# heheyas/V3D

Hardware: AMD Instinct MI355X
Metric: multi-view frames/sec, V3D_512 18-frame 25-step EDM (higher is better)
Workload: dtype bf16; 1 GPU; BASELINE.json configs[1]: V3D_512 random-init SVD-XT weights, 1x18x4x64x64 latent, 25 EulerEDM steps, cfg 4.5 (LinearPredictionGuider), 18-frame VideoDecoder decode to 512x512, one sample per GPU; frames=18, edm_steps=25, parallelism=replica x1, hip_graph=False

## Files before the change

include/v3d_hip.h:

```cpp
#ifndef V3D_HIP_H
#define V3D_HIP_H

#include <stdint.h>

#ifdef __cplusplus
extern "C" {
#endif

#define V3D_ABI_VERSION 9

typedef void* v3d_stream_t;

enum {
    V3D_OK = 0,
    V3D_ERR_ARG = -1,
    V3D_ERR_LAUNCH = -2,
};

int v3d_abi_version(void);
const char* v3d_last_error(void);
int v3d_device_info(int32_t* out4);

enum { V3D_GEMM_LINEAR = 0, V3D_GEMM_CONV3X3 = 1, V3D_GEMM_CONVT3 = 2 };

typedef struct v3d_gemm_args {
    const void* A;
    const void* W;
    void* out;
    const float* bias;
    const float* add;
    const void* res1;
    const void* res2;
    const float* coef;
    int64_t M, N, K;
    int64_t lda, ldw, ldo, ldr1, ldr2;
    int64_t a_rows;
    int64_t a_row0;
    int64_t add_rpg, add_ld;
    int64_t coef_rpg;
    float c_acc, c_res1, c_res2;
    int32_t mode, geglu, out_fp32;
    int32_t Hin, Win, Hout, Wout, stride, up;
    int32_t T, tmin, tmax;
    int64_t S;
    int32_t batch;
    int32_t pad_mode;
    int64_t sA, sW, sO;
    int64_t halo_rows;
    float* gn_stats;
    int64_t gn_rps;
    int32_t gn_cpg;
    int32_t gn_in_silu;
    int64_t gn_nslots;
    const float* gn_in_table;
    int64_t gn_in_rps;
    int64_t gn_in_rows;
    const void* A2;
    int64_t K1, lda2;
} v3d_gemm_args;

int v3d_gemm(const v3d_gemm_args* args, v3d_stream_t stream);
int v3d_gemm_gn_in_supported(const v3d_gemm_args* args);

int v3d_ff_fused(const void* x, int64_t ldx, const void* W1p, const float* b1, const void* W2p, const float* b2,
                 const void* res1, int64_t ldr1, const void* res2, int64_t ldr2, const float* coef, int64_t coef_rpg,
                 float c_acc, float c_res1, float c_res2, void* out, int64_t ldo, int64_t M, int32_t C, int32_t hidden,
                 v3d_stream_t stream);

int v3d_ln_ff_fused(const void* x, int64_t ldx, float ln_eps, const void* W1p, const float* b1, const void* W2p, const float* b2,
                 const void* res1, int64_t ldr1, const void* res2, int64_t ldr2, const float* coef, int64_t coef_rpg,
                 float c_acc, float c_res1, float c_res2, void* out, int64_t ldo, int64_t M, int32_t C, int32_t hidden,
                 v3d_stream_t stream);
int v3d_ln_proj(const void* x, int64_t ldx, float eps, const void* Wp, const float* bias, void* out, int64_t ldo, void* outT,
                int64_t M, int32_t C, int32_t N, int32_t n_rm, int64_t S, v3d_stream_t stream);
int v3d_sizeof_gemm_args(void);

int v3d_groupnorm_stats(const void* x1, int64_t C1, const void* x2, int64_t C2, float* stats, int64_t nslots,
                        int64_t n_img, int64_t S, int32_t groups, int64_t imgs_per_stat, v3d_stream_t stream);
int v3d_groupnorm_stats_table(const void* x1, int64_t C1, const void* x2, int64_t C2, float* stats, int64_t nslots, uint32_t* tickets,
                              int64_t n_img, int64_t S, int32_t groups, int64_t imgs_per_stat, const float* gamma, const float* beta,
                              double count, float eps, float* table, v3d_stream_t stream);
int v3d_groupnorm_finalize(const float* stats, int64_t nslots, double* sums, int64_t n_stat, int32_t groups,
                           const float* gamma, const float* beta, int64_t C, double count, float eps, float* table,
                           v3d_stream_t stream);
int v3d_groupnorm_apply(const void* x1, int64_t C1, const void* x2, int64_t C2, const float* table, void* out,
                        int64_t n_img, int64_t S, int64_t imgs_per_stat, int32_t silu, v3d_stream_t stream);

int v3d_groupnorm_small_supported(int64_t C1, int64_t C2, int64_t S, int32_t groups, int64_t imgs_per_stat);
int v3d_groupnorm_small(const void* x1, int64_t C1, const void* x2, int64_t C2, const float* gamma, const float* beta, void* out,
                        int64_t n_img, int64_t S, int32_t groups, int64_t imgs_per_stat, float eps, int32_t silu, v3d_stream_t stream);

int v3d_layernorm(const void* x, const float* add, int64_t add_rpg, int64_t add_ld, void* xsum_out,
                  const float* gamma, const float* beta, void* out, int64_t M, int64_t C, float eps,
                  v3d_stream_t stream);

int v3d_attn_spatial(const void* q, int64_t ldq, const void* k, int64_t ldk, const void* vT, void* out,
                     int64_t ldo, int64_t n_img, int64_t S, int32_t heads, float scale, v3d_stream_t stream);

int v3d_attn_spatial_ld(const void* q, int64_t ldq, const void* k, int64_t ldk, const void* vT, int64_t ldv, void* out,
                        int64_t ldo, int64_t n_img, int64_t S, int32_t heads, float scale, v3d_stream_t stream);

int v3d_quant_fp8_tiles(const void* x, int64_t ldx, void* x8, int64_t ld8, float* scales, int64_t n_img, int64_t S, int32_t ncols,
                        v3d_stream_t stream);
int v3d_quant_fp8_slab(const void* vT, void* v8, float* vscale, void* amax_scratch, int64_t n_img, int64_t S, int32_t heads, v3d_stream_t stream);
int v3d_attn_spatial_fp8(const void* qk8, int64_t ld8, const float* scales, const void* v8, const float* vscale, void* out, int64_t ldo,
                         int64_t n_img, int64_t S, int32_t heads, float scale, v3d_stream_t stream);

int v3d_attn_temporal(const void* q, int64_t q_sb, int64_t q_st, int64_t q_ss,
                      const void* k, const void* v, int64_t kv_sb, int64_t kv_st, int64_t kv_ss,
                      void* out, int64_t o_sb, int64_t o_st, int64_t o_ss,
                      int64_t B, int32_t Tq, int32_t Tk, int64_t S, int32_t heads, float scale,
                      v3d_stream_t stream);

int v3d_attn_vae_d512(const void* q, int64_t ldq, const void* k, int64_t ldk, const void* vT, const float* bias, void* out,
                      int64_t ldo, int64_t n_img, int64_t S, int32_t C, float scale, v3d_stream_t stream);

int v3d_softmax_rows(const float* in, void* out, int64_t rows, int64_t L, v3d_stream_t stream);

int v3d_timestep_embedding(const float* t, void* out_bf16, int64_t n, int32_t dim, float max_period, v3d_stream_t stream);
int v3d_silu_add(const float* in, const float* in2, void* out_bf16, int64_t n, v3d_stream_t stream);
int v3d_edm_scalings(const float* sigma, float* c_skip, float* c_out, float* c_in, float* c_noise, int64_t n, v3d_stream_t stream);
int v3d_pack_input(const float* x, const float* scale, int64_t C1, const float* cond, int64_t C2, void* out_bf16,
                   int64_t n, int64_t S, int64_t Cpad, v3d_stream_t stream);
int v3d_pack_input_im2col3x3(const float* x, const float* scale, int64_t C1, const float* cond, int64_t C2, void* out_bf16,
                             int64_t n, int32_t H, int32_t W, int64_t Kpad, v3d_stream_t stream);
int v3d_tapsum3x3(const float* y, int64_t ldy, const float* bias, float* out, int64_t n, int32_t H, int32_t W, int32_t C,
                  v3d_stream_t stream);
int v3d_denoise_combine(const float* net, int64_t ldn, const float* x, const float* c_out, const float* c_skip,
                        float* out, int64_t n, int64_t C, int64_t S, v3d_stream_t stream);
int v3d_cfg_combine(const float* x, const float* scale, float* out, int64_t n, int64_t T, int64_t chw, v3d_stream_t stream);
int v3d_euler_step(const float* x, const float* den, const float* sigma, const float* next_sigma, float* out,
                   int64_t n, int64_t chw, v3d_stream_t stream);
int v3d_heun_step(const float* x, const float* den, const float* euler, const float* den2, const float* sigma,
                  const float* next_sigma, float* out, int64_t n, int64_t chw, v3d_stream_t stream);
int v3d_clip_preprocess(const float* img, int64_t B, int32_t H, int32_t W, int32_t S, int32_t P, int32_t antialias,
                        const float* mean3, const float* std3, void* patches_bf16, int32_t Kpad, v3d_stream_t stream);
int v3d_gelu_bf16(const void* in, void* out, int64_t n, v3d_stream_t stream);
int v3d_frames_to_uint8(const float* x, void* out_u8, int64_t n, int32_t C, int64_t S, v3d_stream_t stream);
int v3d_axpb_f32(const float* x, float a, float b, float* out, int64_t n, v3d_stream_t stream);
int v3d_blend_coefs(const float* alpha, const int32_t* kind, const float* ioi, float* out, int64_t n_mixers, int64_t n_img, v3d_stream_t stream);
int v3d_nchw_to_nhwc_bf16(const float* x, float scale, void* out_bf16, int64_t n, int64_t C, int64_t S, int64_t Cpad, v3d_stream_t stream);
int v3d_tmix_small(const float* x, int64_t ld, const float* w, const float* b, float* out, int64_t B, int32_t T,
                   int64_t S, int32_t Cc, int32_t tmin, int32_t tmax, int64_t row0, v3d_stream_t stream);
int v3d_randn_add(const float* x, float scale, uint64_t seed, uint32_t call, float* out, int64_t B, int64_t T_local, int64_t T_global,
                  int64_t t0, int64_t row_elems, v3d_stream_t stream);
int v3d_lincomb_f32(const float* const* src, const float* coef, int32_t nterms, float* out, int64_t n, v3d_stream_t stream);
int v3d_copy2d_bf16(const void* src, int64_t lds, void* dst, int64_t ldd, int64_t rows, int64_t C, v3d_stream_t stream);

typedef struct v3d_gs_camera {
    float view[16];
    float proj[16];
    float tanfovx, tanfovy;
    float bg[3];
    int32_t width, height;
} v3d_gs_camera;

int v3d_gs_knn3(const float* xyz, int64_t n, float* out, v3d_stream_t stream);
int v3d_gs_preprocess_fwd(const float* xyz, const float* scale_raw, const float* rot_raw, const float* opacity_raw, const float* f_dc, int64_t P,
                          const v3d_gs_camera* cam, float* means2d, float* conic_opacity, float* rgb, float* depth, int32_t* radii,
                          int32_t* tiles_touched, int32_t* clamped, v3d_stream_t stream);
int64_t v3d_gs_scan_work_bytes(int64_t n);
int v3d_gs_scan(const int32_t* in, int64_t n, int32_t* out, void* work, int64_t work_bytes, v3d_stream_t stream);
int v3d_gs_duplicate_keys(const float* means2d, const int32_t* radii, const float* depth, const int32_t* offsets, int64_t P, int32_t width,
                          int32_t height, uint64_t* keys, uint32_t* vals, v3d_stream_t stream);
int64_t v3d_gs_sort_work_bytes(int64_t n);
int v3d_gs_radix_sort_pairs(const uint64_t* keys_in, const uint32_t* vals_in, uint64_t* keys_out, uint32_t* vals_out, int64_t n, int32_t nbits,
                            void* work, int64_t work_bytes, v3d_stream_t stream);
int v3d_gs_tile_ranges(const uint64_t* keys_sorted, const uint32_t* vals_sorted, int64_t n_inst, const float* means2d, const int32_t* radii,
                       const int32_t* offsets, int32_t width, int32_t height, int32_t* ranges, int32_t* inst_pos, v3d_stream_t stream);
int v3d_gs_render_fwd(const int32_t* ranges, const uint32_t* vals_sorted, const float* means2d, const float* conic_opacity, const float* rgb,
                      const v3d_gs_camera* cam, float* out_img, float* final_T, int32_t* n_contrib, v3d_stream_t stream);
int v3d_gs_render_bwd(const int32_t* ranges, const uint32_t* vals_sorted, const float* means2d, const float* conic_opacity, const float* rgb,
                      const v3d_gs_camera* cam, const float* final_T, const int32_t* n_contrib, const float* dL_dimg, float* inst_grads,
                      v3d_stream_t stream);
int v3d_gs_reduce_instance_grads(const float* inst_grads, const int32_t* offsets, const int32_t* inst_pos, int64_t P, float* grads9,
                                 v3d_stream_t stream);
int v3d_gs_preprocess_bwd(const float* xyz, const float* scale_raw, const float* rot_raw, const float* opacity_raw, int64_t P,
                          const v3d_gs_camera* cam, const int32_t* radii, const int32_t* clamped, const float* grads9, float* d_xyz,
                          float* d_scale_raw, float* d_rot_raw, float* d_opacity_raw, float* d_f_dc, float* d_means2d, v3d_stream_t stream);
int64_t v3d_gs_ssim_work_floats(int32_t C, int32_t H, int32_t W);
int v3d_gs_ssim_l1_fwd(const float* img, const float* gt, int32_t C, int32_t H, int32_t W, float lambda_dssim, float* work, int64_t work_floats,
                       float* out3, v3d_stream_t stream);
int v3d_gs_ssim_l1_bwd(const float* img, const float* gt, int32_t C, int32_t H, int32_t W, float lambda_dssim, float* work, int64_t work_floats,
                       const float* dloss, float* grad, v3d_stream_t stream);

#ifdef __cplusplus
}
#endif
#endif
```

v3d_amd/csrc/gemm.hip:

```cpp
#include <stdlib.h>

#include <map>
#include <mutex>
#include <vector>
#include <type_traits>

#include "gemm_common.h"


namespace {

__device__ __attribute__((aligned(256))) unsigned int g_zero_page[16384] = {0};

template <int KS>
__device__ __forceinline__ int swz_row(int row) {
    if (KS == 1) return (0x78 >> (((row >> 2) & 3) * 2)) & 3;
    return (row >> 1) & 7;
}

template <int BM, int BN, int WGM, int WGN, int NS, int KS, int MODE, bool GEGLU>
__global__ __launch_bounds__(64 * WGM * WGN, (64 * WGM * WGN) == 256 ? 2 : 1) void gemm_kernel_v2(GP p) {
    constexpr int BK2 = 32 * KS;
    constexpr int ROWB = BK2 * 2;
    constexpr int RPP = 1024 / ROWB;
// ... 114 lines not shown
    asm volatile("" ::: "memory");
    constexpr int NFO_ = GEGLU ? NF / 2 : NF;
    constexpr int STAGE_REGION = MF * 16 * (NFO_ * 32 + 16);
    constexpr bool CAN_STAGE = NW * STAGE_REGION <= NS * STAGE_BYTES;
    epilogue<MF, NF, GEGLU, CAN_STAGE>(p, acc, m0 + wm * WM, n0 + wn * WN, z, lane, lds + (CAN_STAGE ? wave * STAGE_REGION : 0));
}

constexpr int BK = 64;
constexpr int LROW = BK + 8;

template <int BM, int BN, int MODE, bool GEGLU>
__global__ __launch_bounds__(256, 2) void gemm_kernel_v1(GP p) {
    constexpr int AI = BM / 32;
    constexpr int BI = BN / 32;
    constexpr int WM = BM / 2, WN = BN / 2;
    constexpr int MF = WM / 16, NF = WN / 16;
    __shared__ __attribute__((aligned(16))) bf16_t sA[2][BM * LROW];
    __shared__ __attribute__((aligned(16))) bf16_t sB[2][BN * LROW];

    const int tid = threadIdx.x;
    const int lane = tid & 63;
    const int wave = tid >> 6;
    const int wm = wave >> 1, wn = wave & 1;
    const int bid = xcd_remap(blockIdx.x, p.mt * p.nt);
    int tile_m, tile_n;
    tile_coords(p, bid, tile_m, tile_n);
    const long long m0 = (long long)tile_m * BM;
    const long long n0 = (long long)tile_n * BN;
    const long long z = blockIdx.y;
    const bufrsrc_t rsA = make_rsrc(p.A + z * p.sA, p.a_bytes);
    const bufrsrc_t rsW = make_rsrc(p.W + z * p.sW, p.w_bytes);
    const int kc = tid & 7;
    const int r0 = tid >> 3;
    RowInfo<MODE> ri[AI];
#pragma unroll
    for (int i = 0; i < AI; ++i) ri[i].init(p, m0 + r0 + 32 * i);
    u32x4 ra[AI], rb[BI];
    unsigned aoff[AI], boff[BI];
    const int ksteps = (int)((p.K + BK - 1) / BK);
    const int nsteps = ksteps * ntaps<MODE>();
    int ld_tap = 0, ld_k0 = 0;
    auto set_tap = [&](int tap) {
#pragma unroll
        for (int i = 0; i < AI; ++i) {
            long long srow;
            const bool ok = ri[i].tap(p, tap, srow);
            aoff[i] = ok ? (unsigned)(((srow + p.a_row0) * p.lda + kc * 8) * 2) : kInvalid;
        }
#pragma unroll
        for (int i = 0; i < BI; ++i) {
            const long long n = n0 + r0 + 32 * i;
            boff[i] = (n < p.N) ? (unsigned)((((long long)tap * p.N + n) * p.ldw + kc * 8) * 2) : kInvalid;
        }
    };
    set_tap(0);
    auto gload = [&]() {
        const bool kok = (ld_k0 + kc * 8) < p.K;
        const unsigned kb = (unsigned)ld_k0 * 2u;
#pragma unroll
        for (int i = 0; i < AI; ++i) ra[i] = buf_load16(rsA, (kok && aoff[i] != kInvalid) ? aoff[i] + kb : kInvalid);
#pragma unroll
        for (int i = 0; i < BI; ++i) rb[i] = buf_load16(rsW, (kok && boff[i] != kInvalid) ? boff[i] + kb : kInvalid);
        ld_k0 += BK;
        if (ld_k0 >= p.K) {
            ld_k0 = 0;
            ++ld_tap;
            if (ntaps<MODE>() > 1 && ld_tap < ntaps<MODE>()) set_tap(ld_tap);
        }
    };
    auto lstore = [&](int buf) {
#pragma unroll
        for (int i = 0; i < AI; ++i) *reinterpret_cast<u32x4*>(&sA[buf][(r0 + 32 * i) * LROW + kc * 8]) = ra[i];
#pragma unroll
        for (int i = 0; i < BI; ++i) *reinterpret_cast<u32x4*>(&sB[buf][(r0 + 32 * i) * LROW + kc * 8]) = rb[i];
    };
    f32x4 acc[MF][NF];
#pragma unroll
    for (int i = 0; i < MF; ++i)
#pragma unroll
        for (int j = 0; j < NF; ++j) acc[i][j] = f32x4{0.f, 0.f, 0.f, 0.f};
    gload();
    lstore(0);
    __syncthreads();
    const int frow = lane & 15;
    const int fk = (lane >> 4) * 8;
    for (int step = 0; step < nsteps; ++step) {
        const int buf = step & 1;
        if (step + 1 < nsteps) gload();
#pragma unroll
        for (int kk = 0; kk < BK / 32; ++kk) {
            bf16x8 xf[MF], wf[NF];
#pragma unroll
            for (int i = 0; i < MF; ++i)
                xf[i] = *reinterpret_cast<const bf16x8*>(&sA[buf][(wm * WM + i * 16 + frow) * LROW + kk * 32 + fk]);
#pragma unroll
            for (int j = 0; j < NF; ++j)
                wf[j] = *reinterpret_cast<const bf16x8*>(&sB[buf][(wn * WN + j * 16 + frow) * LROW + kk * 32 + fk]);
#pragma unroll
            for (int i = 0; i < MF; ++i)
#pragma unroll
                for (int j = 0; j < NF; ++j)
                    acc[i][j] = __builtin_amdgcn_mfma_f32_16x16x32_bf16(wf[j], xf[i], acc[i][j], 0, 0, 0);
        }
        if (step + 1 < nsteps) lstore(buf ^ 1);
        __syncthreads();
    }
    epilogue<MF, NF, GEGLU, false>(p, acc, m0 + wm * WM, n0 + wn * WN, z, lane, nullptr);
}


template <int BM, int BN, int WGM, int WGN, int MODE, bool GEGLU, int EMF, int NS = 4, int SPAD = 16, bool GN = false>
__global__ __launch_bounds__(512, NS == 3 ? 4 : 2) void gemm_kernel_v3(GP p, int ntiles) {
    constexpr int ROWB = 64, NW = 8;
    static_assert(WGM * WGN == NW, "8 waves");
    constexpr int WM = BM / WGM, WN = BN / WGN;
    constexpr int MF = WM / 16, NF = WN / 16;
    static_assert(MF % EMF == 0, "epilogue chunking");
    constexpr int NPIECE = (BM + BN) / 16;
    constexpr int PPW = NPIECE / NW;
    static_assert(PPW * NW == NPIECE && PPW * 2 < 64, "tile / wave-count mismatch");
    constexpr int APIECES = BM / 16;
    constexpr int STAGE_BYTES = (BM + BN) * ROWB;
    constexpr int NFO = GEGLU ? NF / 2 : NF;
    constexpr int EPI_REGION = EMF * 16 * (NFO * 32 + SPAD);
    __shared__ __attribute__((aligned(1024))) unsigned char lds[NS * STAGE_BYTES + NW * EPI_REGION];

    const int tid = threadIdx.x;
    const int lane = tid & 63;
    const int wave = __builtin_amdgcn_readfirstlane(tid >> 6);
    const int grp = wave >> 2;
    const int wm = wave / WGN, wn = wave % WGN;
    const bf16_t* __restrict__ A = p.A;
    const bf16_t* __restrict__ W = p.W;
    unsigned char* estage = lds + NS * STAGE_BYTES + wave * EPI_REGION;

    const int G = gridDim.x;
    const int my_tiles = (ntiles - (int)blockIdx.x + G - 1) / G;
    auto tile_origin = [&](int it, long long& m0, long long& n0) __attribute__((always_inline)) {
        const int id = xcd_remap((int)blockIdx.x + it * G, ntiles);
        int tm, tn;
        tile_coords(p, id, tm, tn);
        n0 = (long long)tn * BN;
        m0 = (long long)tm * BM;
    };

    const bufrsrc_t rsA = make_rsrc(A, p.a_bytes);
    const bufrsrc_t rsW = make_rsrc(W, p.w_bytes);
    const int prow = lane >> 2;
    const unsigned kchunk_b = (unsigned)(((lane & 3) ^ swz_row<1>(prow)) * 16);
    RowInfo<MODE> ri[PPW];
    unsigned voff[PPW];
    long long ld_n0 = 0;
    int ld_it = 0, ld_tap = 0, ld_k0 = 0;
    auto set_tap = [&](int tap) __attribute__((always_inline)) {
#pragma unroll
        for (int i = 0; i < PPW; ++i) {
            const int q = wave + NW * i;
            if (q < APIECES) {
                long long s_;
                const bool ok = ri[i].tap(p, tap, s_);
                voff[i] = ok ? (unsigned)((s_ + p.a_row0) * p.lda * 2) + kchunk_b : kInvalid;
            } else {
                const long long n = ld_n0 + (q - APIECES) * 16 + prow;
                voff[i] = (n < p.N) ? (unsigned)(((long long)tap * p.N + n) * p.ldw * 2) + kchunk_b : kInvalid;
            }
        }
    };
    auto set_tile = [&](int it) __attribute__((always_inline)) {
        long long m0;
        tile_origin(it, m0, ld_n0);
#pragma unroll
        for (int i = 0; i < PPW; ++i) {
            const int q = wave + NW * i;
            if (q < APIECES) ri[i].init(p, m0 + q * 16 + prow);
        }
        set_tap(0);
    };
    set_tile(0);
    auto issue_piece = [&](int stage, int i, int so) __attribute__((always_inline)) {
        const int q = wave + NW * i;
        __builtin_amdgcn_raw_ptr_buffer_load_lds(q < APIECES ? rsA : rsW, (__attribute__((address_space(3))) void*)(lds + stage * STAGE_BYTES + q * 1024), 16, (int)voff[i], so, 0, 0);
    };
    auto issue_advance = [&]() __attribute__((always_inline)) {
        ld_k0 += 32;
        if (ld_k0 >= (int)p.K) {
            ld_k0 = 0;
            if (++ld_tap < ntaps<MODE>()) {
                set_tap(ld_tap);
            } else {
                ld_tap = 0;
                if (++ld_it < my_tiles) set_tile(ld_it);
                else if (ntaps<MODE>() > 1) set_tap(0);
            }
        }
    };
    auto issue = [&](int stage) __attribute__((always_inline)) {
        const int so = __builtin_amdgcn_readfirstlane(ld_k0 * 2);
#pragma unroll
        for (int i = 0; i < PPW; ++i) issue_piece(stage, i, so);
        issue_advance();
    };

    f32x4 acc[MF][NF];
#pragma unroll
    for (int i = 0; i < MF; ++i)
#pragma unroll
        for (int j = 0; j < NF; ++j) acc[i][j] = f32x4{0.f, 0.f, 0.f, 0.f};
    const int frag_off = (lane & 15) * ROWB + (((lane >> 4) ^ swz_row<1>(lane & 15)) * 16);
    const int a_base = wm * WM * ROWB;
    const int b_base = BM * ROWB + wn * WN * ROWB;
    bf16x8 xf[MF], wf[NF];

    const int nsteps = (int)(p.K / 32) * ntaps<MODE>();

#pragma unroll
    for (int st = 0; st < NS - 1; ++st) issue(st);
    asm volatile("s_waitcnt vmcnt(%0)" ::"n"(PPW * (NS - 2)) : "memory");
    __builtin_amdgcn_s_barrier();
    __builtin_amdgcn_sched_barrier(0);
    int s = 0;
    int rd = 0;
    for (int it = 0; it < my_tiles; ++it) {
        for (int kt = 0; kt < nsteps; ++kt, ++s) {
            {
                const unsigned char* sb = lds + rd * STAGE_BYTES;
#pragma unroll
                for (int i = 0; i < MF; ++i) xf[i] = *reinterpret_cast<const bf16x8*>(sb + a_base + frag_off + i * 16 * ROWB);
#pragma unroll
                for (int j = 0; j < NF; ++j) wf[j] = *reinterpret_cast<const bf16x8*>(sb + b_base + frag_off + j * 16 * ROWB);
            }
            issue(rd == 0 ? NS - 1 : rd - 1);
            rd = (rd + 1 == NS) ? 0 : rd + 1;
            if (grp == 1) {
                asm volatile("s_waitcnt lgkmcnt(0)" ::: "memory");
                __builtin_amdgcn_sched_barrier(0);
            }
            if (grp == 1) {
                asm volatile("s_waitcnt vmcnt(%0)" ::"n"(PPW * (NS - 2)) : "memory");
                __builtin_amdgcn_s_barrier();
                __builtin_amdgcn_sched_barrier(0);
            }
            __builtin_amdgcn_s_setprio(1);
#pragma unroll
            for (int i = 0; i < MF; ++i)
#pragma unroll
                for (int j = 0; j < NF; ++j)
                    acc[i][j] = __builtin_amdgcn_mfma_f32_16x16x32_bf16(wf[j], xf[i], acc[i][j], 0, 0, 0);
            __builtin_amdgcn_s_setprio(0);
            __builtin_amdgcn_sched_barrier(0);
            if (grp == 0) {
                asm volatile("s_waitcnt vmcnt(%0)" ::"n"(PPW * (NS - 2)) : "memory");
                __builtin_amdgcn_s_barrier();
            }
            __builtin_amdgcn_sched_barrier(0);
        }
        long long e_m0, e_n0;
        tile_origin(it, e_m0, e_n0);
        if constexpr (!GEGLU && EMF == 1 && SPAD == 16) {
            const long long mw0 = e_m0 + wm * WM, nw0 = e_n0 + wn * WN;
            if (mw0 < p.M && nw0 < p.N) {
                int lane_e = lane;
                asm volatile("" : "+v"(lane_e));
                auto rowfn = [&](int f) __attribute__((always_inline)) -> long long { return mw0 + f * 16; };
                E4GnRun<WM, MF> run;
                if constexpr (GN) run.init(mw0, p.gn_rps);
                auto flushfn = [&](int f, long long, unsigned& slot, unsigned& sid) __attribute__((always_inline)) -> bool { return run.step(f, slot, sid); };
                e4_retire_tile<MF, NF, GN>(p, acc, nw0, lane_e, estage, rowfn, flushfn);
            }
        } else
        {
            const long long mw0 = e_m0 + wm * WM, nw0 = e_n0 + wn * WN;
            const bool inside = mw0 < p.M && nw0 < p.N;
            const bool res_pre = p.res1 && !p.out_fp32 && (p.ldr1 % 8 == 0) && (reinterpret_cast<uintptr_t>(p.res1) % 16 == 0) && inside;
            u32x4 r0 = {0u, 0u, 0u, 0u}, r1 = r0, r2 = r0;
            if (res_pre) {
                r0 = load_res_piece<0, EMF, NF, GEGLU>(p, mw0, nw0, lane);
                r1 = load_res_piece<1, EMF, NF, GEGLU>(p, mw0, nw0, lane);
                r2 = load_res_piece<2, EMF, NF, GEGLU>(p, mw0, nw0, lane);
            }
            float4 bv[NF];
#pragma unroll
            for (int j = 0; j < NF; ++j)
                bv[j] = (p.bias && inside) ? *reinterpret_cast<const float4*>(p.bias + (int)nw0 + (lane >> 4) * 4 + j * 16) : make_float4(0.f, 0.f, 0.f, 0.f);
            GnAcc<GN ? NF : 1> gn;
            long long sid0 = 0;
            unsigned rem0 = 0;
            if constexpr (GN) {
                gn_zero(gn);
                sid0 = mw0 / p.gn_rps;
                rem0 = (unsigned)(mw0 - sid0 * p.gn_rps);
            }
            if (!GN || inside) v3_retire_chunks<0, MF / EMF, EMF, NF, GEGLU, SPAD, GN>(p, acc, mw0, nw0, lane, estage, r0, r1, r2, res_pre, bv, gn, sid0, rem0);
        }
#pragma unroll
        for (int i = 0; i < MF; ++i)
#pragma unroll
            for (int j = 0; j < NF; ++j) acc[i][j] = f32x4{0.f, 0.f, 0.f, 0.f};
    }
    asm volatile("s_waitcnt vmcnt(0)" ::: "memory");
}

template <int BM, int BN, int NS, int MODE>
__global__ __launch_bounds__(256, 2) void gemm_kernel_v6(GP p, int ntiles) {
    constexpr int ROWB = 64, NW = 4, WGN = 2;
    constexpr int WM = BM / 2, WN = BN / WGN, MF = WM / 16, NF = WN / 16;
    static_assert(NF == 5 || NF == 4, "the hand-managed epilogue retires 80- or 64-channel wave tiles");
    constexpr int NPIECE = (BM + BN) / 16, PPW = (NPIECE + NW - 1) / NW, APIECES = BM / 16, ARI = (APIECES + NW - 1) / NW;
    static_assert(PPW * (NS - 2) < 64, "vmcnt range");
    constexpr int STAGE_BYTES = NPIECE * 1024;
    constexpr int DUMMY_OFF = NS * STAGE_BYTES, NDUMMY = PPW * NW - NPIECE;
    constexpr int EPI_OFF = DUMMY_OFF + NDUMMY * 1024, EPI_REGION = 16 * (NF * 32 + 16);
    __shared__ __attribute__((aligned(1024))) unsigned char lds[EPI_OFF + NW * EPI_REGION];
    static_assert(sizeof(lds) <= 80 * 1024, "two blocks per CU");

    const int tid = threadIdx.x;
    const int lane = tid & 63;
    const int wave = __builtin_amdgcn_readfirstlane(tid >> 6);
    const int wm = wave / WGN, wn = wave % WGN;
    unsigned char* estage = lds + EPI_OFF + wave * EPI_REGION;
    const int G = gridDim.x;
    const int my_tiles = (ntiles - (int)blockIdx.x + G - 1) / G;
    auto tile_origin = [&](int it, long long& m0, long long& n0) __attribute__((always_inline)) {
        const int id = xcd_remap((int)blockIdx.x + it * G, ntiles);
        int tm, tn;
        tile_coords(p, id, tm, tn);
        n0 = (long long)tn * BN;
        m0 = (long long)tm * BM;
    };
    const bufrsrc_t rsA = make_rsrc(p.A, p.a_bytes);
    const bufrsrc_t rsW = make_rsrc(p.W, p.w_bytes);
    const int prow = lane >> 2;
    const unsigned kchunk_b = (unsigned)(((lane & 3) ^ swz_row<1>(prow)) * 16);
    RowInfo<MODE> ri[ARI];
    unsigned voff[PPW];
    long long ld_n0 = 0;
    int ld_it = 0, ld_tap = 0, ld_k0 = 0;
    auto set_tap = [&](int tap) __attribute__((always_inline)) {
#pragma unroll
        for (int i = 0; i < PPW; ++i) {
            const int q = wave + NW * i;
            if (i < ARI && q < APIECES) {
                long long s_;
                const bool ok = ri[i < ARI ? i : 0].tap(p, tap, s_);
                voff[i] = ok ? (unsigned)((s_ + p.a_row0) * p.lda * 2) + kchunk_b : kInvalid;
            } else {
                const long long n = ld_n0 + (q - APIECES) * 16 + prow;
                voff[i] = (q < NPIECE && n < p.N) ? (unsigned)(((long long)tap * p.N + n) * p.ldw * 2) + kchunk_b : kInvalid;
            }
        }
    };
    auto set_tile = [&](int it) __attribute__((always_inline)) {
        long long m0;
        tile_origin(it, m0, ld_n0);
#pragma unroll
        for (int i = 0; i < ARI; ++i) {
            const int q = wave + NW * i;
            if (q < APIECES) ri[i].init(p, m0 + q * 16 + prow);
        }
        set_tap(0);
    };
    set_tile(0);
    auto issue = [&](int stage) __attribute__((always_inline)) {
        const int so = __builtin_amdgcn_readfirstlane(ld_k0 * 2);
#pragma unroll
        for (int i = 0; i < PPW; ++i) {
            const int q = wave + NW * i;
            const int dst = q < NPIECE ? stage * STAGE_BYTES + q * 1024 : DUMMY_OFF + (q - NPIECE) * 1024;
            __builtin_amdgcn_raw_ptr_buffer_load_lds(q < APIECES ? rsA : rsW, (__attribute__((address_space(3))) void*)(lds + dst), 16, (int)voff[i], so, 0, 0);
        }
        ld_k0 += 32;
        if (ld_k0 >= (int)p.K) {
            ld_k0 = 0;
            if (++ld_tap < ntaps<MODE>()) {
                set_tap(ld_tap);
            } else {
                ld_tap = 0;
                if (++ld_it < my_tiles) set_tile(ld_it);
                else if (ntaps<MODE>() > 1) set_tap(0);
            }
        }
    };
    f32x4 acc[MF][NF];
#pragma unroll
    for (int i = 0; i < MF; ++i)
#pragma unroll
        for (int j = 0; j < NF; ++j) acc[i][j] = f32x4{0.f, 0.f, 0.f, 0.f};
    const int frag_off = (lane & 15) * ROWB + (((lane >> 4) ^ swz_row<1>(lane & 15)) * 16);
    const int a_base = wm * WM * ROWB;
    const int b_base = BM * ROWB + wn * WN * ROWB;
    bf16x8 xf[MF], wf[NF];
    const int nsteps = (int)(p.K / 32) * ntaps<MODE>();
#pragma unroll
    for (int st = 0; st < NS - 1; ++st) issue(st);
    asm volatile("s_waitcnt vmcnt(%0)" ::"n"(PPW * (NS - 2)) : "memory");
    __builtin_amdgcn_s_barrier();
    __builtin_amdgcn_sched_barrier(0);
    int rd = 0;
    for (int it = 0; it < my_tiles; ++it) {
        for (int kt = 0; kt < nsteps; ++kt) {
            {
                const unsigned char* sb = lds + rd * STAGE_BYTES;
#pragma unroll
                for (int i = 0; i < MF; ++i) xf[i] = *reinterpret_cast<const bf16x8*>(sb + a_base + frag_off + i * 16 * ROWB);
#pragma unroll
                for (int j = 0; j < NF; ++j) wf[j] = *reinterpret_cast<const bf16x8*>(sb + b_base + frag_off + j * 16 * ROWB);
            }
            issue(rd == 0 ? NS - 1 : rd - 1);
            rd = (rd + 1 == NS) ? 0 : rd + 1;
            __builtin_amdgcn_s_setprio(1);
#pragma unroll
            for (int i = 0; i < MF; ++i)
#pragma unroll
                for (int j = 0; j < NF; ++j)
                    acc[i][j] = __builtin_amdgcn_mfma_f32_16x16x32_bf16(wf[j], xf[i], acc[i][j], 0, 0, 0);
            __builtin_amdgcn_s_setprio(0);
            __builtin_amdgcn_sched_barrier(0);
            asm volatile("s_waitcnt vmcnt(%0)" ::"n"(PPW * (NS - 2)) : "memory");
            __builtin_amdgcn_s_barrier();
            __builtin_amdgcn_sched_barrier(0);
        }
        long long e_m0, e_n0;
        tile_origin(it, e_m0, e_n0);
        const long long mw0 = e_m0 + wm * WM, nw0 = e_n0 + wn * WN;
        if (mw0 < p.M && nw0 < p.N) {
            int lane_e = lane;
            asm volatile("" : "+v"(lane_e));
            auto rowfn = [&](int f) __attribute__((always_inline)) -> long long { return mw0 + f * 16; };
            auto flushfn = [&](int, long long, unsigned&, unsigned&) __attribute__((always_inline)) -> bool { return false; };
            e4_retire_tile<MF, NF, false>(p, acc, nw0, lane_e, estage, rowfn, flushfn);
        }
#pragma unroll
        for (int i = 0; i < MF; ++i)
#pragma unroll
            for (int j = 0; j < NF; ++j) acc[i][j] = f32x4{0.f, 0.f, 0.f, 0.f};
    }
    asm volatile("s_waitcnt vmcnt(0)" ::: "memory");
}

__global__ __launch_bounds__(256) void splitk_finalize_kernel(GP p) {
    const long long n4 = p.N / 4;
    const long long idx = (long long)blockIdx.x * 256 + threadIdx.x;
    if (idx >= p.M * n4) return;
    const long long m = idx / n4;
    const int n = (int)(idx - m * n4) * 4;
    float4 a = make_float4(0.f, 0.f, 0.f, 0.f);
    for (int sp = 0; sp < p.split_n; ++sp) {
        const float4 w = *reinterpret_cast<const float4*>(p.ws + ((long long)sp * p.M + m) * p.N + n);
        a.x += w.x; a.y += w.y; a.z += w.z; a.w += w.w;
    }
    if (p.bias) {
        const float4 b = *reinterpret_cast<const float4*>(p.bias + n);
        a.x += b.x; a.y += b.y; a.z += b.z; a.w += b.w;
    }
    if (p.add) {
        const float4 b = *reinterpret_cast<const float4*>(p.add + (m / p.add_rpg) * p.add_ld + n);
        a.x += b.x; a.y += b.y; a.z += b.z; a.w += b.w;
    }
    float ca = p.c_acc, c1 = p.c_res1, c2 = p.c_res2;
    if (p.coef) {
        const float* cf = p.coef + (m / p.coef_rpg) * 3;
        ca = cf[0]; c1 = cf[1]; c2 = cf[2];
    }
    float o[4] = {ca * a.x, ca * a.y, ca * a.z, ca * a.w};
    if (p.res1) {
        const uint2 rr = *reinterpret_cast<const uint2*>(p.res1 + m * p.ldr1 + n);
        o[0] += c1 * bflo(rr.x); o[1] += c1 * bfhi(rr.x); o[2] += c1 * bflo(rr.y); o[3] += c1 * bfhi(rr.y);
    }
    if (p.res2) {
        const uint2 rr = *reinterpret_cast<const uint2*>(p.res2 + m * p.ldr2 + n);
        o[0] += c2 * bflo(rr.x); o[1] += c2 * bfhi(rr.x); o[2] += c2 * bflo(rr.y); o[3] += c2 * bfhi(rr.y);
    }
    if (p.out_fp32)
        *reinterpret_cast<float4*>(reinterpret_cast<float*>(p.out) + m * p.ldo + n) = make_float4(o[0], o[1], o[2], o[3]);
    else
        *reinterpret_cast<uint2*>(reinterpret_cast<bf16_t*>(p.out) + m * p.ldo + n) = make_uint2(pack2bf(o[0], o[1]), pack2bf(o[2], o[3]));
}

float* splitk_workspace(size_t floats, hipStream_t st) {
    struct Slab { float* ptr; size_t cap; };
    static std::mutex mu;
    static std::map<hipStream_t, Slab> slabs;
    std::lock_guard<std::mutex> lock(mu);
    Slab& s = slabs[st];
    if (floats > s.cap) {
        hipStreamCaptureStatus cs = hipStreamCaptureStatusNone;
        if (hipStreamIsCapturing(st, &cs) != hipSuccess || cs != hipStreamCaptureStatusNone) return nullptr;
        const size_t want = floats + floats / 2;
        float* fresh = nullptr;
        if (hipMalloc(reinterpret_cast<void**>(&fresh), want * sizeof(float)) != hipSuccess) return nullptr;
        s.ptr = fresh;
        s.cap = want;
    }
    return s.ptr;
}

thread_local V3dLaunchInfo g_last_launch = {0, 0, 0, 0, 0, 0, 0};
long long g_gn_epilogue_launches = 0;
template <typename K>
int v3d_occupancy(K kernel, int threads) {
    int n = 0;
    if (hipOccupancyMaxActiveBlocksPerMultiprocessor(&n, kernel, threads, 0) != hipSuccess || n < 1) {
        (void)hipGetLastError();
        n = 1;
    }
    return n;
}
#define V3D_LAUNCH(KERNEL, ...)                                                                                          \
    do {                                                                                                                 \
        static const int occ_ = v3d_occupancy(KERNEL, pl.threads);                                                       \
        occ = occ_;                                                                                                      \
        hipLaunchKernelGGL(KERNEL, dim3(pl.grid_x, pl.grid_y, 1), dim3(pl.threads), 0, st, __VA_ARGS__);                 \
    } while (0)

struct GemmPolicy {
    int impl;
    int splitk;
    int v3s;
    int v6;
    int streamk;
};
const GemmPolicy& env_policy() {
    static const GemmPolicy pol = [] {
        auto rd = [](const char* name, int dflt) { const char* e = getenv(name); return e ? atoi(e) : dflt; };
        return GemmPolicy{rd("V3D_GEMM_IMPL", 0), rd("V3D_GEMM_SPLITK", -1), rd("V3D_GEMM_V3S", 2), rd("V3D_GEMM_V6", 1), rd("V3D_STREAMK", 1)};
    }();
    return pol;
}

enum GemmKernel {
    K_V1, K_V2_128_2x64, K_V2_128_3x32, K_V2_128_4x32, K_V2_256x64_2x64, K_V2_256x64_3x32, K_V2_256x128, K_SPLITK,
    K_V3_256, K_V3_256_GEGLU42, K_V3_256_GN, K_V3_192x320, K_V3_192x320_GN, K_V3_256x128_GEGLU, K_V6, K_HALO1, K_HALO2, K_HALO3, K_HALO4,
    K_COUNT, K_NONE = -1
};
struct GemmPlan {
    int kernel, family, bm, bn, mt, nt;
    long long tiles;
    unsigned grid_x, grid_y;
    int threads, group_m, splitk;
    int sk_tail, sk_full, sk_units;
    size_t sk_slot_bytes;
    bool gn_in_epilogue;
    int mode;
    bool geglu;
};

bool vec4_operands(const GP& p) {
    auto al = [](const void* q, uintptr_t a) { return (reinterpret_cast<uintptr_t>(q) % a) == 0; };
    return al(p.out, 16) && (!p.add || (al(p.add, 16) && p.add_ld % 4 == 0)) && (!p.res1 || (al(p.res1, 8) && p.ldr1 % 4 == 0)) &&
           (!p.res2 || (al(p.res2, 8) && p.ldr2 % 4 == 0));
}
bool v3_ok(const GP& p, int wm, int wn) { return p.M % wm == 0 && p.N % wn == 0 && p.ldo % (p.out_fp32 ? 4 : 8) == 0 && vec4_operands(p); }

GemmPlan plan_gemm(const GP& p, int mode, bool geglu, int batch, int cus, const GemmPolicy& pol) {
    GemmPlan pl = {};
    pl.kernel = K_NONE;
    pl.group_m = -1;
    pl.mode = mode;
    pl.geglu = geglu;
    auto cdiv = [](long long a, long long b) { return (a + b - 1) / b; };
    auto tile = [&](int kernel, int family, int bm, int bn, int threads) {
        pl.kernel = kernel; pl.family = family; pl.bm = bm; pl.bn = bn; pl.threads = threads;
        pl.mt = (int)cdiv(p.M, bm); pl.nt = (int)cdiv(p.N, bn);
        pl.tiles = (long long)pl.mt * pl.nt;
    };
    auto persistent = [&](long long slots) { pl.grid_x = (unsigned)(pl.tiles < slots ? pl.tiles : slots); pl.grid_y = 1; return pl; };
    auto fill = [&](long long bm, long long bn, long long slots) {
        const long long t = cdiv(p.M, bm) * cdiv(p.N, bn);
        return (double)t / (double)(cdiv(t, slots) * slots) * ((double)p.N / (double)(cdiv(p.N, bn) * bn));
    };
    const int taps = mode == V3D_GEMM_LINEAR ? 1 : (mode == V3D_GEMM_CONV3X3 ? 9 : 3);
    const bool dma_ok = v3d_k_steps_ok(p);

    if (p.gn_in) {
        const int halo = v3d_conv_halo_variant(p, mode);
        if (!halo) return pl;
        tile(K_HALO1 + halo - 1, 5, 192, 320, 512);
        pl.gn_in_epilogue = p.gn_stats != nullptr;
        const int G = cus, R = (int)(pl.tiles % G), units = (int)(p.K / 32);
        if (pol.streamk && R != 0 && (G - R) * 8 >= G && (long long)R * units / G >= 4 && (long long)(G - R) * units / G >= 2) {
            pl.sk_tail = R; pl.sk_full = (int)(pl.tiles / G); pl.sk_slot_bytes = (size_t)192 * 320 * 4;
            pl.grid_x = (unsigned)G; pl.grid_y = 1;
        } else {
            persistent(G);
        }
        pl.sk_units = units;
        return pl;
    }

    const bool n320 = !geglu && p.N % 320 == 0;
    const int bm3 = n320 ? 192 : 256, bn3 = n320 ? 320 : 256;
    const double fill3 = fill(bm3, bn3, cus);
    if (pol.v6 && pol.impl == 0 && mode != V3D_GEMM_CONV3X3 && !geglu && batch == 1 && dma_ok && p.M % 192 == 0 && p.N % 160 == 0 && !p.gn_stats && e4_ok(p, 96, 80)) {
        const long long t6 = (p.M / 192) * (p.N / 160), slots = 2ll * cus;
        if (t6 >= slots && (pol.v6 >= 2 || (p.K <= 1280 && fill3 < 0.9 && fill(192, 160, slots) >= fill3))) {
            tile(K_V6, 6, 192, 160, 256);
            pl.group_m = 0;
            return persistent(slots);
        }
    }
    const int bn2 = cdiv(p.N, 64) * 64 < cdiv(p.N, 128) * 128 ? 64 : 128;
    if (pol.impl != 1 && pol.impl != 2 && batch == 1 && dma_ok && p.N >= 256) {
        if (geglu && (p.K < 640 || pol.v3s >= 2) && pol.v3s && v3_ok(p, 64, 64) && cdiv(p.M, 256) * cdiv(p.N, 128) >= 2ll * cus) {
            tile(K_V3_256x128_GEGLU, 3, 256, 128, 512);
            return persistent(2ll * cus);
        }
        const bool want = pol.impl == 3 || fill3 >= 0.9 * fill(128, bn2, 2ll * cus);
        const bool eok = geglu || (n320 ? e4_ok(p, 96, 80) : e4_ok(p, 128, 64));
        if (want && eok && (n320 ? v3_ok(p, 96, 80) : v3_ok(p, 128, 128))) {
            const bool gn = !geglu && p.gn_stats && (n320 ? 80 : 64) % p.gn_cpg == 0 && p.gn_nslots >= p.gn_rps / (n320 ? 96 : 128) + 2;
            tile(n320 ? (gn ? K_V3_192x320_GN : K_V3_192x320) : gn ? K_V3_256_GN : (geglu && p.K < 640) ? K_V3_256_GEGLU42 : K_V3_256, 3, bm3, bn3, 512);
            pl.gn_in_epilogue = gn;
            return persistent(cus);
        }
    }
    tile(K_V1, 1, 128, bn2, 256);
    pl.grid_x = (unsigned)pl.tiles; pl.grid_y = (unsigned)batch;
    if (!geglu) {
        const long long steps = (long long)taps * (p.K / 32);
        int ways = pol.splitk;
        if (ways < 0) ways = (pl.tiles * 4 <= (long long)cus * 3 && steps >= 96) ? (int)((3ll * cus + pl.tiles - 1) / pl.tiles) : 1;
        if (ways > 4) ways = 4;
        if (ways > steps / 32) ways = (int)(steps / 32);
        if (ways > 1 && batch == 1 && pol.impl != 1 && p.K % 64 == 0 && p.K * 2 <= 65536 && p.N % 4 == 0 && p.ldo % 4 == 0 && vec4_operands(p)) {
            pl.kernel = K_SPLITK; pl.family = 2; pl.splitk = ways;
            pl.grid_y = (unsigned)ways;
            pl.tiles *= ways;
            return pl;
        }
    }
    const long long stages = (long long)taps * cdiv(p.K, 32);
    if (pol.impl == 1 || !dma_ok) {
    } else if (bn2 == 64) {
        tile(p.K % 64 == 0 ? K_V2_256x64_2x64 : K_V2_256x64_3x32, 2, 256, 64, 256);
    } else if (((geglu && p.K >= 640) || (mode == V3D_GEMM_CONV3X3 && p.K <= 128)) && p.M >= 4096) {
        tile(K_V2_256x128, 2, 256, 128, 256);
    } else if (stages <= 40) {
        pl.kernel = K_V2_128_3x32; pl.family = 2;
    } else {
        pl.kernel = p.K % 64 == 0 ? K_V2_128_2x64 : K_V2_128_4x32;
        pl.family = 2;
    }
    pl.grid_x = (unsigned)pl.tiles;
    pl.tiles *= batch;
    return pl;
}

struct SkWorkspace {
    hipStream_t st;
    float* ws;
    unsigned* flags;
    size_t slot_bytes;
    int G;
};
std::vector<SkWorkspace> g_sk;
std::mutex g_sk_mu;
long long g_sk_launches = 0;

bool sk_workspace(GP& p, size_t slot_bytes, int G, hipStream_t st) {
    std::lock_guard<std::mutex> lock(g_sk_mu);
    const SkWorkspace* w = nullptr;
    for (const SkWorkspace& c : g_sk)
        if (c.st == st && c.slot_bytes >= slot_bytes && c.G == G) w = &c;
    if (!w) {
        hipStreamCaptureStatus cs = hipStreamCaptureStatusNone;
        if (hipStreamIsCapturing(st, &cs) != hipSuccess || cs != hipStreamCaptureStatusNone) { (void)hipGetLastError(); return false; }
        SkWorkspace n = {st, nullptr, nullptr, slot_bytes, G};
        if (hipMalloc(reinterpret_cast<void**>(&n.ws), (size_t)G * slot_bytes) != hipSuccess ||
            hipMalloc(reinterpret_cast<void**>(&n.flags), ((size_t)G * 8 + 16) * 4) != hipSuccess ||
            hipMemset(n.flags, 0, ((size_t)G * 8 + 16) * 4) != hipSuccess) {
            (void)hipGetLastError();
            return false;
        }
        g_sk.push_back(n);
        w = &g_sk.back();
    }
    p.sk_ws = w->ws;
    p.sk_flags = w->flags;
    ++g_sk_launches;
    return true;
}

constexpr int kNoWorkspace = 1;

template <int MODE, bool GEGLU>
int launch_kernel(const GemmPlan& pl, GP& p, hipStream_t st, int& occ) {
    const int ntiles = (int)pl.tiles;
    switch (pl.kernel) {
        case K_V1:
            if (pl.bn == 64) V3D_LAUNCH((gemm_kernel_v1<128, 64, MODE, GEGLU>), p);
            else V3D_LAUNCH((gemm_kernel_v1<128, 128, MODE, GEGLU>), p);
            break;
        case K_V2_128_2x64: V3D_LAUNCH((gemm_kernel_v2<128, 128, 2, 2, 2, 2, MODE, GEGLU>), p); break;
        case K_V2_128_3x32: V3D_LAUNCH((gemm_kernel_v2<128, 128, 2, 2, 3, 1, MODE, GEGLU>), p); break;
        case K_V2_128_4x32: V3D_LAUNCH((gemm_kernel_v2<128, 128, 2, 2, 4, 1, MODE, GEGLU>), p); break;
        case K_V2_256x64_2x64: V3D_LAUNCH((gemm_kernel_v2<256, 64, 4, 1, 2, 2, MODE, GEGLU>), p); break;
        case K_V2_256x64_3x32: V3D_LAUNCH((gemm_kernel_v2<256, 64, 4, 1, 3, 1, MODE, GEGLU>), p); break;
        case K_V2_256x128: V3D_LAUNCH((gemm_kernel_v2<256, 128, 2, 2, 3, 1, MODE, GEGLU>), p); break;
        case K_SPLITK:
            if constexpr (!GEGLU) {
                float* ws = splitk_workspace((size_t)pl.splitk * (size_t)p.M * (size_t)p.N, st);
                if (!ws) return kNoWorkspace;
                GP q = p;
                q.split_n = pl.splitk;
                q.out = ws; q.out_fp32 = 1; q.ldo = p.N; q.sO = p.M * p.N; q.sA = 0; q.sW = 0;
                q.bias = nullptr; q.add = nullptr; q.res1 = nullptr; q.res2 = nullptr; q.coef = nullptr;
                q.c_acc = 1.f; q.c_res1 = 0.f; q.c_res2 = 0.f;
                if (pl.bn == 64) V3D_LAUNCH((gemm_kernel_v2<128, 64, 2, 2, 2, 2, MODE, GEGLU>), q);
                else V3D_LAUNCH((gemm_kernel_v2<128, 128, 2, 2, 2, 2, MODE, GEGLU>), q);
                p.split_n = pl.splitk;
                p.ws = ws;
                hipLaunchKernelGGL(splitk_finalize_kernel, dim3((unsigned)((p.M * (p.N / 4) + 255) / 256)), dim3(256), 0, st, p);
                return v3d_check_launch("v3d_gemm(split-K)");
            }
            break;
        case K_V3_256: V3D_LAUNCH((gemm_kernel_v3<256, 256, 2, 4, MODE, GEGLU, GEGLU ? 2 : 1>), p, ntiles); break;
        case K_V3_256_GEGLU42:
            if constexpr (GEGLU) V3D_LAUNCH((gemm_kernel_v3<256, 256, 4, 2, MODE, GEGLU, 1>), p, ntiles);
            break;
        case K_V3_256x128_GEGLU:
            if constexpr (GEGLU && MODE == V3D_GEMM_LINEAR) V3D_LAUNCH((gemm_kernel_v3<256, 128, 4, 2, MODE, GEGLU, 1, 3, 0>), p, ntiles);
            break;
        case K_V3_256_GN:
            if constexpr (!GEGLU) V3D_LAUNCH((gemm_kernel_v3<256, 256, 2, 4, MODE, GEGLU, 1, 4, 16, true>), p, ntiles);
            break;
        case K_V3_192x320:
            if constexpr (!GEGLU) V3D_LAUNCH((gemm_kernel_v3<192, 320, 2, 4, MODE, GEGLU, 1>), p, ntiles);
            break;
        case K_V3_192x320_GN:
            if constexpr (!GEGLU) V3D_LAUNCH((gemm_kernel_v3<192, 320, 2, 4, MODE, GEGLU, 1, 4, 16, true>), p, ntiles);
            break;
        case K_V6:
            if constexpr ((MODE == V3D_GEMM_LINEAR || MODE == V3D_GEMM_CONVT3) && !GEGLU) {
                V3D_LAUNCH((gemm_kernel_v6<192, 160, 3, MODE>), p, ntiles);
                return v3d_check_launch("v3d_gemm(v6)");
            }
            break;
    }
    return v3d_check_launch("v3d_gemm");
}

int launch_plan(const GemmPlan& pl, GP& p0, hipStream_t st) {
    GP p = p0;
    p.mt = pl.mt; p.nt = pl.nt; p.group_m = pl.group_m;
    int occ = 1, rc;
    if (pl.family == 5) {
        p.sk_units = pl.sk_units;
        if (pl.sk_tail) {
            if (!sk_workspace(p, pl.sk_slot_bytes, (int)pl.grid_x, st)) return kNoWorkspace;
            p.sk_tail = pl.sk_tail; p.sk_full = pl.sk_full;
        }
        rc = v3d_conv_halo_launch(p, pl.kernel - K_HALO1 + 1, (int)pl.grid_x, (int)pl.tiles, (void*)st);
    } else if (pl.mode == V3D_GEMM_LINEAR) {
        rc = pl.geglu ? launch_kernel<V3D_GEMM_LINEAR, true>(pl, p, st, occ) : launch_kernel<V3D_GEMM_LINEAR, false>(pl, p, st, occ);
    } else if (pl.mode == V3D_GEMM_CONV3X3) {
        rc = launch_kernel<V3D_GEMM_CONV3X3, false>(pl, p, st, occ);
    } else {
        rc = launch_kernel<V3D_GEMM_CONVT3, false>(pl, p, st, occ);
    }
    if (rc == kNoWorkspace) return rc;
    if (pl.family == 3 && pl.gn_in_epilogue) ++g_gn_epilogue_launches;
    g_last_launch = V3dLaunchInfo{pl.family, pl.bm, pl.bn, pl.tiles, occ, pl.splitk, pl.sk_tail};
    return rc;
}

int fill_params(const v3d_gemm_args* a, GP& p) {
    V3D_REQUIRE(a != nullptr, "v3d_gemm: null args");
    V3D_REQUIRE(a->A && a->W && a->out, "v3d_gemm: null A/W/out");
    V3D_REQUIRE(a->M > 0 && a->N > 0 && a->K > 0, "v3d_gemm: bad M/N/K (%lld,%lld,%lld)", (long long)a->M, (long long)a->N, (long long)a->K);
    V3D_REQUIRE(a->K % 8 == 0 && a->lda % 8 == 0, "v3d_gemm: K and lda must be multiples of 8 (K=%lld lda=%lld)", (long long)a->K, (long long)a->lda);
    V3D_REQUIRE(((uintptr_t)a->A & 15) == 0 && ((uintptr_t)a->W & 15) == 0, "v3d_gemm: A/W must be 16-byte aligned");
    V3D_REQUIRE(a->batch >= 1 && a->batch <= 65535, "v3d_gemm: bad batch %d", a->batch);
    V3D_REQUIRE(!a->geglu || (a->N % 32 == 0 && a->mode == V3D_GEMM_LINEAR), "v3d_gemm: geglu needs LINEAR mode and N %% 32 == 0");
    V3D_REQUIRE(!a->add || a->add_rpg > 0, "v3d_gemm: add_rpg must be > 0");
    V3D_REQUIRE(!a->coef || a->coef_rpg > 0, "v3d_gemm: coef_rpg must be > 0");
    V3D_REQUIRE(a->sA % 8 == 0 && a->sW % 8 == 0, "v3d_gemm: batch strides must keep 16-byte alignment");
    V3D_REQUIRE(a->a_rows > 0 && a->a_row0 >= 0, "v3d_gemm: a_rows (rows addressable behind A) must be given");
    V3D_REQUIRE(!a->bias || ((uintptr_t)a->bias & 15) == 0, "v3d_gemm: bias must be 16-byte aligned");
    const long long mtiles = (a->M + 127) / 128, ntiles = (a->N + 63) / 64;
    V3D_REQUIRE(mtiles * ntiles < (1ll << 31), "v3d_gemm: grid too large");
    const int taps = a->mode == V3D_GEMM_LINEAR ? 1 : (a->mode == V3D_GEMM_CONV3X3 ? 9 : 3);
    const long long ldw = a->ldw ? a->ldw : a->K;
    V3D_REQUIRE(ldw >= a->K && ldw % 8 == 0, "v3d_gemm: ldw must be >= K and a multiple of 8");
    const unsigned long long a_bytes = (unsigned long long)a->a_rows * a->lda * 2ull;
    const unsigned long long w_bytes = ((unsigned long long)(taps * a->N - 1) * ldw + a->K) * 2ull;
    V3D_REQUIRE(a_bytes <= kMaxBufBytes && w_bytes <= kMaxBufBytes, "v3d_gemm: operand larger than 4 GiB - 256 B (A %llu B, W %llu B)", a_bytes, w_bytes);
    p.A = (const bf16_t*)a->A; p.W = (const bf16_t*)a->W; p.out = a->out;
    p.bias = a->bias; p.add = a->add; p.res1 = (const bf16_t*)a->res1; p.res2 = (const bf16_t*)a->res2; p.coef = a->coef;
    p.M = a->M; p.N = a->N; p.K = a->K;
    p.lda = a->lda; p.ldw = ldw; p.ldo = a->ldo; p.ldr1 = a->ldr1; p.ldr2 = a->ldr2;
    p.add_rpg = a->add_rpg; p.add_ld = a->add_ld; p.coef_rpg = a->coef_rpg;
    p.c_acc = a->c_acc; p.c_res1 = a->c_res1; p.c_res2 = a->c_res2;
    p.out_fp32 = a->out_fp32;
    p.a_row0 = a->a_row0; p.a_bytes = (unsigned)a_bytes; p.w_bytes = (unsigned)w_bytes;
    p.Hin = a->Hin; p.Win = a->Win; p.Hout = a->Hout; p.Wout = a->Wout; p.stride = a->stride;
    p.upshift = 0;
    p.pad_lo = 1;
    p.T = a->T; p.tmin = a->tmin; p.tmax = a->tmax; p.S = a->S;
    p.halo_rows = a->mode == V3D_GEMM_CONVT3 ? a->halo_rows : 0;
    p.sA = a->sA; p.sW = a->sW; p.sO = a->sO;
    p.mt = p.nt = 0;
    p.group_m = -1;
    p.split_n = 1;
    p.ws = nullptr;
    p.sk_tail = p.sk_full = p.sk_units = 0; p.sk_ws = nullptr; p.sk_flags = nullptr;
    p.gn_stats = nullptr; p.gn_rps = 0; p.gn_cpg = 0; p.gn_nslots = 0;
    if (a->gn_stats) {
        V3D_REQUIRE(!a->geglu && !a->out_fp32 && a->batch == 1, "v3d_gemm: gn_stats needs a bf16, non-GEGLU, unbatched output");
        V3D_REQUIRE(a->gn_cpg > 0 && a->gn_cpg % 2 == 0 && a->N == 32ll * a->gn_cpg, "v3d_gemm: gn_stats needs N = 32 * gn_cpg (got N=%lld cpg=%d)", (long long)a->N, a->gn_cpg);
        V3D_REQUIRE(a->gn_rps >= 16 && a->gn_rps % 16 == 0 && a->gn_rps < (1ll << 30) && a->M % a->gn_rps == 0, "v3d_gemm: gn_rps must be a multiple of 16 that divides M");
        V3D_REQUIRE(a->ldo == a->N && ((uintptr_t)a->gn_stats & 7) == 0, "v3d_gemm: gn_stats needs a dense output (ldo == N) and an 8-byte aligned buffer");
        V3D_REQUIRE(a->gn_nslots >= 1, "v3d_gemm: gn_nslots must be >= 1");
        p.gn_stats = a->gn_stats; p.gn_rps = a->gn_rps; p.gn_cpg = a->gn_cpg; p.gn_nslots = a->gn_nslots;
    }
    p.A2 = (const bf16_t*)a->A2; p.K1 = a->A2 ? a->K1 : a->K; p.lda2 = a->lda2; p.a2_bytes = 0;
    p.gn_in = a->gn_in_table; p.gn_in_rps = a->gn_in_rps; p.gn_in_silu = a->gn_in_silu; p.gn_in_bytes = 0;
    if (a->A2) {
        V3D_REQUIRE(a->gn_in_table != nullptr, "v3d_gemm: a two-source input (A2) is only defined together with gn_in_table");
        const unsigned long long a2b = (unsigned long long)a->a_rows * a->lda2 * 2ull;
        V3D_REQUIRE(a->lda2 >= a->K - a->K1 && a2b <= kMaxBufBytes, "v3d_gemm: bad lda2 / A2 larger than 4 GiB - 256 B");
        p.a2_bytes = (unsigned)a2b;
    }
    if (a->gn_in_table) {
        V3D_REQUIRE(a->gn_in_rps > 0 && a->gn_in_rows > 0, "v3d_gemm: gn_in_table needs gn_in_rps and gn_in_rows");
        const unsigned long long tb = (unsigned long long)a->gn_in_rows * a->K * 8ull;
        V3D_REQUIRE(tb <= kMaxBufBytes && a->batch == 1 && !a->geglu, "v3d_gemm: gn_in_table too large / batched / GEGLU");
        p.gn_in_bytes = (unsigned)tb;
    }
    switch (a->mode) {
        case V3D_GEMM_LINEAR: break;
        case V3D_GEMM_CONV3X3:
            V3D_REQUIRE(a->up == 1 || a->up == 2, "v3d_gemm: up must be 1 or 2");
            V3D_REQUIRE(a->stride == 1 || a->stride == 2, "v3d_gemm: stride must be 1 or 2");
            V3D_REQUIRE(a->Hin > 0 && a->Win > 0 && a->Hout > 0 && a->Wout > 0, "v3d_gemm: bad conv geometry");
            V3D_REQUIRE(a->M % ((long long)a->Hout * a->Wout) == 0, "v3d_gemm: M must be n_img*Hout*Wout");
            V3D_REQUIRE(a->pad_mode == 0 || a->pad_mode == 1, "v3d_gemm: pad_mode must be 0 or 1");
            p.upshift = a->up - 1;
            p.pad_lo = a->pad_mode ? 0 : 1;
            break;
        case V3D_GEMM_CONVT3:
            V3D_REQUIRE(a->T > 0 && a->S > 0, "v3d_gemm: convt3 needs T,S");
            V3D_REQUIRE(a->halo_rows >= 0, "v3d_gemm: halo_rows must be >= 0");
            if (a->halo_rows > 0) {
                V3D_REQUIRE(a->M % ((long long)a->T * a->S) == 0 && a->halo_rows == a->M / a->T, "v3d_gemm: split-halo layout needs M = B*T*S and halo_rows = B*S");
                V3D_REQUIRE(a->a_row0 >= a->halo_rows && a->a_rows >= a->a_row0 + a->M + a->halo_rows, "v3d_gemm: split-halo layout: A must hold halo_rows rows on either side of the M local rows");
                V3D_REQUIRE(a->tmin >= -1 && a->tmax <= a->T, "v3d_gemm: split-halo layout carries one halo frame per side");
            }
            break;
        default:
            v3d_set_error("v3d_gemm: unknown mode %d", a->mode);
            return V3D_ERR_ARG;
    }
    return V3D_OK;
}

}

extern "C" int v3d_debug_last_gemm_launch(long long* out) {
    out[0] = g_last_launch.family; out[1] = g_last_launch.bm; out[2] = g_last_launch.bn; out[3] = g_last_launch.tiles;
    out[4] = g_last_launch.blocks_per_cu; out[5] = g_last_launch.splitk; out[6] = g_last_launch.streamk; out[7] = v3d_num_cus();
    return 0;
}

extern "C" int v3d_debug_gemm_plan(const v3d_gemm_args* a, int cus, const int* policy5, long long* out) {
    GP p;
    const int frc = fill_params(a, p);
    if (frc != V3D_OK) return frc;
    const GemmPolicy pol = policy5 ? GemmPolicy{policy5[0], policy5[1], policy5[2], policy5[3], policy5[4]} : env_policy();
    const GemmPlan pl = plan_gemm(p, a->mode, a->geglu != 0, a->batch, cus, pol);
    out[0] = pl.kernel; out[1] = pl.family; out[2] = pl.bm; out[3] = pl.bn; out[4] = pl.tiles; out[5] = (long long)pl.grid_x * pl.grid_y;
    out[6] = pl.splitk; out[7] = pl.sk_tail; out[8] = pl.gn_in_epilogue; out[9] = K_COUNT;
    return V3D_OK;
}

extern "C" long long v3d_debug_gn_epilogue_launches(void) { return g_gn_epilogue_launches; }

extern "C" int v3d_debug_sk_table(int ntiles, int units, int G, int b, int min_units, int min_saved, int* out) {
    const int R = ntiles % G;
    if (R == 0 || (G - R) * 8 < G || (long long)R * units / G < min_units || (long long)(G - R) * units / G < min_saved) return 0;
    V3dGemmParams p = {};
    p.sk_tail = R;
    p.sk_full = ntiles / G;
    p.sk_units = units;
    int tab[SK_TAB_BYTES / 4] = {0};
    sk_build_table(p, b, G, ntiles, units, tab);
    out[0] = tab[0];
    out[1] = tab[1];
    for (int k = 0; k < 2; ++k)
        for (int j = 0; j < 6; ++j) out[2 + 6 * k + j] = tab[4 + 8 * k + j];
    return 1;
}

extern "C" long long v3d_debug_sk_launches(void) { return g_sk_launches; }
extern "C" long long v3d_debug_sk_timeouts(void) {
    long long t = 0;
    std::lock_guard<std::mutex> lock(g_sk_mu);
    for (const SkWorkspace& c : g_sk) {
        unsigned v = 0;
        if (hipMemcpy(&v, c.flags + (size_t)c.G * 8, 4, hipMemcpyDeviceToHost) == hipSuccess) t += v;
    }
    return t;
}

extern "C" int v3d_gemm_gn_in_supported(const v3d_gemm_args* a) {
    GP p;
    if (!a || !a->gn_in_table || fill_params(a, p) != V3D_OK) return 0;
    return plan_gemm(p, a->mode, false, 1, v3d_num_cus(), env_policy()).kernel != K_NONE;
}

extern "C" int v3d_gemm(const v3d_gemm_args* a, v3d_stream_t stream) {
    GP p;
    const int frc = fill_params(a, p);
    if (frc != V3D_OK) return frc;
    hipStream_t st = (hipStream_t)stream;
    GemmPolicy pol = env_policy();
    GemmPlan pl = plan_gemm(p, a->mode, a->geglu != 0, a->batch, v3d_num_cus(), pol);
    V3D_REQUIRE(pl.kernel != K_NONE, "v3d_gemm: gn_in_table is set but this shape is not one of the LDS-haloed kernels' (v3d_gemm_gn_in_supported): "
                                     "normalise the input with v3d_groupnorm_apply first");
    int rc = launch_plan(pl, p, st);
    if (rc == kNoWorkspace) {
        pol.splitk = 0;
        pol.streamk = 0;
        pl = plan_gemm(p, a->mode, a->geglu != 0, a->batch, v3d_num_cus(), pol);
        rc = launch_plan(pl, p, st);
    }
    if (rc != V3D_OK || !p.gn_stats || pl.gn_in_epilogue) return rc;
    return v3d_groupnorm_stats(a->out, a->N, nullptr, 0, a->gn_stats, a->gn_nslots, a->M / a->gn_rps, a->gn_rps, 32, 1, stream);
}
```

v3d_amd/csrc/gemm_common.h:

```cpp
#pragma once
#include <type_traits>

#include "common.h"

#ifndef E4_ASM_READS
#define E4_ASM_READS 1
#endif

struct V3dGemmParams {
    const bf16_t* A;
    const bf16_t* W;
    void* out;
    const float* bias;
    const float* add;
    const bf16_t* res1;
    const bf16_t* res2;
    const float* coef;
    long long M, N, K;
    long long lda, ldw, ldo, ldr1, ldr2;
    long long add_rpg, add_ld, coef_rpg;
    float c_acc, c_res1, c_res2;
    int out_fp32;
    long long a_row0;
    unsigned a_bytes, w_bytes;
    int Hin, Win, Hout, Wout, stride, upshift;
    int pad_lo;
    int T, tmin, tmax;
    long long S;
    long long halo_rows;
    long long sA, sW, sO;
    int mt, nt;
    int group_m;
    int split_n;
    const float* ws;
    float* gn_stats;
    long long gn_rps;
    long long gn_nslots;
    int gn_cpg;
    const bf16_t* A2;
    long long K1, lda2;
    unsigned a2_bytes;
    const float* gn_in;
    long long gn_in_rps;
    int gn_in_silu;
    unsigned gn_in_bytes;
    int sk_tail;
    int sk_full;
    int sk_units;
    float* sk_ws;
    unsigned* sk_flags;
};

struct V3dLaunchInfo {
    int family, bm, bn;
    long long tiles;
    int blocks_per_cu, splitk, streamk;
};
int v3d_conv_halo_variant(const V3dGemmParams& p, int mode);
int v3d_conv_halo_launch(const V3dGemmParams& p, int variant, int grid, int ntiles, void* stream);
inline bool v3d_k_steps_ok(const V3dGemmParams& p) { return p.K % 32 == 0 && p.K * 2 <= 65536; }

namespace {

using GP = V3dGemmParams;

template <int I, int N, typename F>
__device__ __forceinline__ void static_for(F&& f) {
    if constexpr (I < N) {
        f(std::integral_constant<int, I>{});
        static_for<I + 1, N>(f);
    }
}

template <int MODE>
struct RowInfo {};

template <>
struct RowInfo<V3D_GEMM_LINEAR> {
    long long src;
    bool ok;
    __device__ void init(const GP& p, long long m) {
        ok = m < p.M;
        src = m;
    }
    __device__ bool tap(const GP&, int, long long& s) const {
        s = src;
        return ok;
    }
};

template <>
struct RowInfo<V3D_GEMM_CONV3X3> {
    long long base;
    int iy0, ix0;
    bool ok;
    __device__ void init(const GP& p, long long m) {
        ok = m < p.M;
        long long hw = (long long)p.Hout * p.Wout;
        long long img = m / hw;
        int rem = (int)(m - img * hw);
        int oy = rem / p.Wout;
        int ox = rem - oy * p.Wout;
        base = img * (long long)p.Hin * p.Win;
        iy0 = oy * p.stride - p.pad_lo;
        ix0 = ox * p.stride - p.pad_lo;
    }
    __device__ bool tap(const GP& p, int t, long long& s) const {
        int ky = t / 3, kx = t - ky * 3;
        int iy = iy0 + ky, ix = ix0 + kx;
        bool v = ok && iy >= 0 && ix >= 0 && iy < (p.Hin << p.upshift) && ix < (p.Win << p.upshift);
        s = base + (long long)(iy >> p.upshift) * p.Win + (ix >> p.upshift);
        return v;
    }
};

template <>
struct RowInfo<V3D_GEMM_CONVT3> {
    long long m_;
    long long hoff_;
    int t_;
    bool ok;
    __device__ void init(const GP& p, long long m) {
        ok = m < p.M;
        m_ = m;
        long long frame = m / p.S;
        t_ = (int)(frame % p.T);
        hoff_ = (frame / p.T) * p.S + (m - frame * p.S);
    }
    __device__ bool tap(const GP& p, int t, long long& s) const {
        int tt = t_ + t - 1;
        s = m_ + (long long)(t - 1) * p.S;
        if (p.halo_rows > 0) {
            if (tt < 0) s = hoff_ - p.halo_rows;
            else if (tt >= p.T) s = p.M + hoff_;
        }
        return ok && tt >= p.tmin && tt <= p.tmax;
    }
};

template <int MODE>
constexpr int ntaps() {
    return MODE == V3D_GEMM_LINEAR ? 1 : (MODE == V3D_GEMM_CONV3X3 ? 9 : 3);
}

__device__ __forceinline__ int xcd_remap(int bid, int nblk) {
    const int xcd = bid & 7, slot = bid >> 3;
    const int q = nblk >> 3, r = nblk & 7;
    return (xcd < r ? xcd * (q + 1) : r * (q + 1) + (xcd - r) * q) + slot;
}

__device__ __forceinline__ void tile_coords(const GP& p, int id, int& tm, int& tn) {
    const int gm = p.group_m >= 0 ? p.group_m : (p.mt >= 96 ? 8 : 4);
    if (gm <= 1 || p.nt == 1) {
        tn = id % p.nt;
        tm = id / p.nt;
        return;
    }
    const int width = gm * p.nt;
    const int gid = id / width;
    const int first = gid * gm;
    const int gsz = (p.mt - first) < gm ? (p.mt - first) : gm;
    const int r = id - gid * width;
    tn = r / gsz;
    tm = first + (r - tn * gsz);
}

template <int MF, int NF, bool GEGLU>
struct ResGeom {
    static constexpr int NFO = GEGLU ? NF / 2 : NF;
    static constexpr int CPRO = NFO * 2, ROWS = MF * 16, NV = (ROWS * CPRO + 63) / 64;
};
template <int K, int MF, int NF, bool GEGLU>
__device__ __forceinline__ u32x4 load_res_piece(const GP& p, long long mw0, long long nw0, int lane) {
    using G = ResGeom<MF, NF, GEGLU>;
    u32x4 r = {0u, 0u, 0u, 0u};
    if constexpr (K < G::NV) {
        const long long ncol0 = GEGLU ? ((nw0 >> 5) * 16) : nw0;
        const int c = K * 64 + lane;
        if ((G::ROWS * G::CPRO) % 64 == 0 || c < G::ROWS * G::CPRO)
            r = *reinterpret_cast<const u32x4*>(p.res1 + (mw0 + c / G::CPRO) * p.ldr1 + ncol0 + (c % G::CPRO) * 8);
    }
    return r;
}
template <int K, int MF, int NF, bool GEGLU>
__device__ __forceinline__ void res_piece_to_stage(u32x4 r, unsigned char* stage, int srow, int lane) {
    using G = ResGeom<MF, NF, GEGLU>;
    if constexpr (K < G::NV) {
        const int c = K * 64 + lane;
        if ((G::ROWS * G::CPRO) % 64 == 0 || c < G::ROWS * G::CPRO) *reinterpret_cast<u32x4*>(stage + (c / G::CPRO) * srow + (c % G::CPRO) * 16) = r;
    }
}

template <int NF>
struct GnAcc {
    float s[NF][2], q[NF][2];
};
template <int NF>
__device__ __forceinline__ void gn_zero(GnAcc<NF>& a) {
#pragma unroll
    for (int j = 0; j < NF; ++j) a.s[j][0] = a.s[j][1] = a.q[j][0] = a.q[j][1] = 0.f;
}
typedef __bf16 gn_bf16x2 __attribute__((ext_vector_type(2)));
__device__ __forceinline__ void gn_add_pair(float& s, float& q, uint32_t w) {
    const gn_bf16x2 v = __builtin_bit_cast(gn_bf16x2, w), ones = __builtin_bit_cast(gn_bf16x2, 0x3f803f80u);
    s = __builtin_amdgcn_fdot2_f32_bf16(v, ones, s, false);
    q = __builtin_amdgcn_fdot2_f32_bf16(v, v, q, false);
}
template <int CTRL>
__device__ __forceinline__ float dpp_row_shr(float v) {
    return __int_as_float(__builtin_amdgcn_update_dpp(0, __float_as_int(v), 0x110 | CTRL, 0xf, 0xf, true));
}
template <int NF>
__device__ __forceinline__ void gn_flush(const GP& p, GnAcc<NF>& a, long long sid, long long nw0, int lane, unsigned char* stage, unsigned slot) {
    float* sf = reinterpret_cast<float*>(stage);
#pragma unroll
    for (int j = 0; j < NF; ++j) {
        f32x4 t = {a.s[j][0], a.s[j][1], a.q[j][0], a.q[j][1]};
#pragma unroll
        for (int e = 0; e < 4; ++e) {
            float v = t[e];
            v += dpp_row_shr<1>(v);
            v += dpp_row_shr<2>(v);
            v += dpp_row_shr<4>(v);
            v += dpp_row_shr<8>(v);
            t[e] = v;
        }
        if ((lane & 15) == 15) lds_store16_nowait(sf + (j * 4 + (lane >> 4)) * 4, t);
    }
    const int cpg = p.gn_cpg;
    const int g_lo = (int)(nw0 / cpg), g_hi = (int)((nw0 + NF * 16 - 1) / cpg);
    const int g = g_lo + lane;
    if (g <= g_hi) {
        const int c0 = g * cpg > (int)nw0 ? g * cpg - (int)nw0 : 0;
        const int c1 = (g + 1) * cpg - (int)nw0 < NF * 16 ? (g + 1) * cpg - (int)nw0 : NF * 16;
        float sa = 0.f, sb = 0.f;
        for (int cp = c0 >> 1; cp < (c1 >> 1); ++cp) {
#if E4_ASM_READS
            const unsigned ea = lds_addr(sf + (cp >> 1) * 4 + (cp & 1));
            float e0, e2;
            asm volatile("ds_read_b32 %0, %2\n\tds_read_b32 %1, %2 offset:8\n\ts_waitcnt lgkmcnt(0)" : "=&v"(e0), "=&v"(e2) : "v"(ea) : "memory");
#else
            const float* e = sf + (cp >> 1) * 4 + (cp & 1);
            const float e0 = e[0], e2 = e[2];
#endif
            sa += e0;
            sb += e2;
        }
        float* dst = p.gn_stats + ((sid * p.gn_nslots + slot) * 32 + g) * 2;
        *reinterpret_cast<float2*>(dst) = make_float2(sa, sb);
    }
    gn_zero(a);
}

template <int MF, int NF, bool GEGLU, bool CAN_STAGE, bool FAST_ONLY = false, int SPAD = 16, bool GN = false>
__device__ __forceinline__ void epilogue(const GP& p, f32x4 (&acc)[MF][NF], long long mw0, long long nw0, long long z, int lane,
                                         unsigned char* stage, u32x4 pre0, u32x4 pre1, u32x4 pre2, bool res_pre,
                                         const float4 (&bias_pre)[NF], bool has_bias_pre, GnAcc<GN ? NF : 1>* gn = nullptr) {
    const long long Nout = GEGLU ? p.N / 2 : p.N;
    constexpr int NFO = GEGLU ? NF / 2 : NF;
    constexpr int SROW = NFO * 32 + SPAD;
    const long long ncol0 = GEGLU ? ((nw0 >> 5) * 16) : nw0;
    const bool staged = CAN_STAGE && !p.out_fp32 && (p.ldo % 8 == 0) && (ncol0 % 8 == 0) &&
                        ((reinterpret_cast<uintptr_t>(p.out) + (size_t)z * p.sO * 2) % 16 == 0);
    const bool vec_ok = (p.ldo % 4 == 0) && (!p.res1 || p.ldr1 % 4 == 0) && (!p.res2 || p.ldr2 % 4 == 0);
    const bool fast = (mw0 + MF * 16 <= p.M) && (nw0 + NF * 16 <= p.N) && vec_ok && (staged || p.out_fp32) &&
                      (!p.add || ((reinterpret_cast<uintptr_t>(p.add) % 16 == 0) && (p.add_ld % 4 == 0))) &&
                      (!p.res1 || reinterpret_cast<uintptr_t>(p.res1) % 8 == 0) && (!p.res2 || reinterpret_cast<uintptr_t>(p.res2) % 8 == 0);
    const int fr = lane & 15, fq = (lane >> 4) * 4;
    if (FAST_ONLY && (mw0 >= p.M || nw0 >= p.N)) return;
    if (FAST_ONLY || fast) {
        const int nb = (int)nw0 + fq;
        constexpr int CPRO = NFO * 2;
        constexpr int ROWS = MF * 16;
        constexpr bool WHOLE = (ROWS * CPRO) % 64 == 0;
        const bool res1_lds = CAN_STAGE && p.res1 && !p.out_fp32 && (p.ldr1 % 8 == 0) && (reinterpret_cast<uintptr_t>(p.res1) % 16 == 0);
        if (CAN_STAGE && res1_lds) {
            if (res_pre) {
                res_piece_to_stage<0, MF, NF, GEGLU>(pre0, stage, SROW, lane);
                res_piece_to_stage<1, MF, NF, GEGLU>(pre1, stage, SROW, lane);
                res_piece_to_stage<2, MF, NF, GEGLU>(pre2, stage, SROW, lane);
            } else {
                const bf16_t* rz = p.res1 + mw0 * p.ldr1 + ncol0;
                uint4 rv[(ROWS * CPRO + 63) / 64];
#pragma unroll
                for (int c0 = 0; c0 < ROWS * CPRO; c0 += 64) {
                    const int c = c0 + lane;
                    if (WHOLE || c < ROWS * CPRO) rv[c0 / 64] = *reinterpret_cast<const uint4*>(rz + (long long)(c / CPRO) * p.ldr1 + (c % CPRO) * 8);
                }
#pragma unroll
                for (int c0 = 0; c0 < ROWS * CPRO; c0 += 64) {
                    const int c = c0 + lane;
                    if (WHOLE || c < ROWS * CPRO) *reinterpret_cast<uint4*>(stage + (c / CPRO) * SROW + (c % CPRO) * 16) = rv[c0 / 64];
                }
            }
            asm volatile("s_waitcnt lgkmcnt(0)" ::: "memory");
// ... 116 lines not shown
#pragma unroll
                for (int r = 0; r < 4; ++r) {
                    float g = acc[i][jg][r];
                    if (ng + r < p.N) {
                        if (p.bias) g += p.bias[ng + r];
                        if (addv) g += addv[ng + r];
                    }
                    v[r] = v[r] * gelu_erf_f(g);
                }
                col = (np >> 5) * 16 + (np & 15);
            }
            if (col >= Nout) continue;
#pragma unroll
            for (int r = 0; r < 4; ++r) {
                if (col + r < Nout) {
                    float o = ca * v[r];
                    if (p.res1) o += c1 * bf2f(p.res1[m * p.ldr1 + col + r]);
                    if (p.res2) o += c2 * bf2f(p.res2[m * p.ldr2 + col + r]);
                    if (p.out_fp32)
                        (reinterpret_cast<float*>(p.out) + z * p.sO + m * p.ldo + col)[r] = o;
                    else
                        (reinterpret_cast<bf16_t*>(p.out) + z * p.sO + m * p.ldo + col)[r] = f2bf(o);
                }
            }
        }
    }
}

template <int MF, int NF, bool GEGLU, bool CAN_STAGE, bool FAST_ONLY = false>
__device__ __forceinline__ void epilogue(const GP& p, f32x4 (&acc)[MF][NF], long long mw0, long long nw0, long long z, int lane,
                                         unsigned char* stage) {
    const u32x4 none = {0u, 0u, 0u, 0u};
    float4 nob[NF];
    epilogue<MF, NF, GEGLU, CAN_STAGE, FAST_ONLY>(p, acc, mw0, nw0, z, lane, stage, none, none, none, false, nob, false);
}


template <int C, int NCH, int EMF, int NF, bool GEGLU, int SPAD, bool GN>
__device__ __forceinline__ void v3_retire_chunks(const GP& p, f32x4 (&acc)[NCH * EMF][NF], long long mw0, long long nw0, int lane, unsigned char* estage,
                                                 u32x4 c0, u32x4 c1, u32x4 c2, bool res_pre, const float4 (&bv)[NF], GnAcc<GN ? NF : 1>& gn,
                                                 long long sid0, unsigned rem0) {
    static_assert(ResGeom<EMF, NF, GEGLU>::NV <= 3, "v3 epilogue chunk: at most 3 residual pieces per lane");
    if constexpr (C < NCH) {
        u32x4 n0 = c0, n1 = c1, n2 = c2;
        if constexpr (C + 1 < NCH) {
            if (res_pre) {
                n0 = load_res_piece<0, EMF, NF, GEGLU>(p, mw0 + (C + 1) * EMF * 16, nw0, lane);
                n1 = load_res_piece<1, EMF, NF, GEGLU>(p, mw0 + (C + 1) * EMF * 16, nw0, lane);
                n2 = load_res_piece<2, EMF, NF, GEGLU>(p, mw0 + (C + 1) * EMF * 16, nw0, lane);
            }
        }
        epilogue<EMF, NF, GEGLU, true, true, SPAD, GN>(p, *reinterpret_cast<f32x4(*)[EMF][NF]>(&acc[C * EMF]), mw0 + C * EMF * 16, nw0, 0, lane, estage, c0, c1, c2, res_pre, bv, true, &gn);
        if constexpr (GN) {
            static_assert(EMF == 1, "GN epilogue: one row fragment per chunk");
            const unsigned rps = (unsigned)p.gn_rps;
            const unsigned here = (rem0 + C * 16) / rps, next = (rem0 + (C + 1) * 16) / rps;
            const unsigned off = here == rem0 / rps ? rem0 - here * rps : 0u;
            if (C + 1 == NCH || next != here) gn_flush<NF>(p, gn, sid0 + here, nw0, lane, estage, (off + NCH * 16 - 1) / (NCH * 16));
        }
        v3_retire_chunks<C + 1, NCH, EMF, NF, GEGLU, SPAD, GN>(p, acc, mw0, nw0, lane, estage, n0, n1, n2, res_pre, bv, gn, sid0, rem0);
    }
}


struct E4Res {
    u32x4 a0, a1, a2;
};
template <int NF>
struct E4Tile {
    f32x4 ba[NF];
    float ca, c1, c2;
    unsigned add_grp, coef_grp, add_rem, coef_rem;
};
__device__ __forceinline__ unsigned e4_udiv(unsigned a, unsigned b) {
    return (unsigned)__builtin_amdgcn_readfirstlane((int)(a / b));
}
__device__ __forceinline__ u32x4 e4_load16(const void* ptr) {
    u32x4 r;
    asm volatile("global_load_dwordx4 %0, %1, off" : "=v"(r) : "v"(ptr) : "memory");
    return r;
}
__device__ __forceinline__ float e4_load4(const float* ptr) {
    float r;
    asm volatile("global_load_dword %0, %1, off" : "=v"(r) : "v"(ptr) : "memory");
    return r;
}
template <int NF>
__device__ __forceinline__ void e4_load_res(const GP& p, long long m0f, long long nw0, int lane, E4Res& r) {
    constexpr int CPRO = NF * 2, NP = 16 * CPRO;
    auto piece = [&](const bf16_t* base, long long ld, int k) __attribute__((always_inline)) -> u32x4 {
        int c = k * 64 + lane;
        if (NP % 64 != 0 && c >= NP) c = lane;
        return e4_load16(base + (m0f + c / CPRO) * ld + nw0 + (c % CPRO) * 8);
    };
    r.a0 = piece(p.res1, p.ldr1, 0);
    r.a1 = piece(p.res1, p.ldr1, 1);
    if constexpr (NP > 128) r.a2 = piece(p.res1, p.ldr1, 2);
}
__device__ __forceinline__ void e4_wait_res(E4Res& r) {
    asm volatile("s_waitcnt vmcnt(0)" : "+v"(r.a0), "+v"(r.a1), "+v"(r.a2)::"memory");
}
template <int N>
__device__ __forceinline__ void e4_wait_cnt(E4Res& r) {
    static_assert(N >= 0 && N < 64, "vmcnt range");
    asm volatile("s_waitcnt vmcnt(%3)" : "+v"(r.a0), "+v"(r.a1), "+v"(r.a2) : "n"(N) : "memory");
}
template <int NF>
__device__ __forceinline__ void e4_tile_consts(const GP& p, long long m0f, long long nw0, int lane, E4Tile<NF>& t) {
    const int nb = (int)nw0 + (lane >> 4) * 4;
    f32x4 bv[NF], av[NF];
    float cf0 = p.c_acc, cf1 = p.c_res1, cf2 = p.c_res2;
#pragma unroll
    for (int j = 0; j < NF; ++j) bv[j] = av[j] = f32x4{0.f, 0.f, 0.f, 0.f};
    if (p.bias) {
#pragma unroll
        for (int j = 0; j < NF; ++j) bv[j] = __builtin_bit_cast(f32x4, e4_load16(p.bias + nb + j * 16));
    }
    t.add_grp = p.add ? e4_udiv((unsigned)m0f, (unsigned)p.add_rpg) : 0u;
    t.add_rem = p.add ? (unsigned)m0f - t.add_grp * (unsigned)p.add_rpg : 0u;
    if (p.add) {
        const float* av0 = p.add + (long long)t.add_grp * p.add_ld + nb;
#pragma unroll
        for (int j = 0; j < NF; ++j) av[j] = __builtin_bit_cast(f32x4, e4_load16(av0 + j * 16));
    }
    t.coef_grp = p.coef ? e4_udiv((unsigned)m0f, (unsigned)p.coef_rpg) : 0u;
    t.coef_rem = p.coef ? (unsigned)m0f - t.coef_grp * (unsigned)p.coef_rpg : 0u;
    if (p.coef) {
        const float* cf = p.coef + (long long)t.coef_grp * 3;
        cf0 = e4_load4(cf);
        cf1 = e4_load4(cf + 1);
        cf2 = e4_load4(cf + 2);
    }
    static_assert(NF == 4 || NF == 5, "e4: 64- or 80-channel wave tiles");
    if constexpr (NF == 5)
        asm volatile("s_waitcnt vmcnt(0)" : "+v"(bv[0]), "+v"(bv[1]), "+v"(bv[2]), "+v"(bv[3]), "+v"(bv[4]), "+v"(av[0]), "+v"(av[1]), "+v"(av[2]), "+v"(av[3]),
                     "+v"(av[4]), "+v"(cf0), "+v"(cf1), "+v"(cf2)::"memory");
    else
        asm volatile("s_waitcnt vmcnt(0)" : "+v"(bv[0]), "+v"(bv[1]), "+v"(bv[2]), "+v"(bv[3]), "+v"(av[0]), "+v"(av[1]), "+v"(av[2]), "+v"(av[3]), "+v"(cf0),
                     "+v"(cf1), "+v"(cf2)::"memory");
#pragma unroll
    for (int j = 0; j < NF; ++j) t.ba[j] = bv[j] + av[j];
    t.ca = cf0;
    t.c1 = cf1;
    t.c2 = cf2;
}
__device__ __forceinline__ void e4_lds_read8(u32x2& dst, unsigned addr) { asm volatile("ds_read_b64 %0, %1" : "=v"(dst) : "v"(addr) : "memory"); }
__device__ __forceinline__ void e4_lds_read16(u32x4& dst, unsigned addr) { asm volatile("ds_read_b128 %0, %1" : "=v"(dst) : "v"(addr) : "memory"); }
__device__ __forceinline__ void e4_lds_write16(unsigned addr, u32x4 v) { asm volatile("ds_write_b128 %0, %1" ::"v"(addr), "v"(v) : "memory"); }
__device__ __forceinline__ void e4_lds_write8(unsigned addr, uint32_t w0, uint32_t w1) {
    const u32x2 v = {w0, w1};
    asm volatile("ds_write_b64 %0, %1" ::"v"(addr), "v"(v) : "memory");
}

template <int NF, bool GN, int RD = E4_ASM_READS>
__device__ __forceinline__ void e4_fragment(const GP& p, f32x4 (&acc)[NF], long long m0f, long long nw0, int lane, unsigned char* stage, const E4Res& cur,
                                            const E4Tile<NF>& t, GnAcc<GN ? NF : 1>& gn) {
    constexpr int CPRO = NF * 2, NP = 16 * CPRO, SROW = NF * 32 + 16;
    const int fr = lane & 15, fq = (lane >> 4) * 4;
    const unsigned sbase = lds_addr(stage);
    auto piece_addr = [&](int k) __attribute__((always_inline)) -> unsigned {
        const int c = k * 64 + lane;
        return sbase + (unsigned)((c / CPRO) * SROW + (c % CPRO) * 16);
    };
    const int mine_off = fr * SROW + fq * 2;
    const unsigned mine = sbase + (unsigned)mine_off;
    const bool has1 = p.res1 != nullptr, has2 = p.res2 != nullptr;
    if (has1) {
        e4_lds_write16(piece_addr(0), cur.a0);
        e4_lds_write16(piece_addr(1), cur.a1);
        if constexpr (NP > 128) {
            if (NP % 64 == 0 || lane < NP - 128) e4_lds_write16(piece_addr(2), cur.a2);
        }
    }
    u32x2 q2[NF];
#pragma unroll
    for (int j = 0; j < NF; ++j) q2[j] = u32x2{0u, 0u};
    if (has2) {
        const bf16_t* r2 = p.res2 + (m0f + fr) * p.ldr2 + nw0 + fq;
#pragma unroll
        for (int j = 0; j < NF; ++j) asm volatile("global_load_dwordx2 %0, %1, off" : "=v"(q2[j]) : "v"(r2 + j * 16) : "memory");
        static_assert(NF == 4 || NF == 5, "e4: 64- or 80-channel wave tiles");
        if constexpr (NF == 5)
            asm volatile("s_waitcnt vmcnt(0)" : "+v"(q2[0]), "+v"(q2[1]), "+v"(q2[2]), "+v"(q2[3]), "+v"(q2[4])::"memory");
        else
            asm volatile("s_waitcnt vmcnt(0)" : "+v"(q2[0]), "+v"(q2[1]), "+v"(q2[2]), "+v"(q2[3])::"memory");
    }
    if constexpr (RD != 0) {
    u32x2 rr[RD == 1 ? NF : 1];
#pragma unroll
    for (int j = 0; j < (RD == 1 ? NF : 1); ++j) rr[j] = u32x2{0u, 0u};
    if (has1) {
        asm volatile("s_waitcnt lgkmcnt(0)" ::: "memory");
        if constexpr (RD == 1) {
#pragma unroll
            for (int j = 0; j < NF; ++j) e4_lds_read8(rr[j], mine + j * 32);
            static_assert(NF == 4 || NF == 5, "e4: 64- or 80-channel wave tiles");
            if constexpr (NF == 5) asm volatile("s_waitcnt lgkmcnt(0)" : "+v"(rr[0]), "+v"(rr[1]), "+v"(rr[2]), "+v"(rr[3]), "+v"(rr[RD == 1 ? 4 : 0])::"memory");
            else asm volatile("s_waitcnt lgkmcnt(0)" : "+v"(rr[0]), "+v"(rr[1]), "+v"(rr[2]), "+v"(rr[3])::"memory");
        }
    }
#pragma unroll
    for (int j = 0; j < NF; ++j) {
        float o[4];
#pragma unroll
        for (int r = 0; r < 4; ++r) o[r] = (acc[j][r] + t.ba[j][r]) * t.ca;
        if (has1) {
            const int jr = RD == 1 ? j : 0;
            if constexpr (RD != 1) {
                e4_lds_read8(rr[0], mine + j * 32);
                asm volatile("s_waitcnt lgkmcnt(0)" : "+v"(rr[0])::"memory");
            }
            o[0] += t.c1 * bflo(rr[jr][0]); o[1] += t.c1 * bfhi(rr[jr][0]); o[2] += t.c1 * bflo(rr[jr][1]); o[3] += t.c1 * bfhi(rr[jr][1]);
        }
        if (has2) {
            o[0] += t.c2 * bflo(q2[j][0]); o[1] += t.c2 * bfhi(q2[j][0]); o[2] += t.c2 * bflo(q2[j][1]); o[3] += t.c2 * bfhi(q2[j][1]);
        }
        const uint32_t w0 = pack2bf(o[0], o[1]), w1 = pack2bf(o[2], o[3]);
        e4_lds_write8(mine + j * 32, w0, w1);
        if constexpr (GN) {
            gn_add_pair(gn.s[j][0], gn.q[j][0], w0);
            gn_add_pair(gn.s[j][1], gn.q[j][1], w1);
        }
    }
    asm volatile("s_waitcnt lgkmcnt(0)" ::: "memory");
    bf16_t* outz = reinterpret_cast<bf16_t*>(p.out) + m0f * p.ldo + nw0;
    constexpr int NK = (NP + 63) / 64;
    static_assert(NK == 2 || NK == 3, "row pieces per lane");
#pragma unroll
    for (int k = 0; k < NK; ++k) {
        const int c = k * 64 + lane;
        int cr = c;
        if (NP % 64 != 0 && cr >= NP) cr = lane;
        u32x4 sr;
        e4_lds_read16(sr, sbase + (unsigned)((cr / CPRO) * SROW + (cr % CPRO) * 16));
        asm volatile("s_waitcnt lgkmcnt(0)" : "+v"(sr)::"memory");
        const int row = c / CPRO, ch = c % CPRO;
        if (NP % 64 == 0 || c < NP) *reinterpret_cast<u32x4*>(outz + (long long)row * p.ldo + ch * 8) = sr;
    }
    } else {
    if (has1) asm volatile("s_waitcnt lgkmcnt(0)" ::: "memory");
#pragma unroll
    for (int j = 0; j < NF; ++j) {
        float o[4];
#pragma unroll
        for (int r = 0; r < 4; ++r) o[r] = (acc[j][r] + t.ba[j][r]) * t.ca;
        if (has1) {
            const uint2 rr = *reinterpret_cast<const uint2*>(stage + mine_off + j * 32);
            o[0] += t.c1 * bflo(rr.x); o[1] += t.c1 * bfhi(rr.x); o[2] += t.c1 * bflo(rr.y); o[3] += t.c1 * bfhi(rr.y);
        }
        if (has2) {
            o[0] += t.c2 * bflo(q2[j][0]); o[1] += t.c2 * bfhi(q2[j][0]); o[2] += t.c2 * bflo(q2[j][1]); o[3] += t.c2 * bfhi(q2[j][1]);
        }
        const uint32_t w0 = pack2bf(o[0], o[1]), w1 = pack2bf(o[2], o[3]);
        e4_lds_write8(mine + j * 32, w0, w1);
        if constexpr (GN) {
            gn_add_pair(gn.s[j][0], gn.q[j][0], w0);
            gn_add_pair(gn.s[j][1], gn.q[j][1], w1);
        }
    }
    asm volatile("s_waitcnt lgkmcnt(0)" ::: "memory");
    bf16_t* outz = reinterpret_cast<bf16_t*>(p.out) + m0f * p.ldo + nw0;
#pragma unroll
    for (int k = 0; k < (NP + 63) / 64; ++k) {
        const int c = k * 64 + lane;
        const int row = c / CPRO, ch = c % CPRO;
        if (NP % 64 == 0 || c < NP) *reinterpret_cast<uint4*>(outz + (long long)row * p.ldo + ch * 8) = *reinterpret_cast<const uint4*>(stage + row * SROW + ch * 16);
    }
    }
}

template <int NF>
struct E4Cnt {
    static constexpr int NP = 16 * NF * 2;
    static constexpr int LOADS = NP > 128 ? 3 : 2;
    static constexpr int STORES = (NP + 63) / 64;
};
template <int WMR, int MF>
struct E4GnRun {
    unsigned sid, rem, sid0, rem0, rps;
    __device__ __forceinline__ void init(long long mw0, long long gn_rps) {
        rps = (unsigned)gn_rps;
        sid0 = sid = rps ? e4_udiv((unsigned)mw0, rps) : 0u;
        rem0 = rem = (unsigned)mw0 - sid * rps;
    }
    __device__ __forceinline__ bool step(int f, unsigned& slot, unsigned& sid_out) {
        const unsigned first = sid == sid0 ? rem0 : 0u;
        slot = (first + WMR - 1) / WMR;
        sid_out = sid;
        rem += 16;
        const bool ends = rem >= rps;
        if (ends) {
            rem -= rps;
            ++sid;
        }
        return f + 1 == MF || ends;
    }
};
template <int F, int MF, int NF, bool GN, int RD, typename RowFn, typename FlushFn>
__device__ __forceinline__ void e4_retire(const GP& p, f32x4 (&acc)[MF][NF], long long nw0, int lane, unsigned char* stage, E4Res cur, E4Res n1, E4Res n2,
                                          E4Tile<NF> t, GnAcc<GN ? NF : 1>& gn, RowFn rowfn, FlushFn flushfn) {
    if constexpr (F < MF) {
        const long long m0f = rowfn(F);
        const bool has1 = p.res1 != nullptr;
        E4Res n3 = n2;
        if constexpr (F + 1 < MF) {
            if (has1) e4_load_res<NF>(p, rowfn(F + 1), nw0, lane, n1);
        }
        if constexpr (F >= 1) {
            if (has1) e4_wait_cnt<E4Cnt<NF>::STORES + (F + 1 < MF ? E4Cnt<NF>::LOADS : 0)>(cur);
        }
        bool regroup = false;
        if constexpr (F > 0) {
            const unsigned d = (unsigned)(m0f - rowfn(F - 1));
            t.add_rem += d;
            t.coef_rem += d;
            regroup = (p.add && t.add_rem >= (unsigned)p.add_rpg) || (p.coef && t.coef_rem >= (unsigned)p.coef_rpg);
        }
        if (regroup) {
            e4_tile_consts<NF>(p, m0f, nw0, lane, t);
            asm volatile("" : "+v"(n1.a0), "+v"(n1.a1), "+v"(n1.a2), "+v"(n2.a0), "+v"(n2.a1), "+v"(n2.a2), "+v"(n3.a0), "+v"(n3.a1), "+v"(n3.a2));
        }
        {
            f32x4 accf[NF];
#pragma unroll
            for (int j = 0; j < NF; ++j) accf[j] = acc[F][j];
            e4_fragment<NF, GN, RD>(p, accf, m0f, nw0, lane, stage, cur, t, gn);
        }
        if constexpr (GN) {
            unsigned slot = 0, sid = 0;
            if (flushfn(F, m0f, slot, sid)) gn_flush<NF>(p, gn, (long long)sid, nw0, lane, stage, slot);
        }
        e4_retire<F + 1, MF, NF, GN, RD>(p, acc, nw0, lane, stage, n1, n2, n3, t, gn, rowfn, flushfn);
    }
}
template <int MF, int NF, bool GN, int RD = E4_ASM_READS, typename RowFn, typename FlushFn>
__device__ __forceinline__ void e4_retire_tile(const GP& p, f32x4 (&acc)[MF][NF], long long nw0, int lane, unsigned char* stage, RowFn rowfn, FlushFn flushfn) {
    E4Res r0, r1, r2;
    r0.a0 = r0.a1 = r0.a2 = u32x4{0u, 0u, 0u, 0u};
    r1 = r0;
    r2 = r0;
    if (p.res1) e4_load_res<NF>(p, rowfn(0), nw0, lane, r0);
    E4Tile<NF> t;
    e4_tile_consts<NF>(p, rowfn(0), nw0, lane, t);
    asm volatile("" : "+v"(r0.a0), "+v"(r0.a1), "+v"(r0.a2), "+v"(r1.a0), "+v"(r1.a1), "+v"(r1.a2), "+v"(r2.a0), "+v"(r2.a1), "+v"(r2.a2));
    GnAcc<GN ? NF : 1> gn;
    if constexpr (GN) gn_zero(gn);
    e4_retire<0, MF, NF, GN, RD>(p, acc, nw0, lane, stage, r0, r1, r2, t, gn, rowfn, flushfn);
}

struct SkItem {
    int tile;
    int u0, u1;
    int role;
    int d0, d1;
};
constexpr int SK_TAB_BYTES = 96;
__host__ __device__ __forceinline__ void sk_build_table(const GP& p, int b, int G, int ntiles, int U, int* tab) {
    tab[1] = 0;
    if (p.sk_tail == 0) {
        tab[0] = (ntiles - b + G - 1) / G;
        return;
    }
    const long long RU = (long long)p.sk_tail * U;
    const long long lo = b * RU / G, hi = (b + 1) * RU / G;
    int n = 0;
    for (long long a = lo; a < hi; ++n) {
        const long long jt = a / U, t0 = jt * U, t1 = t0 + U;
        const long long e = hi < t1 ? hi : t1;
        int* q = tab + 4 + 8 * n;
        q[0] = p.sk_full * G + (int)jt;
        q[1] = (int)(a - t0);
        q[2] = (int)(e - t0);
        q[3] = a > t0 ? 1 : (e < t1 ? 2 : 0);
        q[4] = b + 1;
        q[5] = (int)((t1 * G + RU - 1) / RU) - 1;
        if (n == 0 && q[3] == 1) tab[1] = 1;
        a = e;
    }
    tab[0] = p.sk_full + n;
}
__device__ __forceinline__ SkItem sk_item(const GP& p, int b, int G, int i, int nitems, int ndonor, int U, const int* tab) {
    SkItem it;
    it.u0 = 0; it.u1 = U; it.role = 0; it.d0 = it.d1 = 0;
    it.tile = i < nitems ? b + (i - ndonor) * G : -1;
    if (p.sk_tail != 0 && i < nitems && (i < ndonor || i >= ndonor + p.sk_full)) {
        const int* q = tab + 4 + 8 * (i < ndonor ? 0 : ndonor);
        it.tile = __builtin_amdgcn_readfirstlane(q[0]);
        it.u0 = __builtin_amdgcn_readfirstlane(q[1]);
        it.u1 = __builtin_amdgcn_readfirstlane(q[2]);
        it.role = __builtin_amdgcn_readfirstlane(q[3]);
        it.d0 = __builtin_amdgcn_readfirstlane(q[4]);
        it.d1 = __builtin_amdgcn_readfirstlane(q[5]);
    }
    return it;
}
template <int MF, int NF>
__device__ __forceinline__ void sk_publish(const GP& p, const f32x4 (&acc)[MF][NF], int blk, int wave, int lane) {
    asm volatile("" : "+v"(lane));
    const float* base = p.sk_ws + ((size_t)blk * 8 + wave) * (MF * NF) * 256;
    unsigned voff = (unsigned)lane * 16u;
#pragma unroll
    for (int i = 0; i < MF; ++i)
#pragma unroll
        for (int j = 0; j < NF; ++j) {
            constexpr int dummy = 0;
            (void)dummy;
            const int k = i * NF + j;
            if (k % 4 == 0 && k > 0) voff += 4096u;
            switch (k % 4) {
                case 0: asm volatile("global_store_dwordx4 %0, %1, %2 sc0 sc1\n\ts_nop 1" ::"v"(voff), "v"(acc[i][j]), "s"(base) : "memory"); break;
                case 1: asm volatile("global_store_dwordx4 %0, %1, %2 offset:1024 sc0 sc1\n\ts_nop 1" ::"v"(voff), "v"(acc[i][j]), "s"(base) : "memory"); break;
                case 2: asm volatile("global_store_dwordx4 %0, %1, %2 offset:2048 sc0 sc1\n\ts_nop 1" ::"v"(voff), "v"(acc[i][j]), "s"(base) : "memory"); break;
                default: asm volatile("global_store_dwordx4 %0, %1, %2 offset:3072 sc0 sc1\n\ts_nop 1" ::"v"(voff), "v"(acc[i][j]), "s"(base) : "memory"); break;
            }
        }
    asm volatile("s_waitcnt vmcnt(0)" ::: "memory");
    if (lane == 0) __hip_atomic_store(p.sk_flags + blk * 8 + wave, 1u, __ATOMIC_RELAXED, __HIP_MEMORY_SCOPE_AGENT);
}
template <int MF, int NF>
__device__ __forceinline__ void sk_gather(const GP& p, f32x4 (&acc)[MF][NF], int d0, int d1, int wave, int lane, int G) {
    asm volatile("" : "+v"(lane));
    for (int d = d0; d <= d1; ++d) {
        unsigned* flag = p.sk_flags + d * 8 + wave;
        bool ok = false;
        for (int spin = 0; spin < (1 << 21); ++spin) {
            if (__builtin_amdgcn_readfirstlane((int)__hip_atomic_load(flag, __ATOMIC_RELAXED, __HIP_MEMORY_SCOPE_AGENT)) != 0) { ok = true; break; }
            __builtin_amdgcn_s_sleep(4);
        }
        if (!ok) {
            if (lane == 0) atomicAdd(p.sk_flags + G * 8, 1u);
            continue;
        }
        __builtin_amdgcn_fence(__ATOMIC_ACQUIRE, "agent");
        const float* base = p.sk_ws + ((size_t)d * 8 + wave) * (MF * NF) * 256;
        static_assert(MF % 2 == 0, "rows are gathered in pairs");
        auto load = [&](f32x4& dst, int k) __attribute__((always_inline)) {
            const unsigned voff = (unsigned)lane * 16u + (unsigned)(k / 4) * 4096u;
            switch (k % 4) {
                case 0: asm volatile("global_load_dwordx4 %0, %1, %2 sc0 sc1" : "=v"(dst) : "v"(voff), "s"(base) : "memory"); break;
                case 1: asm volatile("global_load_dwordx4 %0, %1, %2 offset:1024 sc0 sc1" : "=v"(dst) : "v"(voff), "s"(base) : "memory"); break;
                case 2: asm volatile("global_load_dwordx4 %0, %1, %2 offset:2048 sc0 sc1" : "=v"(dst) : "v"(voff), "s"(base) : "memory"); break;
                default: asm volatile("global_load_dwordx4 %0, %1, %2 offset:3072 sc0 sc1" : "=v"(dst) : "v"(voff), "s"(base) : "memory"); break;
            }
        };
#pragma unroll
        for (int i = 0; i < MF; i += 2) {
            f32x4 r[2 * NF];
#pragma unroll
            for (int j = 0; j < 2 * NF; ++j) load(r[j], i * NF + j);
            if constexpr (NF == 5)
                asm volatile("s_waitcnt vmcnt(0)" : "+v"(r[0]), "+v"(r[1]), "+v"(r[2]), "+v"(r[3]), "+v"(r[4]), "+v"(r[5]), "+v"(r[6]), "+v"(r[7]), "+v"(r[8]), "+v"(r[9])::"memory");
            else if constexpr (NF == 4)
                asm volatile("s_waitcnt vmcnt(0)" : "+v"(r[0]), "+v"(r[1]), "+v"(r[2]), "+v"(r[3]), "+v"(r[4]), "+v"(r[5]), "+v"(r[6]), "+v"(r[7])::"memory");
            else
                static_assert(NF == 4 || NF == 5, "wait statement for this fragment count");
#pragma unroll
            for (int j = 0; j < 2 * NF; ++j) acc[i + j / NF][j % NF] += r[j];
        }
        if (lane == 0) __hip_atomic_store(flag, 0u, __ATOMIC_RELAXED, __HIP_MEMORY_SCOPE_AGENT);
    }
}

inline bool e4_ok(const V3dGemmParams& p, int wm, int wn) {
    auto al = [](const void* q, uintptr_t a) { return (reinterpret_cast<uintptr_t>(q) % a) == 0; };
    if (p.out_fp32 || p.M % wm || p.N % wn || p.ldo % 8 || !al(p.out, 16)) return false;
    if (p.M >= (1ll << 32) || (p.add && p.add_rpg >= (1ll << 32)) || (p.coef && p.coef_rpg >= (1ll << 32))) return false;
    if (p.bias && !al(p.bias, 16)) return false;
    if (p.add && (!al(p.add, 16) || p.add_ld % 4 || p.add_rpg % 16)) return false;
    if (p.res1 && (!al(p.res1, 16) || p.ldr1 % 8)) return false;
    if (p.res2 && (!al(p.res2, 8) || p.ldr2 % 4)) return false;
    if (p.coef && p.coef_rpg % 16) return false;
    return true;
}

}
```

v3d_amd/engine/packing.py:

```python
from __future__ import annotations

from dataclasses import dataclass, field
from typing import Dict, List, Optional

import torch
import torch.nn as nn

BF, F32 = torch.bfloat16, torch.float32


def _bf(t: torch.Tensor) -> torch.Tensor:
    from ..ops import get_ops
    return t.detach().to(get_ops().act_dtype).contiguous()


def _f(t: torch.Tensor) -> torch.Tensor:
    return t.detach().to(F32).contiguous()


def round_up(x: int, m: int) -> int:
    return (x + m - 1) // m * m


def pack_linear(lin: nn.Linear, k_pad: int = 0):
    w = lin.weight.detach()
    if k_pad and w.shape[1] < k_pad:
        w = torch.cat([w, w.new_zeros(w.shape[0], k_pad - w.shape[1])], dim=1)
    return _bf(w), (None if lin.bias is None else _f(lin.bias))


def pack_conv1x1(conv: nn.Module):
    w = conv.weight.detach()
    return _bf(w.reshape(w.shape[0], w.shape[1])), (None if conv.bias is None else _f(conv.bias))


def pack_conv3x3(conv: nn.Conv2d):
    w = conv.weight.detach()
    O, I = w.shape[0], w.shape[1]
    Ip = round_up(I, 8)
    if Ip != I:
        w = torch.cat([w, w.new_zeros(O, Ip - I, 3, 3)], dim=1)
    return _bf(w.permute(2, 3, 0, 1).reshape(9, O, Ip)), (None if conv.bias is None else _f(conv.bias))


def pack_conv3x3_im2col(conv: nn.Conv2d, Kpad=96):
    w = conv.weight.detach()
    O, I = w.shape[0], w.shape[1]
    assert I <= 8 and Kpad >= 72
    wp = w.new_zeros(O, Kpad)
    wp.view(O, Kpad)[:, :72].view(O, 9, 8)[:, :, :I] = w.permute(0, 2, 3, 1).reshape(O, 9, I)
    return _bf(wp), (None if conv.bias is None else _f(conv.bias))


def pack_conv3x3_taps(conv: nn.Conv2d, Npad=64):
    w = conv.weight.detach()
    O, I = w.shape[0], w.shape[1]
    assert 9 * O <= Npad
    wp = w.new_zeros(Npad, I)
    wp[:9 * O] = w.permute(2, 3, 0, 1).reshape(9 * O, I)
    return _bf(wp), (None if conv.bias is None else _f(conv.bias))


def pack_convt3(conv: nn.Conv3d):
    w = conv.weight.detach()
    O, I = w.shape[0], w.shape[1]
    return _bf(w.reshape(O, I, 3).permute(2, 0, 1)), (None if conv.bias is None else _f(conv.bias))


def pack_geglu(lin: nn.Linear):
    w, b = lin.weight.detach(), lin.bias.detach()
    inner = w.shape[0] // 2
    assert inner % 16 == 0
    wv, wg = w[:inner].reshape(inner // 16, 16, -1), w[inner:].reshape(inner // 16, 16, -1)
    wp = torch.stack([wv, wg], dim=1).reshape(2 * inner, -1)
    bp = torch.stack([b[:inner].reshape(-1, 16), b[inner:].reshape(-1, 16)], dim=1).reshape(2 * inner)
    return _bf(wp), _f(bp)


def pack_norm(n: nn.Module):
    return _f(n.weight), _f(n.bias), float(n.eps)


@dataclass
class ResPack:
    cin: int
    cout: int
    split: Optional[tuple]
    gn1: tuple = None
    w1: torch.Tensor = None
    b1: torch.Tensor = None
    gn2: tuple = None
    w2: torch.Tensor = None
    b2: torch.Tensor = None
    skip_w: Optional[torch.Tensor] = None
    skip_b: Optional[torch.Tensor] = None
    emb_off: int = -1
    t_gn1: tuple = None
    t_w1: torch.Tensor = None
    t_b1: torch.Tensor = None
    t_gn2: tuple = None
    t_w2: torch.Tensor = None
    t_b2: torch.Tensor = None
    t_emb_off: int = -1
    mixer: int = -1
    alpha: float = 0.0


@dataclass
class FFPack:
    w1: torch.Tensor
    b1: torch.Tensor
    w2: torch.Tensor
    b2: torch.Tensor
    w1_fused: Optional[torch.Tensor] = None
    b1_fused: Optional[torch.Tensor] = None
    w2_fused: Optional[torch.Tensor] = None
    w1_ln_fused: Optional[torch.Tensor] = None
    b1_ln_fused: Optional[torch.Tensor] = None
    ln_eps: float = 0.0


def ff_fused_row_order(hidden: int) -> torch.Tensor:
    s_, a, g, h, c = torch.meshgrid(torch.arange(hidden // 32), torch.arange(2), torch.arange(4), torch.arange(2), torch.arange(4),
                                    indexing="ij")
    return ((g & 1) * hidden + 32 * s_ + 16 * a + 8 * (g >> 1) + 4 * h + c).reshape(-1)


def ff_fused_k_perm(hidden: int) -> torch.Tensor:
    s_, a, h, t, c = torch.meshgrid(torch.arange(hidden // 32), torch.arange(2), torch.arange(2), torch.arange(2), torch.arange(4),
                                    indexing="ij")
    return (32 * s_ + 16 * a + 8 * t + 4 * h + c).reshape(-1)


def ff_dma_tile_index(rows: int, cols: int, slab_rows: int, slab_cols: int) -> torch.Tensor:
    assert rows % slab_rows == 0 and cols % slab_cols == 0 and slab_rows % 16 == 0 and slab_cols % 32 == 0
    idx = []
    swz = torch.tensor([0, 2, 3, 1])
    r16, pp, e = torch.meshgrid(torch.arange(16), torch.arange(4), torch.arange(8), indexing="ij")
    chunk = pp ^ swz[(r16 >> 2) & 3]
    piece = r16 * cols + chunk * 8 + e
    for sr in range(rows // slab_rows):
        for sc in range(cols // slab_cols):
            for cb in range(slab_cols // 32):
                for rb in range(slab_rows // 16):
                    idx.append(((sr * slab_rows + rb * 16) * cols + sc * slab_cols + cb * 32) + piece.reshape(-1))
    return torch.cat(idx)


def ff_fused_pack(w1: torch.Tensor, b1: torch.Tensor, w2: torch.Tensor, ln=None):
    hidden = w2.shape[-1]
    C = w1.shape[1]
    if ln is not None:
        w1f = w1.detach().float()
        b1 = b1.detach().float() + w1f @ ln[1].detach().float()
        w1 = w1f * ln[0].detach().float()[None, :]
    ro = ff_fused_row_order(hidden).to(w1.device)
    w1p = w1[ro]
    w2p = w2.reshape(-1, hidden)[:, ff_fused_k_perm(hidden).to(w2.device)]
    t1 = ff_dma_tile_index(2 * hidden, C, 64, C).to(w1.device)
    t2 = ff_dma_tile_index(C, hidden, C, 32).to(w2.device)
    return (_bf(w1p.reshape(-1)[t1].reshape(2 * hidden, C)), _f(b1[ro]), _bf(w2p.reshape(-1)[t2].reshape(C, hidden)))


def ln_proj_pack(w: torch.Tensor, gamma: torch.Tensor, beta: torch.Tensor):
    N, C = w.shape
    wf = w.detach().float()
    wg = wf * gamma.detach().float()[None, :]
    return (_bf(wg.reshape(-1)[ff_dma_tile_index(N, C, 64, C).to(w.device)].reshape(N, C)), _f(wf @ beta.detach().float()))


@dataclass
class SVTPack:
    C: int
    heads: int
    norm: tuple
    proj_in: tuple
    proj_out: tuple
    s_norm1: tuple = None
    s_wqk: torch.Tensor = None
    s_wv: torch.Tensor = None
    s_wo: tuple = None
    s_ctx_off: int = 0
    s_norm3: tuple = None
    s_ff: FFPack = None
    t_norm_in: tuple = None
    t_ff_in: FFPack = None
    t_norm1: tuple = None
    t_wqkv: torch.Tensor = None
    s_wqkv_fused: Optional[tuple] = None
    t_wqkv_fused: Optional[tuple] = None
    t_wo: tuple = None
    t_ctx_off: int = 0
    s_attn2: object = None
    s_norm2: object = None
    t_attn2: object = None
# ... 12 lines not shown
    device: torch.device
    in_channels: int
    in_pad: int
    model_channels: int
    out_channels: int
    context_dim: int
    adm_in: Optional[int]
    time_embed: tuple
    label_emb: Optional[tuple]
    conv_in: tuple
    input_stages: List[list]
    middle: list
    output_stages: List[list]
    out_norm: tuple
    out_conv: tuple
    emb_w: torch.Tensor
    emb_b: torch.Tensor
    ctx_w: torch.Tensor
    ctx_b: torch.Tensor
    mix_alpha: torch.Tensor
    mix_kind: torch.Tensor
    uses_ioi: bool
    conv_in_gemm: Optional[tuple] = None
    out_conv_taps: Optional[tuple] = None


def _pack_ff(ff, norm=None) -> FFPack:
    w1, b1 = pack_geglu(ff.net[0].proj)
    w2, b2 = pack_linear(ff.net[2])
    p = FFPack(w1, b1, w2, b2)
    C, hidden = w2.shape[-2], w2.shape[-1]
    if C == 320 and hidden % 64 == 0 and hidden >= 128:
        lin1, lin2 = ff.net[0].proj, ff.net[2]
        p.w1_fused, p.b1_fused, p.w2_fused = ff_fused_pack(lin1.weight.detach(), lin1.bias.detach(), lin2.weight.detach())
        if norm is not None:
            p.w1_ln_fused, p.b1_ln_fused, _ = ff_fused_pack(lin1.weight.detach(), lin1.bias.detach(), lin2.weight.detach(),
                                                             ln=(norm.weight, norm.bias))
            p.ln_eps = float(norm.eps)
    return p


class _Collector:

    def __init__(self):
        self.emb_w, self.emb_b, self.emb_cols = [], [], 0
        self.ctx_w, self.ctx_b, self.ctx_cols = [], [], 0
        self.alphas, self.kinds = [], []

    def add_emb(self, lin: nn.Linear) -> int:
        off = self.emb_cols
        self.emb_w.append(lin.weight.detach().float())
        self.emb_b.append(lin.bias.detach().float())
        self.emb_cols += lin.weight.shape[0]
        return off

    def add_ctx(self, attn) -> int:
        off = self.ctx_cols
        wo, wv = attn.to_out[0].weight.detach().float(), attn.to_v.weight.detach().float()
        self.ctx_w.append(wo @ wv)
        self.ctx_b.append(attn.to_out[0].bias.detach().float())
        self.ctx_cols += wo.shape[0]
        return off

    def add_mixer(self, blender, kind: int) -> int:
        self.alphas.append(blender.alpha_value())
        self.kinds.append(kind)
        return len(self.alphas) - 1


def pack_resblock(rb, col: Optional[_Collector]) -> ResPack:
    p = ResPack(cin=rb.channels, cout=rb.out_channels, split=getattr(rb, "concat_split", None))
    p.gn1 = pack_norm(rb.in_layers[0])
    p.w1, p.b1 = pack_conv3x3(rb.in_layers[2])
    p.gn2 = pack_norm(rb.out_layers[0])
    p.w2, p.b2 = pack_conv3x3(rb.out_layers[3])
    if not isinstance(rb.skip_connection, nn.Identity):
        p.skip_w, p.skip_b = pack_conv1x1(rb.skip_connection)
    if rb.emb_layers is not None:
        p.emb_off = col.add_emb(rb.emb_layers[1])
    ts = rb.time_stack
    p.t_gn1 = pack_norm(ts.in_layers[0])
    p.t_w1, p.t_b1 = pack_convt3(ts.in_layers[2])
    p.t_gn2 = pack_norm(ts.out_layers[0])
    p.t_w2, p.t_b2 = pack_convt3(ts.out_layers[3])
    if ts.emb_layers is not None:
        p.t_emb_off = col.add_emb(ts.emb_layers[1])
    p.mixer = col.add_mixer(rb.time_mixer, 0)
    return p


def pack_svt(st, col: _Collector) -> SVTPack:
    assert len(st.transformer_blocks) == 1 and len(st.time_stack) == 1, "transformer_depth > 1 is not used by V3D/SVD"
    blk, tb = st.transformer_blocks[0], st.time_stack[0]
    C = st.proj_in.weight.shape[0]
    p = SVTPack(C=C, heads=st.n_heads, norm=pack_norm(st.norm), proj_in=pack_linear(st.proj_in), proj_out=pack_linear(st.proj_out))
    assert st.d_head == 64, "attention kernels are specialised for d_head = 64"
    p.s_norm1 = pack_norm(blk.norm1)
    p.s_wqk = _bf(torch.cat([blk.attn1.to_q.weight.detach(), blk.attn1.to_k.weight.detach()], dim=0))
    p.s_wv = _bf(blk.attn1.to_v.weight)
    if C == 320:
        p.s_wqkv_fused = ln_proj_pack(torch.cat([blk.attn1.to_q.weight, blk.attn1.to_k.weight, blk.attn1.to_v.weight], dim=0), blk.norm1.weight, blk.norm1.bias)
        p.t_wqkv_fused = ln_proj_pack(torch.cat([tb.attn1.to_q.weight, tb.attn1.to_k.weight, tb.attn1.to_v.weight], dim=0), tb.norm1.weight, tb.norm1.bias)
    p.s_wo = pack_linear(blk.attn1.to_out[0])
    p.s_ctx_off = col.add_ctx(blk.attn2)
    p.s_attn2, p.s_norm2 = blk.attn2, blk.norm2
    p.s_norm3 = pack_norm(blk.norm3)
    p.s_ff = _pack_ff(blk.ff, blk.norm3)
    assert tb.ff_in is not False and tb.is_res
    p.t_norm_in = pack_norm(tb.norm_in)
    p.t_ff_in = _pack_ff(tb.ff_in)
    p.t_norm1 = pack_norm(tb.norm1)
    p.t_wqkv = _bf(torch.cat([tb.attn1.to_q.weight.detach(), tb.attn1.to_k.weight.detach(), tb.attn1.to_v.weight.detach()], dim=0))
    p.t_wo = pack_linear(tb.attn1.to_out[0])
    assert tb.attn2 is not None, "disable_temporal_crossattention is not used by V3D/SVD"
    p.t_ctx_off = col.add_ctx(tb.attn2)
    p.t_attn2, p.t_norm2 = tb.attn2, tb.norm2
    p.t_norm3 = pack_norm(tb.norm3)
    p.t_ff = _pack_ff(tb.ff, tb.norm3)
    p.tpe = pack_linear(st.time_pos_embed[0]) + pack_linear(st.time_pos_embed[2])
    p.max_period = float(st.max_time_embed_period)
    p.mixer = col.add_mixer(st.time_mixer, 1)
    return p


def cross_attn_pack(p: SVTPack, which: str):
    if which not in p.x2:
        if torch.cuda.is_available() and torch.cuda.is_current_stream_capturing():
            raise RuntimeError("cross_attn_pack: first multi-token cross-attention evaluation inside a HIP-graph capture; run one eager evaluation before capturing")
        attn, norm = (p.s_attn2, p.s_norm2) if which == "s" else (p.t_attn2, p.t_norm2)
        wq = _bf(attn.to_q.weight)
        wkv = _bf(torch.cat([attn.to_k.weight.detach(), attn.to_v.weight.detach()], dim=0))
        p.x2[which] = (pack_norm(norm), wq, wkv) + pack_linear(attn.to_out[0])
    return p.x2[which]


def pack_unet(net) -> UNetPack:
    from ..sgm.modules.diffusionmodules.openaimodel import Downsample, Upsample
    from ..sgm.modules.diffusionmodules.video_model import VideoResBlock
    from ..sgm.modules.video_attention import SpatialVideoTransformer

    col = _Collector()
    dev = net.out[2].weight.device

    def pack_stage(seq) -> list:
        items = []
        for m in seq:
            if isinstance(m, VideoResBlock):
                items.append(("res", pack_resblock(m, col)))
            elif isinstance(m, SpatialVideoTransformer):
                items.append(("svt", pack_svt(m, col)))
            elif isinstance(m, Downsample):
                items.append(("down", pack_conv3x3(m.op)))
            elif isinstance(m, Upsample):
                items.append(("up", pack_conv3x3(m.conv)))
            elif isinstance(m, nn.Conv2d):
                items.append(("conv_in", pack_conv3x3(m)))
            else:
                raise TypeError(f"unsupported U-Net stage member {type(m).__name__}")
        return items

    input_stages = [pack_stage(seq) for seq in net.input_blocks]
    middle = pack_stage(net.middle_block)
    output_stages = [pack_stage(seq) for seq in net.output_blocks]
    conv_in = input_stages[0][0][1]
    te = net.time_embed
    time_embed = pack_linear(te[0]) + pack_linear(te[2])
    label = None
    adm_in = None
    if net.num_classes == "sequential":
        le = net.label_emb[0]
        adm_in = le[0].weight.shape[1]
        label = pack_linear(le[0], k_pad=round_up(adm_in, 8)) + pack_linear(le[2])
    uses_ioi = net.merge_strategy == "learned_with_images"
    return UNetPack(
        device=dev, in_channels=net.in_channels, in_pad=round_up(net.in_channels, 8), model_channels=net.model_channels,
        out_channels=net.out_channels, context_dim=net.context_dim, adm_in=adm_in, time_embed=time_embed, label_emb=label,
        conv_in=conv_in, input_stages=input_stages, middle=middle, output_stages=output_stages,
        out_norm=pack_norm(net.out[0]), out_conv=pack_conv3x3(net.out[2]),
        conv_in_gemm=pack_conv3x3_im2col(net.input_blocks[0][0]) if net.in_channels <= 8 else None,
        out_conv_taps=pack_conv3x3_taps(net.out[2]) if 9 * net.out_channels <= 64 else None,
        emb_w=_bf(torch.cat(col.emb_w, 0)), emb_b=_f(torch.cat(col.emb_b, 0)),
        ctx_w=_bf(torch.cat(col.ctx_w, 0)), ctx_b=_f(torch.cat(col.ctx_b, 0)),
        mix_alpha=torch.tensor(col.alphas, dtype=F32, device=dev), mix_kind=torch.tensor(col.kinds, dtype=torch.int32, device=dev),
        uses_ioi=uses_ioi)


@dataclass
class AttnPack:
    C: int
    norm: tuple
    wq: tuple
    wk: tuple
    wv: torch.Tensor
    bv: torch.Tensor
    proj: tuple


@dataclass
class VAEPack:
    device: torch.device
    z_channels: int
    z_pad: int
    conv_in: tuple
    mid: list
    up: List[dict]
    norm_out: tuple
    conv_out: tuple
    tmix_w: torch.Tensor
    tmix_b: torch.Tensor
    out_ch: int


def pack_vae_resblock(rb) -> ResPack:
    p = ResPack(cin=rb.in_channels, cout=rb.out_channels, split=None)
    p.gn1 = pack_norm(rb.norm1)
    p.w1, p.b1 = pack_conv3x3(rb.conv1)
    p.gn2 = pack_norm(rb.norm2)
    p.w2, p.b2 = pack_conv3x3(rb.conv2)
    if rb.in_channels != rb.out_channels:
        p.skip_w, p.skip_b = pack_conv1x1(rb.nin_shortcut)
    ts = rb.time_stack
    p.t_gn1 = pack_norm(ts.in_layers[0])
    p.t_w1, p.t_b1 = pack_convt3(ts.in_layers[2])
    p.t_gn2 = pack_norm(ts.out_layers[0])
    p.t_w2, p.t_b2 = pack_convt3(ts.out_layers[3])
    m = float(rb.mix_factor.detach().float().cpu())
    p.alpha = m if rb.merge_strategy == "fixed" else float(torch.sigmoid(torch.tensor(m)))
    return p


def pack_vae_decoder(dec) -> VAEPack:
    dev = dec.conv_in.weight.device
    a = dec.mid.attn_1
    wv, bv = pack_conv1x1(a.v)
    attn = AttnPack(C=a.in_channels, norm=pack_norm(a.norm), wq=pack_conv1x1(a.q), wk=pack_conv1x1(a.k), wv=wv, bv=bv,
                    proj=pack_conv1x1(a.proj_out))
    mid = [("res", pack_vae_resblock(dec.mid.block_1)), ("attn", attn), ("res", pack_vae_resblock(dec.mid.block_2))]
    up = []
    for lvl in dec.up:
        d = {"blocks": [pack_vae_resblock(b) for b in lvl.block], "upsample": None}
        if hasattr(lvl, "upsample"):
            d["upsample"] = pack_conv3x3(lvl.upsample.conv)
        up.append(d)
    co = dec.conv_out
    tw = co.time_mix_conv.weight.detach()
    return VAEPack(device=dev, z_channels=dec.conv_in.weight.shape[1], z_pad=round_up(dec.conv_in.weight.shape[1], 8),
                   conv_in=pack_conv3x3(dec.conv_in), mid=mid, up=up, norm_out=pack_norm(dec.norm_out),
                   conv_out=pack_conv3x3(co), tmix_w=_f(tw.reshape(tw.shape[0], tw.shape[1], 3)), tmix_b=_f(co.time_mix_conv.bias),
                   out_ch=co.weight.shape[0])



@dataclass
class VAEEncPack:
    device: torch.device
    in_ch: int
    in_pad: int
    conv_in: tuple
    down: List[dict]
    mid: list
    norm_out: tuple
    conv_out: tuple
    out_ch: int


def pack_resnet2d(rb) -> ResPack:
    p = ResPack(cin=rb.in_channels, cout=rb.out_channels, split=None)
    p.gn1 = pack_norm(rb.norm1)
    p.w1, p.b1 = pack_conv3x3(rb.conv1)
    p.gn2 = pack_norm(rb.norm2)
    p.w2, p.b2 = pack_conv3x3(rb.conv2)
    if rb.in_channels != rb.out_channels:
        p.skip_w, p.skip_b = pack_conv1x1(rb.nin_shortcut)
    return p


def _pack_attnblock(a) -> AttnPack:
    wv, bv = pack_conv1x1(a.v)
    return AttnPack(C=a.in_channels, norm=pack_norm(a.norm), wq=pack_conv1x1(a.q), wk=pack_conv1x1(a.k), wv=wv, bv=bv,
                    proj=pack_conv1x1(a.proj_out))


def pack_vae_encoder(enc) -> VAEEncPack:
    down = []
    for lvl in enc.down:
        d = {"blocks": [pack_resnet2d(b) for b in lvl.block], "attn": [_pack_attnblock(a) for a in lvl.attn], "downsample": None}
        if hasattr(lvl, "downsample"):
            d["downsample"] = pack_conv3x3(lvl.downsample.conv)
        down.append(d)
    mid = [("res", pack_resnet2d(enc.mid.block_1)), ("attn", _pack_attnblock(enc.mid.attn_1)), ("res", pack_resnet2d(enc.mid.block_2))]
    cin = enc.conv_in.weight.shape[1]
    return VAEEncPack(device=enc.conv_in.weight.device, in_ch=cin, in_pad=round_up(cin, 8), conv_in=pack_conv3x3(enc.conv_in), down=down,
                      mid=mid, norm_out=pack_norm(enc.norm_out), conv_out=pack_conv3x3(enc.conv_out), out_ch=enc.conv_out.weight.shape[0])
```

v3d_amd/engine/unet.py:

```python
from __future__ import annotations

import os

from typing import Optional

import torch

from ..ops import GemmCall, get_ops
from .blocks import Env, Geo, unet_resblock
from .packing import SVTPack, UNetPack, cross_attn_pack, round_up

BF, F32 = torch.bfloat16, torch.float32


def _cast_rows_bf16(ops, x2d: torch.Tensor, pad_to: int = 0) -> torch.Tensor:
    n, C = x2d.shape
    return ops.nchw_to_nhwc_bf16(x2d.float().contiguous().reshape(n, C, 1), 1.0, max(pad_to, round_up(C, 8)))


def frame_pos_table(ops, p: SVTPack, B: int, frame_ids) -> torch.Tensor:
    key = (B, tuple(frame_ids))
    tab = p.tables.get(key)
    if tab is None:
        dev = p.proj_in[0].device
# ... 46 lines not shown
        ops.layernorm(x, ga, be, n1, eps)
        qk = ops.linear(n1, p.s_wqk)
        vT = ops.empty((n, C, S), ops.act_dtype, x.device) if S % 8 == 0 else ops.empty((n, C, -(-S // 8) * 8), ops.act_dtype, x.device)[..., :S]
        ops.gemm(GemmCall(A=p.s_wv, W=n1.view(n, S, C), out=vT, M=C, N=S, K=C, batch=n))
    a = ops.empty((n * S, C), ops.act_dtype, x.device)
    if os.environ.get("V3D_ATTN_FP8", "0") not in ("", "0") and hasattr(ops, "attn_spatial_fp8") and S % 16 == 0:
        qk8, qk_scales = ops.quant_fp8_tiles(qk, n, S)
        v8, v_scale = ops.quant_fp8_slab(vT, p.heads)
        ops.attn_spatial_fp8(qk8, qk_scales, v8, v_scale, a, n, S, p.heads, 0.125)
    else:
        ops.attn_spatial(qk[:, :C], qk[:, C:], vT, a, n, S, p.heads, 0.125)
    multi = env.ctx_tok is not None
    if multi:
        x = ops.linear(a, p.s_wo[0], p.s_wo[1], res1=x)
        x = cross_attention(ops, x, cross_attn_pack(p, "s"), env.ctx_tok, env.n_ctx, p.heads)
    else:
        x = ops.linear(a, p.s_wo[0], p.s_wo[1], res1=x, add=ctx[:, p.s_ctx_off:], add_rpg=S, add_ld=ctx_ld)
    x_s = feed_forward(ops, x, p.s_ff, res1=x, ln=p.s_norm3)

    frames = range(T) if sh is None else sh.local_frames
    table = frame_pos_table(ops, p, B, frames)
    ga, be, eps = p.t_norm_in
    x_mix = ops.empty((n * S, C), ops.act_dtype, x.device)
    nin = ops.empty((n * S, C), ops.act_dtype, x.device)
    ops.layernorm(x_s, ga, be, nin, eps, add=table, add_rpg=S, add_ld=C, xsum_out=x_mix)
    x_t = feed_forward(ops, nin, p.t_ff_in, res1=x_mix)
    ga, be, eps = p.t_norm1
    ta = ops.empty((B, T, S, C), ops.act_dtype, x.device)
    if sh is None and ln_proj:
        qkv = ops.ln_proj(x_t, eps, p.t_wqkv_fused[0], p.t_wqkv_fused[1], 3 * C, S)[0].view(B, T, S, 3 * C)
        ops.attn_temporal(qkv[..., :C], qkv[..., C:2 * C], qkv[..., 2 * C:], ta, p.heads, 0.125)
    elif sh is None:
        n1 = ops.empty((n * S, C), ops.act_dtype, x.device) if n1 is None else n1
        ops.layernorm(x_t, ga, be, n1, eps)
        qkv = ops.linear(n1, p.t_wqkv).view(B, T, S, 3 * C)
        ops.attn_temporal(qkv[..., :C], qkv[..., C:2 * C], qkv[..., 2 * C:], ta, p.heads, 0.125)
    else:
        n1 = ops.empty((n * S, C), ops.act_dtype, x.device) if n1 is None else n1
        ops.layernorm(x_t, ga, be, n1, eps)
        kv_loc = ops.linear(n1, p.t_wqkv[C:]).view(B, T, S, 2 * C)
        kv, pending = sh.allgather_frames(kv_loc, async_op=True)
        q = ops.linear(n1, p.t_wqkv[:C]).view(B, T, S, C)
        pending.wait()
        ops.attn_temporal(q, kv[..., :C], kv[..., C:], ta, p.heads, 0.125)
    if multi:
        x_t = ops.linear(ta.view(n * S, C), p.t_wo[0], p.t_wo[1], res1=x_t)
        x_t = cross_attention(ops, x_t, cross_attn_pack(p, "t"), env.ctx0_tok, env.n_ctx, p.heads)
    else:
        x_t = ops.linear(ta.view(n * S, C), p.t_wo[0], p.t_wo[1], res1=x_t, add=ctx[n:, p.t_ctx_off:], add_rpg=S * T,
                         add_ld=ctx_ld)
    x = feed_forward(ops, x_t, p.t_ff, res1=x_t, res2=x_s, coef=env.coefs[p.mixer], coef_rpg=S, ln=p.t_norm3)
    return ops.linear(x, p.proj_out[0], p.proj_out[1], res1=x_in)


_FF_FUSED = os.environ.get("V3D_FF_FUSED", "1") not in ("", "0")
_LN_FF = os.environ.get("V3D_LN_FF", "1") not in ("", "0")


def feed_forward(ops, xin, ff, *, res1, res2=None, coef=None, coef_rpg=0, ln=None):
    M, C = xin.shape
    kw = dict(res1=res1)
    if res2 is not None:
        kw.update(res2=res2, coef=coef, coef_rpg=coef_rpg)
    fused = _FF_FUSED and ff.w2_fused is not None and M % 128 == 0 and hasattr(ops, "ff_fused")
    if ln is not None:
        if fused and _LN_FF and ff.w1_ln_fused is not None and hasattr(ops, "ln_ff_fused"):
            out = ops.empty((M, C), ops.act_dtype, xin.device)
            return ops.ln_ff_fused(xin, ff.ln_eps, ff.w1_ln_fused, ff.b1_ln_fused, ff.w2_fused, ff.b2, out, **kw)
        ga, be, eps = ln
        normed = ops.empty((M, C), ops.act_dtype, xin.device)
        ops.layernorm(xin, ga, be, normed, eps)
        xin = normed
    if fused:
        out = ops.empty((M, C), ops.act_dtype, xin.device)
        return ops.ff_fused(xin, ff.w1_fused, ff.b1_fused, ff.w2_fused, ff.b2, out, **kw)
    f = ops.linear(xin, ff.w1, ff.b1, geglu=True)
    return ops.linear(f, ff.w2, ff.b2, **kw)


def run_unet(pk: UNetPack, x, scale, concat, timesteps, context, y, num_video_frames, image_only_indicator, shard=None,
             context_frame0=None):
    ops = get_ops()
    n, _, H, W = x.shape
    ops.begin_evaluation(x.device)
    T = int(num_video_frames) if num_video_frames is not None else 1
    if shard is None:
        from ..dist import active_shard
        shard = active_shard()
    if shard is not None:
        T = shard.T_local
        if context_frame0 is None:
            context_frame0 = shard.context_frame0
        assert context_frame0 is not None, "frame-sharded evaluation needs the context of each sample's global frame 0 (FrameShard.activate)"
    assert n % T == 0, f"batch {n} is not a multiple of num_video_frames {T}"
    B = n // T
    dev = x.device
    mc = pk.model_channels

    te = ops.timestep_embedding(timesteps.reshape(-1).float().contiguous(), mc)
    w0, b0, w2, b2 = pk.time_embed
    e = ops.linear(ops.silu_add(ops.linear(te, w0, b0, out_dtype=F32)), w2, b2, out_dtype=F32)
    lab = None
    if pk.label_emb is not None:
        w0, b0, w2, b2 = pk.label_emb
        yb = _cast_rows_bf16(ops, y.reshape(n, -1), w0.shape[1])
        lab = ops.linear(ops.silu_add(ops.linear(yb, w0, b0, out_dtype=F32)), w2, b2, out_dtype=F32)
    semb = ops.silu_add(e, lab)
    emb_all = ops.linear(semb, pk.emb_w, pk.emb_b, out_dtype=F32)
    assert context is not None and context.dim() == 3 and context.shape[0] == n and 1 <= context.shape[1] <= 32, \
        f"context must be [n={n}, N, context_dim] with 1 <= N <= 32 tokens per image (V3D / SVD condition on one), got {None if context is None else tuple(context.shape)}"
    n_ctx = context.shape[1]
    ctx_all = ctx_tok = ctx0_tok = None
    if n_ctx == 1:
        c2 = context.reshape(n, -1)
        c0 = c2[::T] if context_frame0 is None else context_frame0.reshape(B, -1)
        cb = _cast_rows_bf16(ops, torch.cat([c2, c0.to(c2.dtype)], dim=0))
        ctx_all = ops.linear(cb, pk.ctx_w, pk.ctx_b, out_dtype=F32)
    else:
        assert shard is None, "frame-sharded evaluation supports one context token per image"
        c0 = context[::T] if context_frame0 is None else context_frame0.reshape(B, n_ctx, -1)
        both = _cast_rows_bf16(ops, torch.cat([context.reshape(n * n_ctx, -1), c0.reshape(B * n_ctx, -1).to(context.dtype)], dim=0))
        ctx_tok, ctx0_tok = both[:n * n_ctx], both[n * n_ctx:]
    ioi = None
    assert not pk.uses_ioi or image_only_indicator is not None, "image_only_indicator is required by merge_strategy='learned_with_images'"
    if pk.uses_ioi and image_only_indicator is not None:
        ioi = image_only_indicator
        if shard is not None and ioi.numel() == B * shard.T_global:
            ioi = ioi.reshape(B, shard.T_global)[:, shard.t0:shard.t0 + T]
        ioi = ioi.reshape(-1).float().contiguous()
        assert ioi.numel() == n, f"image_only_indicator has {ioi.numel()} entries for {n} images"
    coefs = ops.blend_coefs(pk.mix_alpha, pk.mix_kind, ioi, n)
    env = Env(ops=ops, emb_all=emb_all, ctx_all=ctx_all, coefs=coefs, shard=shard, ctx_tok=ctx_tok, ctx0_tok=ctx0_tok, n_ctx=n_ctx)

    in_gemm = pk.conv_in_gemm is not None and x.dim() == 4 and os.environ.get("V3D_CONV_IO_GEMM", "1") != "0"
    if in_gemm:
        h = ops.pack_input_im2col3x3(x.float().contiguous(), scale, None if concat is None else concat.float().contiguous(), pk.conv_in_gemm[0].shape[-1])
    else:
        h = ops.pack_input(x.float().contiguous(), scale, None if concat is None else concat.float().contiguous(), pk.in_pad)
    g = Geo(n=n, B=B, T=T, H=H, W=W)

    def run_stage(items, h, g, skip=None):
        for kind, p in items:
            if kind == "conv_in":
                h = ops.linear(h, pk.conv_in_gemm[0], pk.conv_in_gemm[1]) if in_gemm else ops.conv3x3(h, p[0], p[1], g.n, g.H, g.W)
            elif kind == "res":
                h = unet_resblock(env, g, p, h, skip)
                skip = None
            elif kind == "svt":
                h = run_svt(env, g, p, h)
            elif kind == "down":
                h = ops.conv3x3(h, p[0], p[1], g.n, g.H, g.W, stride=2)
                g = Geo(n=g.n, B=g.B, T=g.T, H=(g.H + 1) // 2, W=(g.W + 1) // 2)
            elif kind == "up":
                h = ops.conv3x3(h, p[0], p[1], g.n, g.H, g.W, up=2)
                g = Geo(n=g.n, B=g.B, T=g.T, H=g.H * 2, W=g.W * 2)
            else:
                raise ValueError(kind)
        return h, g

    hs = []
    for items in pk.input_stages:
        h, g = run_stage(items, h, g)
        hs.append(h)
    h, g = run_stage(pk.middle, h, g)
    for items in pk.output_stages:
        h, g = run_stage(items, h, g, skip=hs.pop())
    ga, be, eps = pk.out_norm
    h = ops.groupnorm(h, None, ga, be, g.n, g.S, eps=eps, silu=True)
    if pk.out_conv_taps is not None and os.environ.get("V3D_CONV_IO_GEMM", "1") != "0":
        y = ops.linear(h, pk.out_conv_taps[0], None, out_dtype=F32)
        out = ops.tapsum3x3(y, pk.out_conv_taps[1], g.n, g.H, g.W, pk.out_channels)
    else:
        out = ops.conv3x3(h, pk.out_conv[0], pk.out_conv[1], g.n, g.H, g.W, out_dtype=F32)
    return out.view(n, g.H, g.W, pk.out_channels).permute(0, 3, 1, 2)
```

v3d_amd/engine/vae.py:

```python
from __future__ import annotations

import torch

from ..ops import GemmCall, get_ops
from .blocks import Env, Geo, res_spatial, vae_resblock
from .packing import AttnPack, VAEEncPack, VAEPack

F32 = torch.float32


def run_vae_attn(env: Env, g: Geo, p: AttnPack, x: torch.Tensor) -> torch.Tensor:
    ops = env.ops
    n, S, C = g.n, g.S, p.C
    ga, be, eps = p.norm
    hn = ops.groupnorm(x, None, ga, be, n, S, eps=eps, silu=False)
    q = ops.linear(hn, *p.wq)
    k = ops.linear(hn, *p.wk)
    vT = ops.empty((n, C, S), None, x.device)
    ops.gemm(GemmCall(A=p.wv, W=hn.view(n, S, C), out=vT, M=C, N=S, K=C, batch=n))
    if C in getattr(ops, "ATTN_VAE_WIDTHS", ()) and S % 8 == 0:
        o = ops.empty((n * S, C), None, x.device)
        ops.attn_vae(q, k, vT, p.bv, o, n, S, C, float(C) ** -0.5)
        return ops.linear(o, p.proj[0], p.proj[1], res1=x)
    scores = ops.empty((n, S, S), F32, x.device)
    ops.gemm(GemmCall(A=q.view(n, S, C), W=k.view(n, S, C), out=scores, M=S, N=S, K=C, batch=n, c_acc=float(C) ** -0.5))
    prob = ops.empty((n, S, S), None, x.device)
    ops.softmax_rows(scores, prob)
    o = ops.empty((n, S, C), None, x.device)
    ops.gemm(GemmCall(A=prob, W=vT, out=o, M=S, N=C, K=S, batch=n, bias=p.bv))
    return ops.linear(o.view(n * S, C), p.proj[0], p.proj[1], res1=x)


def run_decoder(pk: VAEPack, z: torch.Tensor, T: int, shard=None) -> torch.Tensor:
    ops = get_ops()
    n, _, H, W = z.shape
    ops.begin_evaluation(z.device)
    if shard is None:
        from ..dist import active_shard
        shard = active_shard()
    if shard is not None:
        if n % shard.T_local != 0:
            raise ValueError(f"frame-sharded decode: {n} latent frames is not a multiple of this rank's {shard.T_local} frames "
                             "(chunked decode_first_stage is not defined under a FrameShard: decode all local frames in one call)")
        T = shard.T_local
    assert n % T == 0, f"{n} latent frames is not a multiple of timesteps={T}"
    env = Env(ops=ops, shard=shard)
    g = Geo(n=n, B=n // T, T=T, H=H, W=W)
    h = ops.nchw_to_nhwc_bf16(z.float().contiguous(), 1.0, pk.z_pad)
    h = ops.conv3x3(h, pk.conv_in[0], pk.conv_in[1], n, H, W)
    for kind, p in pk.mid:
        h = vae_resblock(env, g, p, h) if kind == "res" else run_vae_attn(env, g, p, h)
    for lvl in reversed(range(len(pk.up))):
        for p in pk.up[lvl]["blocks"]:
            h = vae_resblock(env, g, p, h)
        us = pk.up[lvl]["upsample"]
        if us is not None:
            h = ops.conv3x3(h, us[0], us[1], g.n, g.H, g.W, up=2)
            g = Geo(n=g.n, B=g.B, T=g.T, H=g.H * 2, W=g.W * 2)
    ga, be, eps = pk.norm_out
    h = ops.groupnorm(h, None, ga, be, g.n, g.S, eps=eps, silu=True)
    y = ops.empty((g.n * g.S, 4), F32, z.device)
    ops.conv3x3(h, pk.conv_out[0], pk.conv_out[1], g.n, g.H, g.W, out=y[:, :pk.out_ch])
    if shard is None:
        out = ops.tmix_small(y, pk.tmix_w, pk.tmix_b, g.B, g.T, g.S, pk.out_ch, 0, g.T - 1)
    else:
        out = shard.tmix_small(ops, y, pk.tmix_w, pk.tmix_b, g, pk.out_ch)
    return out.view(g.n, pk.out_ch, g.H, g.W)


def run_encoder(pk: VAEEncPack, x: torch.Tensor) -> torch.Tensor:
    ops = get_ops()
    n, _, H, W = x.shape
    ops.begin_evaluation(x.device)
    env = Env(ops=ops, shard=None)
    g = Geo(n=n, B=n, T=1, H=H, W=W)
    h = ops.nchw_to_nhwc_bf16(x.float().contiguous(), 1.0, pk.in_pad)
    h = ops.conv3x3(h, pk.conv_in[0], pk.conv_in[1], n, H, W)
    for lvl in pk.down:
        for i, p in enumerate(lvl["blocks"]):
            h = res_spatial(env, g, p, h, None)
            if lvl["attn"]:
                h = run_vae_attn(env, g, lvl["attn"][i], h)
        ds = lvl["downsample"]
        if ds is not None:
            assert g.H % 2 == 0 and g.W % 2 == 0, "VAE Downsample expects even feature maps"
            h = ops.conv3x3(h, ds[0], ds[1], g.n, g.H, g.W, stride=2, pad_mode=1)
            g = Geo(n=g.n, B=g.B, T=1, H=g.H // 2, W=g.W // 2)
    for kind, p in pk.mid:
        h = res_spatial(env, g, p, h, None) if kind == "res" else run_vae_attn(env, g, p, h)
    ga, be, eps = pk.norm_out
    h = ops.groupnorm(h, None, ga, be, g.n, g.S, eps=eps, silu=True)
    y = ops.conv3x3(h, pk.conv_out[0], pk.conv_out[1], g.n, g.H, g.W, out_dtype=F32)
    return y.view(g.n, g.H, g.W, pk.out_ch).permute(0, 3, 1, 2).contiguous()
```

v3d_amd/hip.py:

```python
from __future__ import annotations

import ctypes as C
import os
from typing import Optional

import torch

from .ops import GemmCall, OpsBase

_HERE = os.path.dirname(os.path.abspath(__file__))
LIB_PATH = os.environ.get("V3D_HIP_LIB") or os.path.join(_HERE, "lib", "libv3d_hip.so")

ABI_VERSION = 9

c_i64, c_i32, c_f32, c_f64, c_vp = C.c_int64, C.c_int32, C.c_float, C.c_double, C.c_void_p


class _GemmArgs(C.Structure):
    _fields_ = [
        ("A", c_vp), ("W", c_vp), ("out", c_vp), ("bias", c_vp), ("add", c_vp), ("res1", c_vp), ("res2", c_vp),
        ("coef", c_vp),
        ("M", c_i64), ("N", c_i64), ("K", c_i64),
        ("lda", c_i64), ("ldw", c_i64), ("ldo", c_i64), ("ldr1", c_i64), ("ldr2", c_i64),
        ("a_rows", c_i64), ("a_row0", c_i64),
        ("add_rpg", c_i64), ("add_ld", c_i64), ("coef_rpg", c_i64),
        ("c_acc", c_f32), ("c_res1", c_f32), ("c_res2", c_f32),
        ("mode", c_i32), ("geglu", c_i32), ("out_fp32", c_i32),
        ("Hin", c_i32), ("Win", c_i32), ("Hout", c_i32), ("Wout", c_i32), ("stride", c_i32), ("up", c_i32),
        ("T", c_i32), ("tmin", c_i32), ("tmax", c_i32),
        ("S", c_i64),
        ("batch", c_i32), ("pad_mode", c_i32),
        ("sA", c_i64), ("sW", c_i64), ("sO", c_i64),
        ("halo_rows", c_i64),
        ("gn_stats", c_vp), ("gn_rps", c_i64), ("gn_cpg", c_i32), ("gn_in_silu", c_i32),
        ("gn_nslots", c_i64),
        ("gn_in_table", c_vp), ("gn_in_rps", c_i64), ("gn_in_rows", c_i64),
        ("A2", c_vp), ("K1", c_i64), ("lda2", c_i64),
    ]


class GsCamera(C.Structure):
    _fields_ = [("view", c_f32 * 16), ("proj", c_f32 * 16), ("tanfovx", c_f32), ("tanfovy", c_f32), ("bg", c_f32 * 3),
                ("width", c_i32), ("height", c_i32)]


_CAM = C.POINTER(GsCamera)

SIGNATURES = {
    "v3d_abi_version": (c_i32, []),
    "v3d_last_error": (C.c_char_p, []),
    "v3d_device_info": (c_i32, [c_vp]),
    "v3d_gemm": (c_i32, [C.POINTER(_GemmArgs), c_vp]),
    "v3d_sizeof_gemm_args": (c_i32, []),
    "v3d_ff_fused": (c_i32, [c_vp, c_i64, c_vp, c_vp, c_vp, c_vp, c_vp, c_i64, c_vp, c_i64, c_vp, c_i64, c_f32, c_f32, c_f32,
                             c_vp, c_i64, c_i64, c_i32, c_i32, c_vp]),
    "v3d_ln_ff_fused": (c_i32, [c_vp, c_i64, c_f32, c_vp, c_vp, c_vp, c_vp, c_vp, c_i64, c_vp, c_i64, c_vp, c_i64, c_f32, c_f32, c_f32,
                                c_vp, c_i64, c_i64, c_i32, c_i32, c_vp]),
    "v3d_ln_proj": (c_i32, [c_vp, c_i64, c_f32, c_vp, c_vp, c_vp, c_i64, c_vp, c_i64, c_i32, c_i32, c_i32, c_i64, c_vp]),
    "v3d_gemm_gn_in_supported": (c_i32, [C.POINTER(_GemmArgs)]),
    "v3d_groupnorm_stats": (c_i32, [c_vp, c_i64, c_vp, c_i64, c_vp, c_i64, c_i64, c_i64, c_i32, c_i64, c_vp]),
    "v3d_groupnorm_stats_table": (c_i32, [c_vp, c_i64, c_vp, c_i64, c_vp, c_i64, c_vp, c_i64, c_i64, c_i32, c_i64, c_vp, c_vp, C.c_double, C.c_float, c_vp, c_vp]),
    "v3d_groupnorm_finalize": (c_i32, [c_vp, c_i64, c_vp, c_i64, c_i32, c_vp, c_vp, c_i64, c_f64, c_f32, c_vp, c_vp]),
    "v3d_groupnorm_apply": (c_i32, [c_vp, c_i64, c_vp, c_i64, c_vp, c_vp, c_i64, c_i64, c_i64, c_i32, c_vp]),
    "v3d_groupnorm_small_supported": (c_i32, [c_i64, c_i64, c_i64, c_i32, c_i64]),
    "v3d_groupnorm_small": (c_i32, [c_vp, c_i64, c_vp, c_i64, c_vp, c_vp, c_vp, c_i64, c_i64, c_i32, c_i64, c_f32, c_i32, c_vp]),
    "v3d_layernorm": (c_i32, [c_vp, c_vp, c_i64, c_i64, c_vp, c_vp, c_vp, c_vp, c_i64, c_i64, c_f32, c_vp]),
    "v3d_attn_spatial": (c_i32, [c_vp, c_i64, c_vp, c_i64, c_vp, c_vp, c_i64, c_i64, c_i64, c_i32, c_f32, c_vp]),
    "v3d_attn_spatial_ld": (c_i32, [c_vp, c_i64, c_vp, c_i64, c_vp, c_i64, c_vp, c_i64, c_i64, c_i64, c_i32, c_f32, c_vp]),
    "v3d_attn_temporal": (c_i32, [c_vp, c_i64, c_i64, c_i64, c_vp, c_vp, c_i64, c_i64, c_i64, c_vp, c_i64, c_i64,
                                  c_i64, c_i64, c_i32, c_i32, c_i64, c_i32, c_f32, c_vp]),
    "v3d_attn_vae_d512": (c_i32, [c_vp, c_i64, c_vp, c_i64, c_vp, c_vp, c_vp, c_i64, c_i64, c_i64, c_i32, c_f32, c_vp]),
    "v3d_quant_fp8_tiles": (c_i32, [c_vp, c_i64, c_vp, c_i64, c_vp, c_i64, c_i64, c_i32, c_vp]),
    "v3d_quant_fp8_slab": (c_i32, [c_vp, c_vp, c_vp, c_vp, c_i64, c_i64, c_i32, c_vp]),
    "v3d_attn_spatial_fp8": (c_i32, [c_vp, c_i64, c_vp, c_vp, c_vp, c_vp, c_i64, c_i64, c_i64, c_i32, c_f32, c_vp]),
    "v3d_softmax_rows": (c_i32, [c_vp, c_vp, c_i64, c_i64, c_vp]),
    "v3d_timestep_embedding": (c_i32, [c_vp, c_vp, c_i64, c_i32, c_f32, c_vp]),
    "v3d_silu_add": (c_i32, [c_vp, c_vp, c_vp, c_i64, c_vp]),
    "v3d_edm_scalings": (c_i32, [c_vp, c_vp, c_vp, c_vp, c_vp, c_i64, c_vp]),
    "v3d_pack_input": (c_i32, [c_vp, c_vp, c_i64, c_vp, c_i64, c_vp, c_i64, c_i64, c_i64, c_vp]),
    "v3d_pack_input_im2col3x3": (c_i32, [c_vp, c_vp, c_i64, c_vp, c_i64, c_vp, c_i64, c_i32, c_i32, c_i64, c_vp]),
    "v3d_tapsum3x3": (c_i32, [c_vp, c_i64, c_vp, c_vp, c_i64, c_i32, c_i32, c_i32, c_vp]),
    "v3d_denoise_combine": (c_i32, [c_vp, c_i64, c_vp, c_vp, c_vp, c_vp, c_i64, c_i64, c_i64, c_vp]),
    "v3d_cfg_combine": (c_i32, [c_vp, c_vp, c_vp, c_i64, c_i64, c_i64, c_vp]),
    "v3d_euler_step": (c_i32, [c_vp, c_vp, c_vp, c_vp, c_vp, c_i64, c_i64, c_vp]),
    "v3d_heun_step": (c_i32, [c_vp, c_vp, c_vp, c_vp, c_vp, c_vp, c_vp, c_i64, c_i64, c_vp]),
    "v3d_clip_preprocess": (c_i32, [c_vp, c_i64, c_i32, c_i32, c_i32, c_i32, c_i32, c_vp, c_vp, c_vp, c_i32, c_vp]),
    "v3d_gelu_bf16": (c_i32, [c_vp, c_vp, c_i64, c_vp]),
    "v3d_frames_to_uint8": (c_i32, [c_vp, c_vp, c_i64, c_i32, c_i64, c_vp]),
    "v3d_axpb_f32": (c_i32, [c_vp, c_f32, c_f32, c_vp, c_i64, c_vp]),
    "v3d_blend_coefs": (c_i32, [c_vp, c_vp, c_vp, c_vp, c_i64, c_i64, c_vp]),
    "v3d_nchw_to_nhwc_bf16": (c_i32, [c_vp, c_f32, c_vp, c_i64, c_i64, c_i64, c_i64, c_vp]),
    "v3d_tmix_small": (c_i32, [c_vp, c_i64, c_vp, c_vp, c_vp, c_i64, c_i32, c_i64, c_i32, c_i32, c_i32, c_i64, c_vp]),
    "v3d_copy2d_bf16": (c_i32, [c_vp, c_i64, c_vp, c_i64, c_i64, c_i64, c_vp]),
    "v3d_randn_add": (c_i32, [c_vp, c_f32, C.c_uint64, C.c_uint32, c_vp, c_i64, c_i64, c_i64, c_i64, c_i64, c_vp]),
    "v3d_lincomb_f32": (c_i32, [c_vp, c_vp, c_i32, c_vp, c_i64, c_vp]),
    "v3d_gs_knn3": (c_i32, [c_vp, c_i64, c_vp, c_vp]),
    "v3d_gs_preprocess_fwd": (c_i32, [c_vp, c_vp, c_vp, c_vp, c_vp, c_i64, _CAM, c_vp, c_vp, c_vp, c_vp, c_vp, c_vp, c_vp, c_vp]),
    "v3d_gs_scan_work_bytes": (c_i64, [c_i64]),
    "v3d_gs_scan": (c_i32, [c_vp, c_i64, c_vp, c_vp, c_i64, c_vp]),
    "v3d_gs_duplicate_keys": (c_i32, [c_vp, c_vp, c_vp, c_vp, c_i64, c_i32, c_i32, c_vp, c_vp, c_vp]),
    "v3d_gs_sort_work_bytes": (c_i64, [c_i64]),
    "v3d_gs_radix_sort_pairs": (c_i32, [c_vp, c_vp, c_vp, c_vp, c_i64, c_i32, c_vp, c_i64, c_vp]),
    "v3d_gs_tile_ranges": (c_i32, [c_vp, c_vp, c_i64, c_vp, c_vp, c_vp, c_i32, c_i32, c_vp, c_vp, c_vp]),
    "v3d_gs_render_fwd": (c_i32, [c_vp, c_vp, c_vp, c_vp, c_vp, _CAM, c_vp, c_vp, c_vp, c_vp]),
    "v3d_gs_render_bwd": (c_i32, [c_vp, c_vp, c_vp, c_vp, c_vp, _CAM, c_vp, c_vp, c_vp, c_vp, c_vp]),
    "v3d_gs_reduce_instance_grads": (c_i32, [c_vp, c_vp, c_vp, c_i64, c_vp, c_vp]),
    "v3d_gs_preprocess_bwd": (c_i32, [c_vp, c_vp, c_vp, c_vp, c_i64, _CAM, c_vp, c_vp, c_vp, c_vp, c_vp, c_vp, c_vp, c_vp, c_vp, c_vp]),
    "v3d_gs_ssim_work_floats": (c_i64, [c_i32, c_i32, c_i32]),
    "v3d_gs_ssim_l1_fwd": (c_i32, [c_vp, c_vp, c_i32, c_i32, c_i32, c_f32, c_vp, c_i64, c_vp, c_vp]),
    "v3d_gs_ssim_l1_bwd": (c_i32, [c_vp, c_vp, c_i32, c_i32, c_i32, c_f32, c_vp, c_i64, c_vp, c_vp, c_vp]),
}


def load_library(path: str = LIB_PATH) -> C.CDLL:
    if not os.path.exists(path):
        raise RuntimeError(
            f"{path} not found: the HIP extension is not built. Run `python -c 'import __graft_entry__ as g; g.build()'` "
            "(or `python -m v3d_amd.build`). There is no CPU fallback for the V3D hot path.")
    lib = C.CDLL(path)
    for name, (res, args) in SIGNATURES.items():
        fn = getattr(lib, name)
        fn.restype = res
        fn.argtypes = args
    v = lib.v3d_abi_version()
    if v != ABI_VERSION:
        raise RuntimeError(f"libv3d_hip.so ABI version {v} != expected {ABI_VERSION}; rebuild the extension")
    if lib.v3d_sizeof_gemm_args() != C.sizeof(_GemmArgs):
        raise RuntimeError(f"v3d_gemm_args layout mismatch: library {lib.v3d_sizeof_gemm_args()} B vs binding {C.sizeof(_GemmArgs)} B")
    return lib


def _ptr(t: Optional[torch.Tensor]):
    return None if t is None else t.data_ptr()


class HipOps(OpsBase):
    name = "hip"

    def __init__(self, device: Optional[torch.device] = None, lib_path: Optional[str] = None):
        self.lib = load_library(lib_path or LIB_PATH)
        if not torch.cuda.is_available():
            raise RuntimeError("v3d_amd: no HIP device visible (torch.cuda.is_available() is False); the V3D hot path "
                               "has no CPU fallback")
        self.device = torch.device("cuda", torch.cuda.current_device()) if device is None else torch.device(device)
        info = (c_i32 * 4)()
        self._check(self.lib.v3d_device_info(C.cast(info, c_vp)), "v3d_device_info")
        self.cu_count, self.lds_bytes, self.wave_size, self.arch = info[0], info[1], info[2], info[3]
        if self.wave_size != 64:
            raise RuntimeError(f"v3d_amd kernels are wave64 gfx950 code; device reports wave size {self.wave_size}")

    def streamk_timeouts(self) -> int:
        fn = self.lib.v3d_debug_sk_timeouts
        fn.restype, fn.argtypes = C.c_longlong, []
        return int(fn())

    def last_gemm_launch(self) -> dict:
        fn = self.lib.v3d_debug_last_gemm_launch
        fn.restype, fn.argtypes = c_i32, [c_vp]
        o = (C.c_longlong * 8)()
        fn(C.cast(o, c_vp))
        fam, bm, bn, tiles, bpc, sk, tail, cus = (int(v) for v in o)
        slots = max(1, bpc) * max(1, cus)
        tiles_eff = tiles * max(1, sk)
        fill = 1.0 if tail else tiles_eff / (-(-tiles_eff // slots) * slots) if tiles_eff else 0.0
        return {"family": fam, "bm": bm, "bn": bn, "tiles": tiles, "blocks_per_cu": bpc, "splitk": sk, "streamk_tail": tail, "cus": cus, "fill": fill}

    def gemm_plan(self, g: GemmCall) -> dict:
        fn = self.lib.v3d_debug_gemm_plan
        fn.restype, fn.argtypes = c_i32, [C.POINTER(_GemmArgs), c_i32, c_vp, c_vp]
        o = (C.c_longlong * 10)()
        a = self._gemm_args(g)
        self._check(fn(C.byref(a), self.cu_count, None, C.cast(o, c_vp)), "v3d_debug_gemm_plan")
        kid, fam, bm, bn, tiles, grid, sk, tail, gn, _ = (int(v) for v in o)
        return {"kernel": kid, "family": fam, "bm": bm, "bn": bn, "tiles": tiles, "grid": grid, "splitk": sk, "streamk_tail": tail, "gn_in_epilogue": bool(gn)}

    def check_health(self):
        n = self.streamk_timeouts()
        if n:
            raise RuntimeError(f"v3d_amd: {n} stream-K hand-off(s) timed out in this process (a donor block was not co-resident): results of the "
                               "affected launches are wrong; rerun with V3D_STREAMK=0 and report the configuration")

    def _check(self, rc: int, what: str):
        if rc != 0:
            msg = self.lib.v3d_last_error()
            raise RuntimeError(f"{what} failed (rc={rc}): {msg.decode() if msg else ''}")

    @staticmethod
    def _stream():
        return torch.cuda.current_stream().cuda_stream

    @staticmethod
    def _req(t: torch.Tensor, dtype, what: str, inner_contig: bool = True):
        if t.device.type != "cuda":
            raise RuntimeError(f"{what}: tensor is on {t.device}, HIP ops need device memory")
        if t.dtype != dtype:
            raise RuntimeError(f"{what}: dtype {t.dtype} != {dtype}")
        if inner_contig and t.dim() > 0 and t.stride(-1) != 1 and t.shape[-1] != 1:
            raise RuntimeError(f"{what}: inner stride must be 1")
        return t

    @staticmethod
    def _req_c(t: torch.Tensor, dtype, what: str):
        HipOps._req(t, dtype, what)
        if not t.is_contiguous():
            raise RuntimeError(f"{what}: tensor must be contiguous")
        return t

    _MAX_OPERAND_BYTES = 0xFFFFFF00

    def _gemm_in_row_chunks(self, g: GemmCall) -> bool:
        import dataclasses
        import math
        if g.batch != 1 or g.mode == 2 or g.A.dim() != 2:
            return False
        lda = g.A.stride(0)
        rows_in = g.A.shape[0]
        if rows_in * lda * 2 <= self._MAX_OPERAND_BYTES:
            return False
        if g.mode == 1:
            s_out, s_in = g.Hout * g.Wout, g.Hin * g.Win
        else:
            s_out = s_in = 1
        align = 1
        for rpg in (g.add_rpg if g.add is not None else 0, g.coef_rpg if g.coef is not None else 0, g.gn_rps if g.gn_stats is not None else 0):
            if rpg:
                align = align * rpg // math.gcd(align, rpg)
        unit_out = s_out * align // math.gcd(s_out, align)
        unit_in = unit_out // s_out * s_in
        units = g.M // unit_out
        if units * unit_out != g.M:
            raise RuntimeError("gemm: operand larger than 4 GiB and M is not a whole number of images / row groups")
        per = max(1, int((self._MAX_OPERAND_BYTES // 2) // (unit_in * lda * 2)))
        for u0 in range(0, units, per):
            u1 = min(units, u0 + per)
            r0, r1 = u0 * unit_out, u1 * unit_out
            kw = dict(A=g.A[u0 * unit_in:u1 * unit_in], out=g.out[r0:r1], M=r1 - r0, a_rows=0)
            if g.res1 is not None:
                kw["res1"] = g.res1[r0:r1]
            if g.res2 is not None:
                kw["res2"] = g.res2[r0:r1]
            if g.add is not None:
                kw["add"] = g.add[r0 // g.add_rpg:]
            if g.coef is not None:
                kw["coef"] = g.coef.reshape(-1, 3)[r0 // g.coef_rpg:].contiguous()
            if g.gn_stats is not None:
                kw["gn_stats"] = g.gn_stats[r0 // g.gn_rps:]
            if g.gn_in is not None:
                raise RuntimeError("gemm: gn_in is not defined for operands beyond one buffer descriptor (normalise with groupnorm_apply first)")
            self.gemm(dataclasses.replace(g, **kw))
        return True

    def _gemm_args(self, g: GemmCall) -> _GemmArgs:
        bf, f32 = torch.bfloat16, torch.float32
        a = _GemmArgs()
        self._req(g.A, bf, "gemm.A")
        self._req(g.W, bf, "gemm.W")
        ldw = g.W.stride(-2)
        if g.W.dim() == 3 and g.mode != 0 and g.W.stride(0) != g.N * ldw:
            raise RuntimeError("gemm.W: taps must be densely stacked")
        out_fp32 = g.out.dtype == f32
        self._req(g.out, f32 if out_fp32 else bf, "gemm.out")
        a.A, a.W, a.out = g.A.data_ptr(), g.W.data_ptr(), g.out.data_ptr()
        a.bias = _ptr(None if g.bias is None else self._req_c(g.bias, f32, "gemm.bias"))
        a.add = _ptr(None if g.add is None else self._req(g.add, f32, "gemm.add"))
        a.res1 = _ptr(None if g.res1 is None else self._req(g.res1, bf, "gemm.res1"))
        a.res2 = _ptr(None if g.res2 is None else self._req(g.res2, bf, "gemm.res2"))
        a.coef = _ptr(None if g.coef is None else self._req_c(g.coef, f32, "gemm.coef"))
        a.M, a.N, a.K = g.M, g.N, g.K
        a.lda = g.A.stride(-2) if g.A.dim() >= 2 else g.K
        a.ldw = ldw
        a.ldo = g.out.stride(-2)
        a.ldr1 = 0 if g.res1 is None else g.res1.stride(-2)
        a.ldr2 = 0 if g.res2 is None else g.res2.stride(-2)
        a.a_rows = g.a_rows if g.a_rows else g.A.shape[-2]
        a.a_row0 = g.a_row0
        a.add_rpg, a.add_ld, a.coef_rpg = g.add_rpg, g.add_ld, g.coef_rpg
        a.c_acc, a.c_res1, a.c_res2 = g.c_acc, g.c_res1, g.c_res2
        a.mode, a.geglu, a.out_fp32 = g.mode, int(g.geglu), int(out_fp32)
        a.Hin, a.Win, a.Hout, a.Wout, a.stride, a.up = g.Hin, g.Win, g.Hout, g.Wout, g.stride, g.up
        a.T, a.tmin, a.tmax, a.S = g.T, g.tmin, g.tmax, g.S
        a.batch = g.batch
        a.pad_mode = g.pad_mode
        a.halo_rows = g.halo_rows
        if g.gn_stats is not None:
            self._req_c(g.gn_stats, f32, "gemm.gn_stats")
            a.gn_stats, a.gn_rps, a.gn_cpg, a.gn_nslots = g.gn_stats.data_ptr(), g.gn_rps, g.gn_cpg, g.gn_stats.shape[1]
        if g.gn_in is not None:
            self._req_c(g.gn_in, f32, "gemm.gn_in")
            a.gn_in_table, a.gn_in_rps, a.gn_in_rows, a.gn_in_silu = g.gn_in.data_ptr(), g.gn_in_rps, g.gn_in.shape[0], int(g.gn_in_silu)
        if g.A2 is not None:
            self._req(g.A2, bf, "gemm.A2")
            a.A2, a.K1, a.lda2 = g.A2.data_ptr(), g.A.shape[-1], g.A2.stride(-2)
        if g.batch > 1:
            if g.mode != 0:
                raise RuntimeError("gemm: batching is only defined for LINEAR mode")
            a.sA = g.A.stride(0) if g.A.dim() == 3 else 0
            a.sW = g.W.stride(0) if g.W.dim() == 3 else 0
            a.sO = g.out.stride(0) if g.out.dim() == 3 else 0
            if g.out.dim() != 3:
                raise RuntimeError("gemm: batched out must be 3-D")
        return a

    def gemm(self, g: GemmCall):
        if self._gemm_in_row_chunks(g):
            return
        a = self._gemm_args(g)
        self._check(self.lib.v3d_gemm(C.byref(a), self._stream()), "v3d_gemm")

    def gemm_gn_in_supported(self, g: GemmCall) -> bool:
        if g.gn_in is None or g.A.dim() != 2 or g.A.shape[0] * g.A.stride(0) * 2 > self._MAX_OPERAND_BYTES:
            return False
        a = self._gemm_args(g)
        return bool(self.lib.v3d_gemm_gn_in_supported(C.byref(a)))

    def groupnorm_stats(self, x1, x2, stats, n_img, S, groups, imgs_per_stat):
        bf = torch.bfloat16
        self._req_c(x1, bf, "gn.x1")
        if x2 is not None:
            self._req_c(x2, bf, "gn.x2")
        self._req_c(stats, torch.float32, "gn.stats")
        self._check(self.lib.v3d_groupnorm_stats(x1.data_ptr(), x1.shape[-1], _ptr(x2), 0 if x2 is None else x2.shape[-1],
                                                 stats.data_ptr(), stats.shape[1], n_img, S, groups, imgs_per_stat, self._stream()),
                    "v3d_groupnorm_stats")

    def groupnorm_stats_table(self, x1, x2, stats, tickets, n_img, S, groups, imgs_per_stat, gamma, beta, count, eps, table):
        bf, f32 = torch.bfloat16, torch.float32
        self._req_c(x1, bf, "gn.x1")
        if x2 is not None:
            self._req_c(x2, bf, "gn.x2")
        self._req_c(stats, f32, "gn.stats"); self._req_c(gamma, f32, "gn.gamma"); self._req_c(beta, f32, "gn.beta"); self._req_c(table, f32, "gn.table")
        if tickets.dtype != torch.int32 or tickets.numel() < n_img // imgs_per_stat or not tickets.is_contiguous():
            raise ValueError("gn.tickets: need a contiguous int32 tensor with one (zero) entry per statistics group")
        self._check(self.lib.v3d_groupnorm_stats_table(x1.data_ptr(), x1.shape[-1], _ptr(x2), 0 if x2 is None else x2.shape[-1], stats.data_ptr(), stats.shape[1],
                                                       tickets.data_ptr(), n_img, S, groups, imgs_per_stat, gamma.data_ptr(), beta.data_ptr(), float(count), float(eps),
                                                       table.data_ptr(), self._stream()), "v3d_groupnorm_stats_table")

    def groupnorm_finalize(self, stats, sums, gamma, beta, count, eps, table):
        f32 = torch.float32
        if stats is not None:
            self._req_c(stats, f32, "gn.stats")
        if sums is not None:
            self._req_c(sums, torch.float64, "gn.sums")
        ref = stats if stats is not None else sums
        n_stat, groups = ref.shape[0], ref.shape[-2]
        Cc = 0
        if table is not None:
            self._req_c(gamma, f32, "gn.gamma"); self._req_c(beta, f32, "gn.beta"); self._req_c(table, f32, "gn.table")
            Cc = gamma.numel()
        self._check(self.lib.v3d_groupnorm_finalize(_ptr(stats), 0 if stats is None else stats.shape[1], _ptr(sums), n_stat, groups,
                                                    _ptr(gamma) if table is not None else None, _ptr(beta) if table is not None else None, Cc,
                                                    float(count), float(eps), _ptr(table), self._stream()), "v3d_groupnorm_finalize")

    def groupnorm_small_supported(self, C1, C2, S, imgs_per_stat=1, groups=32):
        return bool(self.lib.v3d_groupnorm_small_supported(C1, C2, S, groups, imgs_per_stat))

    def groupnorm_small(self, x1, x2, gamma, beta, out, n_img, S, *, eps, silu, imgs_per_stat=1, groups=32):
        bf = torch.bfloat16
        self._req(x1, bf, "gns.x1"); self._req_c(gamma, torch.float32, "gns.gamma"); self._req_c(beta, torch.float32, "gns.beta"); self._req_c(out, bf, "gns.out")
        C1, C2 = x1.shape[-1], 0
        assert x1.stride(-1) == 1 and x1.stride(0) == C1
        if x2 is not None:
            self._req(x2, bf, "gns.x2")
            C2 = x2.shape[-1]
            assert x2.stride(-1) == 1 and x2.stride(0) == C2
        self._check(self.lib.v3d_groupnorm_small(x1.data_ptr(), C1, _ptr(x2), C2, gamma.data_ptr(), beta.data_ptr(), out.data_ptr(), n_img, S, groups,
                                                 imgs_per_stat, eps, int(silu), self._stream()), "v3d_groupnorm_small")
        return out

    def groupnorm_apply(self, x1, x2, table, out, n_img, S, imgs_per_stat, silu):
        bf, f32 = torch.bfloat16, torch.float32
        self._req_c(x1, bf, "gn.x1")
        if x2 is not None:
            self._req_c(x2, bf, "gn.x2")
        self._req_c(table, f32, "gn.table")
        self._req_c(out, bf, "gn.out")
        self._check(self.lib.v3d_groupnorm_apply(x1.data_ptr(), x1.shape[-1], _ptr(x2), 0 if x2 is None else x2.shape[-1],
                                                 table.data_ptr(), out.data_ptr(), n_img, S, imgs_per_stat, int(silu),
                                                 self._stream()), "v3d_groupnorm_apply")

    def layernorm(self, x, gamma, beta, out, eps, add=None, add_rpg=0, add_ld=0, xsum_out=None):
        bf, f32 = torch.bfloat16, torch.float32
        self._req_c(x, bf, "ln.x"); self._req_c(out, bf, "ln.out")
        self._req_c(gamma, f32, "ln.gamma"); self._req_c(beta, f32, "ln.beta")
        if add is not None:
            self._req(add, f32, "ln.add")
        if xsum_out is not None:
            self._req_c(xsum_out, bf, "ln.xsum_out")
        M, Cc = x.numel() // x.shape[-1], x.shape[-1]
        self._check(self.lib.v3d_layernorm(x.data_ptr(), _ptr(add), add_rpg, add_ld, _ptr(xsum_out), gamma.data_ptr(),
                                           beta.data_ptr(), out.data_ptr(), M, Cc, float(eps), self._stream()), "v3d_layernorm")

    def attn_spatial(self, q, k, vT, out, n_img, S, heads, scale, ldv=None):
        bf = torch.bfloat16
        self._req(q, bf, "attn.q"); self._req(k, bf, "attn.k"); self._req(out, bf, "attn.out")
        self._req(vT, bf, "attn.vT")
        if ldv is None:
            ldv = vT.stride(-2) if vT.dim() >= 2 else S
        C = heads * 64
        if vT.dim() == 3 and (vT.shape[-1] != S or vT.stride(0) != C * ldv or vT.stride(1) != ldv):
            raise RuntimeError(f"attn.vT: expected [n_img, {C}, {S}] rows at stride {ldv}, got shape {tuple(vT.shape)} strides {vT.stride()}")
        if ldv == S and S % 8 == 0:
            self._req_c(vT, bf, "attn.vT")
            self._check(self.lib.v3d_attn_spatial(q.data_ptr(), q.stride(-2), k.data_ptr(), k.stride(-2), vT.data_ptr(),
                                                  out.data_ptr(), out.stride(-2), n_img, S, heads, float(scale), self._stream()),
                        "v3d_attn_spatial")
            return
        self._check(self.lib.v3d_attn_spatial_ld(q.data_ptr(), q.stride(-2), k.data_ptr(), k.stride(-2), vT.data_ptr(), ldv,
                                                 out.data_ptr(), out.stride(-2), n_img, S, heads, float(scale), self._stream()),
                    "v3d_attn_spatial_ld")

    def attn_temporal(self, q, k, v, out, heads, scale):
        bf = torch.bfloat16
        for t, nm in ((q, "q"), (k, "k"), (v, "v"), (out, "out")):
            self._req(t, bf, f"tattn.{nm}")
        B, Tq, S, _ = q.shape
        Tk = k.shape[1]
        assert k.stride()[:3] == v.stride()[:3], "k and v must share strides"
        self._check(self.lib.v3d_attn_temporal(q.data_ptr(), q.stride(0), q.stride(1), q.stride(2),
                                               k.data_ptr(), v.data_ptr(), k.stride(0), k.stride(1), k.stride(2),
                                               out.data_ptr(), out.stride(0), out.stride(1), out.stride(2),
                                               B, Tq, Tk, S, heads, float(scale), self._stream()), "v3d_attn_temporal")

    ATTN_VAE_WIDTHS = (128, 256, 512)

    def attn_vae(self, q, k, vT, bias, out, n_img, S, C, scale):
        bf = torch.bfloat16
        self._req(q, bf, "attn_vae.q"); self._req(k, bf, "attn_vae.k"); self._req_c(vT, bf, "attn_vae.vT"); self._req(out, bf, "attn_vae.out")
        if bias is not None:
            self._req_c(bias, torch.float32, "attn_vae.bias")
        self._check(self.lib.v3d_attn_vae_d512(q.data_ptr(), q.stride(-2), k.data_ptr(), k.stride(-2), vT.data_ptr(), _ptr(bias), out.data_ptr(),
                                               out.stride(-2), n_img, S, C, float(scale), self._stream()), "v3d_attn_vae_d512")

    def quant_fp8_tiles(self, x, n_img, S):
        self._req(x, torch.bfloat16, "quant_fp8_tiles.x")
        ncols = x.shape[-1]
        x8 = torch.empty((n_img * S, ncols), dtype=torch.uint8, device=x.device)
        scales = torch.empty((n_img, (S + 63) // 64, ncols // 64), dtype=torch.float32, device=x.device)
        self._check(self.lib.v3d_quant_fp8_tiles(x.data_ptr(), x.stride(-2), x8.data_ptr(), ncols, scales.data_ptr(), n_img, S, ncols, self._stream()),
                    "v3d_quant_fp8_tiles")
        return x8, scales

    def quant_fp8_slab(self, vT, heads):
        self._req_c(vT, torch.bfloat16, "quant_fp8_slab.vT")
        n_img, _, S = vT.shape
        v8 = torch.empty(vT.shape, dtype=torch.uint8, device=vT.device)
        vscale = torch.empty((n_img, heads), dtype=torch.float32, device=vT.device)
        scratch = torch.empty((n_img, heads), dtype=torch.int32, device=vT.device)
        self._check(self.lib.v3d_quant_fp8_slab(vT.data_ptr(), v8.data_ptr(), vscale.data_ptr(), scratch.data_ptr(), n_img, S, heads, self._stream()),
                    "v3d_quant_fp8_slab")
        return v8, vscale

    def attn_spatial_fp8(self, qk8, scales, v8, vscale, out, n_img, S, heads, scale):
        self._req_c(qk8, torch.uint8, "attn_fp8.qk8"); self._req_c(v8, torch.uint8, "attn_fp8.v8")
        self._req_c(scales, torch.float32, "attn_fp8.scales"); self._req_c(vscale, torch.float32, "attn_fp8.vscale")
        self._req(out, torch.bfloat16, "attn_fp8.out")
        self._check(self.lib.v3d_attn_spatial_fp8(qk8.data_ptr(), qk8.stride(-2), scales.data_ptr(), v8.data_ptr(), vscale.data_ptr(), out.data_ptr(),
                                                  out.stride(-2), n_img, S, heads, float(scale), self._stream()), "v3d_attn_spatial_fp8")

    def softmax_rows(self, inp, out):
        self._req_c(inp, torch.float32, "softmax.in"); self._req_c(out, torch.bfloat16, "softmax.out")
        L = inp.shape[-1]
        self._check(self.lib.v3d_softmax_rows(inp.data_ptr(), out.data_ptr(), inp.numel() // L, L, self._stream()), "v3d_softmax_rows")

    def timestep_embedding(self, t, dim, max_period=10000.0):
        self._req_c(t, torch.float32, "temb.t")
        out = self.empty((t.numel(), dim), torch.bfloat16, t.device)
        self._check(self.lib.v3d_timestep_embedding(t.data_ptr(), out.data_ptr(), t.numel(), dim, float(max_period), self._stream()),
# ... 364 lines not shown
```

v3d_amd/ops.py:

```python
from __future__ import annotations

import os

import contextlib
import dataclasses
from typing import Optional

import torch

GEMM_LINEAR, GEMM_CONV3X3, GEMM_CONVT3 = 0, 1, 2


@dataclasses.dataclass
class GemmCall:
    A: torch.Tensor
    W: torch.Tensor
    out: torch.Tensor
    M: int
    N: int
    K: int
    bias: Optional[torch.Tensor] = None
    add: Optional[torch.Tensor] = None
    add_rpg: int = 0
    add_ld: int = 0
    res1: Optional[torch.Tensor] = None
    res2: Optional[torch.Tensor] = None
    coef: Optional[torch.Tensor] = None
    coef_rpg: int = 0
    c_acc: float = 1.0
    c_res1: float = 1.0
    c_res2: float = 1.0
    mode: int = GEMM_LINEAR
    geglu: bool = False
    Hin: int = 0
    Win: int = 0
    Hout: int = 0
    Wout: int = 0
    stride: int = 1
    up: int = 1
    pad_mode: int = 0
    T: int = 0
    S: int = 0
    tmin: int = 0
    tmax: int = 0
    a_row0: int = 0
    a_rows: int = 0
    batch: int = 1
    halo_rows: int = 0
    gn_stats: Optional[torch.Tensor] = None
    gn_rps: int = 0
    gn_cpg: int = 0
    gn_in: Optional[torch.Tensor] = None
    gn_in_rps: int = 0
    gn_in_silu: bool = True
    A2: Optional[torch.Tensor] = None


class OpsBase:

    name = "base"
    act_dtype = torch.bfloat16

    def empty(self, shape, dtype=None, device=None):
        return torch.empty(shape, dtype=dtype or self.act_dtype, device=device if device is not None else self.device)

    def zeros(self, shape, dtype=torch.float32, device=None):
        return torch.zeros(shape, dtype=dtype, device=device if device is not None else self.device)

    _ZERO_ARENA_FLOATS = 32 << 20

    def begin_evaluation(self, device):
        key = str(device)
        arenas = self.__dict__.setdefault("_zero_arenas", {})
        arena = arenas.get(key)
        if arena is None:
            return
        if torch.device(device).type == "cuda" and torch.cuda.is_current_stream_capturing():
            arena[0].zero_()
        elif arena[1] > 0:
            arena[0][:arena[1]].zero_()
        arena[1] = 0

    def zeros_f32_pooled(self, shape, device):
        n = 1
        for d in shape:
            n *= int(d)
        key = str(device)
        arenas = self.__dict__.setdefault("_zero_arenas", {})
        arena = arenas.get(key)
        if arena is None or arena[1] + n > arena[0].numel():
            if torch.device(device).type == "cuda" and torch.cuda.is_current_stream_capturing():
                return torch.zeros(shape, dtype=torch.float32, device=device)
            grown = max(n, self._ZERO_ARENA_FLOATS, 0 if arena is None else 2 * arena[0].numel())
            if arena is not None:
                self.__dict__.setdefault("_retired_arenas", []).append(arena[0])
            arena = [torch.zeros(grown, dtype=torch.float32, device=device), 0]
            arenas[key] = arena
        t = arena[0][arena[1]:arena[1] + n].view(shape)
        arena[1] += (n + 63) // 64 * 64
        return t

    @staticmethod
    def gn_nslots(rps, imgs_per_stat=1):
        return max(8 * imgs_per_stat, rps // 64 + 2)

    def gn_stats_buffer(self, n_stat, device, groups=32, *, rps, imgs_per_stat=1):
        return self.zeros_f32_pooled((n_stat, self.gn_nslots(rps, imgs_per_stat), groups, 2), device)

    def linear(self, x2d, w, bias=None, *, out=None, out_dtype=None, geglu=False, **epi):
        M, K = x2d.shape
        N = w.shape[-2]
        n_out = N // 2 if geglu else N
        if out is None:
            out = self.empty((M, n_out), out_dtype or self.act_dtype, x2d.device)
        self.gemm(GemmCall(A=x2d, W=w, out=out, M=M, N=N, K=K, bias=bias, geglu=geglu, **epi))
        return out

    def conv3x3(self, x, w, bias, n_img, Hin, Win, *, stride=1, up=1, pad_mode=0, out=None, out_dtype=None, **epi):
        Hl, Wl = Hin * up, Win * up
        ptot = 1 if pad_mode else 2
        Hout, Wout = (Hl + ptot - 3) // stride + 1, (Wl + ptot - 3) // stride + 1
        K = x.shape[-1]
        N = w.shape[-2]
        M = n_img * Hout * Wout
        if out is None:
            out = self.empty((M, N), out_dtype or self.act_dtype, x.device)
        self.gemm(GemmCall(A=x, W=w, out=out, M=M, N=N, K=K, bias=bias, mode=GEMM_CONV3X3, Hin=Hin, Win=Win,
                           Hout=Hout, Wout=Wout, stride=stride, up=up, pad_mode=pad_mode, **epi))
        return out

    def convt3(self, x, w, bias, T, S, *, tmin=0, tmax=None, a_row0=0, M=None, out=None, out_dtype=None, halo_rows=0, **epi):
        K = x.shape[-1]
        N = w.shape[-2]
        if M is None:
            M = x.shape[0]
        if tmax is None:
            tmax = T - 1
        if out is None:
            out = self.empty((M, N), out_dtype or self.act_dtype, x.device)
        self.gemm(GemmCall(A=x, W=w, out=out, M=M, N=N, K=K, bias=bias, mode=GEMM_CONVT3, T=T, S=S, tmin=tmin,
                           tmax=tmax, a_row0=a_row0, halo_rows=halo_rows, **epi))
        return out

    def groupnorm_table(self, x1, x2, gamma, beta, n_img, S, *, eps, imgs_per_stat=1, groups=32, stats_hook=None, count_imgs=None, stats=None):
        C = x1.shape[-1] + (x2.shape[-1] if x2 is not None else 0)
        n_stat = n_img // imgs_per_stat
        if count_imgs is None:
            count_imgs = imgs_per_stat
        count = float(count_imgs) * S * (C // groups)
        table = self.empty((n_stat, C, 2), torch.float32, x1.device)
        if stats is None and stats_hook is None and self._GN_FUSED_TABLE and groups <= 32 and groups % 2 == 0 and hasattr(self, "groupnorm_stats_table"):
            stats = self.gn_stats_buffer(n_stat, x1.device, groups, rps=imgs_per_stat * S, imgs_per_stat=imgs_per_stat)
            tickets = self.zeros_f32_pooled((n_stat,), x1.device).view(torch.int32)
            self.groupnorm_stats_table(x1, x2, stats, tickets, n_img, S, groups, imgs_per_stat, gamma, beta, count, eps, table)
            return table
        if stats is None:
            stats = self.gn_stats_buffer(n_stat, x1.device, groups, rps=imgs_per_stat * S, imgs_per_stat=imgs_per_stat)
            self.groupnorm_stats(x1, x2, stats, n_img, S, groups, imgs_per_stat)
        if stats_hook is None:
            self.groupnorm_finalize(stats, None, gamma, beta, count, eps, table)
        else:
            sums = self.empty((n_stat, groups, 2), torch.float64, x1.device)
            self.groupnorm_finalize(stats, sums, None, None, count, eps, None)
            sums = stats_hook(sums)
            self.groupnorm_finalize(None, sums, gamma, beta, count, eps, table)
        return table

    def groupnorm(self, x1, x2, gamma, beta, n_img, S, *, eps, silu, imgs_per_stat=1, groups=32, stats_hook=None,
                  count_imgs=None, out=None, stats=None, table=None):
        C = x1.shape[-1] + (x2.shape[-1] if x2 is not None else 0)
        if out is None:
            out = self.empty((n_img * S, C), self.act_dtype, x1.device)
        if tuple(out.shape) != (n_img * S, C):
            raise ValueError(f"groupnorm: out has shape {tuple(out.shape)}, the normalised tensor is [{n_img * S}, {C}]")
        if (table is None and stats is None and stats_hook is None and (count_imgs is None or count_imgs == imgs_per_stat)
                and self.groupnorm_small_fits(x1, x2, S, imgs_per_stat, groups)):
            return self.groupnorm_small(x1, x2, gamma, beta, out, n_img, S, eps=eps, silu=silu, imgs_per_stat=imgs_per_stat, groups=groups)
        if table is None:
            table = self.groupnorm_table(x1, x2, gamma, beta, n_img, S, eps=eps, imgs_per_stat=imgs_per_stat, groups=groups,
                                         stats_hook=stats_hook, count_imgs=count_imgs, stats=stats)
        self.groupnorm_apply(x1, x2, table, out, n_img, S, imgs_per_stat, silu)
        return out

    _GN_FUSED_TABLE = os.environ.get("V3D_GN_FUSED_TABLE", "1") not in ("", "0")
    _GN_SMALL = os.environ.get("V3D_GN_SMALL", "1") not in ("", "0")

    def groupnorm_small_fits(self, x1, x2, S, imgs_per_stat=1, groups=32) -> bool:
        if not self._GN_SMALL or x1.stride(0) != x1.shape[-1] or (x2 is not None and x2.stride(0) != x2.shape[-1]):
            return False
        return self.groupnorm_small_supported(x1.shape[-1], 0 if x2 is None else x2.shape[-1], S, imgs_per_stat, groups)

    def groupnorm_small_supported(self, C1, C2, S, imgs_per_stat=1, groups=32) -> bool:
        return False

    def gemm_gn_in_supported(self, g: "GemmCall") -> bool:
        return False


_ACTIVE: Optional[OpsBase] = None
_DEFAULT: Optional[OpsBase] = None


def get_ops() -> OpsBase:
    global _DEFAULT
    if _ACTIVE is not None:
        return _ACTIVE
    if _DEFAULT is None:
        from .hip import HipOps
        _DEFAULT = HipOps()
    return _DEFAULT


@contextlib.contextmanager
def use_backend(ops: OpsBase):
    global _ACTIVE
    prev = _ACTIVE
    _ACTIVE = ops
    try:
        yield ops
    finally:
        _ACTIVE = prev
```

Baseline: 12.89 frames/s.

## Fold nearest-2x upsample into a 4-tap phase-decomposed conv3x3 GEMM

```diff
diff --git a/include/v3d_hip.h b/include/v3d_hip.h
--- a/include/v3d_hip.h
+++ b/include/v3d_hip.h
@@ -7,7 +7,7 @@
 extern "C" {
 #endif
 
-#define V3D_ABI_VERSION 9
+#define V3D_ABI_VERSION 10
 
 typedef void* v3d_stream_t;
 
@@ -21,7 +21,7 @@
 const char* v3d_last_error(void);
 int v3d_device_info(int32_t* out4);
 
-enum { V3D_GEMM_LINEAR = 0, V3D_GEMM_CONV3X3 = 1, V3D_GEMM_CONVT3 = 2 };
+enum { V3D_GEMM_LINEAR = 0, V3D_GEMM_CONV3X3 = 1, V3D_GEMM_CONVT3 = 2, V3D_GEMM_CONV3X3_UP2FOLD = 3 };
 
 typedef struct v3d_gemm_args {
     const void* A;
@@ -61,6 +61,7 @@
 
 int v3d_gemm(const v3d_gemm_args* args, v3d_stream_t stream);
 int v3d_gemm_gn_in_supported(const v3d_gemm_args* args);
+int v3d_gemm_up2_fold_supported(const v3d_gemm_args* args);
 
 int v3d_ff_fused(const void* x, int64_t ldx, const void* W1p, const float* b1, const void* W2p, const float* b2,
                  const void* res1, int64_t ldr1, const void* res2, int64_t ldr2, const float* coef, int64_t coef_rpg,
diff --git a/v3d_amd/csrc/gemm.hip b/v3d_amd/csrc/gemm.hip
--- a/v3d_amd/csrc/gemm.hip
+++ b/v3d_amd/csrc/gemm.hip
@@ -290,13 +290,14 @@
     unsigned voff[PPW];
     long long ld_n0 = 0;
     int ld_it = 0, ld_tap = 0, ld_k0 = 0;
+    int ld_phase = 0;
     auto set_tap = [&](int tap) __attribute__((always_inline)) {
 #pragma unroll
         for (int i = 0; i < PPW; ++i) {
             const int q = wave + NW * i;
             if (q < APIECES) {
                 long long s_;
-                const bool ok = ri[i].tap(p, tap, s_);
+                const bool ok = ri[i].tap(p, MODE == V3D_GEMM_CONV3X3_UP2FOLD ? fold_tap(tap, ld_phase) : tap, s_);
                 voff[i] = ok ? (unsigned)((s_ + p.a_row0) * p.lda * 2) + kchunk_b : kInvalid;
             } else {
                 const long long n = ld_n0 + (q - APIECES) * 16 + prow;
@@ -307,6 +308,7 @@
     auto set_tile = [&](int it) __attribute__((always_inline)) {
         long long m0;
         tile_origin(it, m0, ld_n0);
+        if constexpr (MODE == V3D_GEMM_CONV3X3_UP2FOLD) ld_phase = __builtin_amdgcn_readfirstlane((int)((unsigned)ld_n0 / (unsigned)p.up_cout));
 #pragma unroll
         for (int i = 0; i < PPW; ++i) {
             const int q = wave + NW * i;
@@ -403,7 +405,7 @@
                 E4GnRun<WM, MF> run;
                 if constexpr (GN) run.init(mw0, p.gn_rps);
                 auto flushfn = [&](int f, long long, unsigned& slot, unsigned& sid) __attribute__((always_inline)) -> bool { return run.step(f, slot, sid); };
-                e4_retire_tile<MF, NF, GN>(p, acc, nw0, lane_e, estage, rowfn, flushfn);
+                e4_retire_tile<MF, NF, GN, E4_ASM_READS, MODE == V3D_GEMM_CONV3X3_UP2FOLD>(p, acc, nw0, lane_e, estage, rowfn, flushfn);
             }
         } else
         {
@@ -709,6 +711,17 @@
     const int taps = mode == V3D_GEMM_LINEAR ? 1 : (mode == V3D_GEMM_CONV3X3 ? 9 : 3);
     const bool dma_ok = v3d_k_steps_ok(p);
 
+    if (mode == V3D_GEMM_CONV3X3_UP2FOLD) {
+        const long long cout = p.up_cout;
+        const bool w320 = cout % 320 == 0;
+        const int bm = w320 ? 192 : 256, bn = w320 ? 320 : 256;
+        const bool ok = pol.impl != 1 && pol.impl != 2 && batch == 1 && !geglu && dma_ok && cout > 0 && cout % bn == 0 && p.Wout >= 8 &&
+                        4 * p.M < (1ll << 32) && !p.add && !p.res1 && !p.res2 && !p.coef && !p.gn_stats && !p.gn_in && !p.A2 &&
+                        (w320 ? e4_ok(p, 96, 80) && v3_ok(p, 96, 80) : e4_ok(p, 128, 64) && v3_ok(p, 128, 128));
+        if (!ok) return pl;
+        tile(w320 ? K_V3_192x320 : K_V3_256, 3, bm, bn, 512);
+        return persistent(cus);
+    }
     if (p.gn_in) {
         const int halo = v3d_conv_halo_variant(p, mode);
         if (!halo) return pl;
@@ -877,11 +890,20 @@
     return v3d_check_launch("v3d_gemm");
 }
 
+int launch_up2fold(const GemmPlan& pl, GP& p, hipStream_t st, int& occ) {
+    const int ntiles = (int)pl.tiles;
+    if (pl.kernel == K_V3_192x320) V3D_LAUNCH((gemm_kernel_v3<192, 320, 2, 4, V3D_GEMM_CONV3X3_UP2FOLD, false, 1>), p, ntiles);
+    else V3D_LAUNCH((gemm_kernel_v3<256, 256, 2, 4, V3D_GEMM_CONV3X3_UP2FOLD, false, 1>), p, ntiles);
+    return v3d_check_launch("v3d_gemm(up2 fold)");
+}
+
 int launch_plan(const GemmPlan& pl, GP& p0, hipStream_t st) {
     GP p = p0;
     p.mt = pl.mt; p.nt = pl.nt; p.group_m = pl.group_m;
     int occ = 1, rc;
-    if (pl.family == 5) {
+    if (pl.mode == V3D_GEMM_CONV3X3_UP2FOLD) {
+        rc = launch_up2fold(pl, p, st, occ);
+    } else if (pl.family == 5) {
         p.sk_units = pl.sk_units;
         if (pl.sk_tail) {
             if (!sk_workspace(p, pl.sk_slot_bytes, (int)pl.grid_x, st)) return kNoWorkspace;
@@ -916,7 +938,7 @@
     V3D_REQUIRE(!a->bias || ((uintptr_t)a->bias & 15) == 0, "v3d_gemm: bias must be 16-byte aligned");
     const long long mtiles = (a->M + 127) / 128, ntiles = (a->N + 63) / 64;
     V3D_REQUIRE(mtiles * ntiles < (1ll << 31), "v3d_gemm: grid too large");
-    const int taps = a->mode == V3D_GEMM_LINEAR ? 1 : (a->mode == V3D_GEMM_CONV3X3 ? 9 : 3);
+    const int taps = a->mode == V3D_GEMM_LINEAR ? 1 : (a->mode == V3D_GEMM_CONV3X3 ? 9 : (a->mode == V3D_GEMM_CONV3X3_UP2FOLD ? 4 : 3));
     const long long ldw = a->ldw ? a->ldw : a->K;
     V3D_REQUIRE(ldw >= a->K && ldw % 8 == 0, "v3d_gemm: ldw must be >= K and a multiple of 8");
     const unsigned long long a_bytes = (unsigned long long)a->a_rows * a->lda * 2ull;
@@ -932,6 +954,7 @@
     p.a_row0 = a->a_row0; p.a_bytes = (unsigned)a_bytes; p.w_bytes = (unsigned)w_bytes;
     p.Hin = a->Hin; p.Win = a->Win; p.Hout = a->Hout; p.Wout = a->Wout; p.stride = a->stride;
     p.upshift = 0;
+    p.up_cout = 0;
     p.pad_lo = 1;
     p.T = a->T; p.tmin = a->tmin; p.tmax = a->tmax; p.S = a->S;
     p.halo_rows = a->mode == V3D_GEMM_CONVT3 ? a->halo_rows : 0;
@@ -975,6 +998,14 @@
             p.upshift = a->up - 1;
             p.pad_lo = a->pad_mode ? 0 : 1;
             break;
+        case V3D_GEMM_CONV3X3_UP2FOLD:
+            V3D_REQUIRE(a->Hin > 0 && a->Win > 0 && a->Hout == a->Hin && a->Wout == a->Win && a->stride == 1 && a->up == 1 && a->pad_mode == 0,
+                        "v3d_gemm: the folded upsampling conv runs on the low-res map (Hout = Hin, Wout = Win, stride 1, up 1, pad_mode 0)");
+            V3D_REQUIRE(a->M % ((long long)a->Hin * a->Win) == 0, "v3d_gemm: M must be n_img*Hin*Win");
+            V3D_REQUIRE(a->N % 4 == 0 && a->batch == 1 && !a->geglu && !a->out_fp32 && !a->gn_stats && !a->gn_in_table && !a->A2,
+                        "v3d_gemm: the folded upsampling conv takes N = 4 * Cout phase-major columns and a plain bf16 output");
+            p.up_cout = (int)(a->N / 4);
+            break;
         case V3D_GEMM_CONVT3:
             V3D_REQUIRE(a->T > 0 && a->S > 0, "v3d_gemm: convt3 needs T,S");
             V3D_REQUIRE(a->halo_rows >= 0, "v3d_gemm: halo_rows must be >= 0");
@@ -1045,6 +1076,12 @@
     return plan_gemm(p, a->mode, false, 1, v3d_num_cus(), env_policy()).kernel != K_NONE;
 }
 
+extern "C" int v3d_gemm_up2_fold_supported(const v3d_gemm_args* a) {
+    GP p;
+    if (!a || a->mode != V3D_GEMM_CONV3X3_UP2FOLD || fill_params(a, p) != V3D_OK) return 0;
+    return plan_gemm(p, a->mode, false, 1, v3d_num_cus(), env_policy()).kernel != K_NONE;
+}
+
 extern "C" int v3d_gemm(const v3d_gemm_args* a, v3d_stream_t stream) {
     GP p;
     const int frc = fill_params(a, p);
@@ -1052,6 +1089,8 @@
     hipStream_t st = (hipStream_t)stream;
     GemmPolicy pol = env_policy();
     GemmPlan pl = plan_gemm(p, a->mode, a->geglu != 0, a->batch, v3d_num_cus(), pol);
+    V3D_REQUIRE(pl.kernel != K_NONE || a->mode != V3D_GEMM_CONV3X3_UP2FOLD, "v3d_gemm: this shape is outside the folded upsampling conv's contract "
+                                     "(v3d_gemm_up2_fold_supported): run the 9-tap CONV3X3 call with up = 2");
     V3D_REQUIRE(pl.kernel != K_NONE, "v3d_gemm: gn_in_table is set but this shape is not one of the LDS-haloed kernels' (v3d_gemm_gn_in_supported): "
                                      "normalise the input with v3d_groupnorm_apply first");
     int rc = launch_plan(pl, p, st);
diff --git a/v3d_amd/csrc/gemm_common.h b/v3d_amd/csrc/gemm_common.h
--- a/v3d_amd/csrc/gemm_common.h
+++ b/v3d_amd/csrc/gemm_common.h
@@ -49,6 +49,7 @@
     int sk_units;
     float* sk_ws;
     unsigned* sk_flags;
+    int up_cout;
 };
 
 struct V3dLaunchInfo {
@@ -138,9 +139,13 @@
     }
 };
 
+template <>
+struct RowInfo<V3D_GEMM_CONV3X3_UP2FOLD> : RowInfo<V3D_GEMM_CONV3X3> {};
+__device__ __forceinline__ int fold_tap(int t, int phase) { return ((phase >> 1) + (t >> 1)) * 3 + (phase & 1) + (t & 1); }
+
 template <int MODE>
 constexpr int ntaps() {
-    return MODE == V3D_GEMM_LINEAR ? 1 : (MODE == V3D_GEMM_CONV3X3 ? 9 : 3);
+    return MODE == V3D_GEMM_LINEAR ? 1 : (MODE == V3D_GEMM_CONV3X3 ? 9 : (MODE == V3D_GEMM_CONV3X3_UP2FOLD ? 4 : 3));
 }
 
 __device__ __forceinline__ int xcd_remap(int bid, int nblk) {
@@ -563,7 +568,7 @@
     asm volatile("ds_write_b64 %0, %1" ::"v"(addr), "v"(v) : "memory");
 }
 
-template <int NF, bool GN, int RD = E4_ASM_READS>
+template <int NF, bool GN, int RD = E4_ASM_READS, bool D2S = false>
 __device__ __forceinline__ void e4_fragment(const GP& p, f32x4 (&acc)[NF], long long m0f, long long nw0, int lane, unsigned char* stage, const E4Res& cur,
                                             const E4Tile<NF>& t, GnAcc<GN ? NF : 1>& gn) {
     constexpr int CPRO = NF * 2, NP = 16 * CPRO, SROW = NF * 32 + 16;
@@ -635,6 +640,14 @@
     }
     asm volatile("s_waitcnt lgkmcnt(0)" ::: "memory");
     bf16_t* outz = reinterpret_cast<bf16_t*>(p.out) + m0f * p.ldo + nw0;
+    unsigned d2s_w = 0, d2s_rem = 0;
+    if constexpr (D2S) {
+        d2s_w = (unsigned)p.Wout;
+        const unsigned phase = e4_udiv((unsigned)nw0, (unsigned)p.up_cout), line = e4_udiv((unsigned)m0f, d2s_w);
+        d2s_rem = (unsigned)m0f - line * d2s_w;
+        const long long pix0 = 2 * m0f + 2ll * d2s_w * (line + (phase >> 1)) + (phase & 1);
+        outz = reinterpret_cast<bf16_t*>(p.out) + pix0 * p.ldo + (nw0 - (long long)phase * p.up_cout);
+    }
     constexpr int NK = (NP + 63) / 64;
     static_assert(NK == 2 || NK == 3, "row pieces per lane");
 #pragma unroll
@@ -646,9 +659,15 @@
         e4_lds_read16(sr, sbase + (unsigned)((cr / CPRO) * SROW + (cr % CPRO) * 16));
         asm volatile("s_waitcnt lgkmcnt(0)" : "+v"(sr)::"memory");
         const int row = c / CPRO, ch = c % CPRO;
-        if (NP % 64 == 0 || c < NP) *reinterpret_cast<u32x4*>(outz + (long long)row * p.ldo + ch * 8) = sr;
+        long long orow = row;
+        if constexpr (D2S) {
+            const unsigned r = d2s_rem + (unsigned)row;
+            orow = 2 * row + 2 * (int)d2s_w * ((r >= d2s_w ? 1 : 0) + (r >= 2 * d2s_w ? 1 : 0));
+        }
+        if (NP % 64 == 0 || c < NP) *reinterpret_cast<u32x4*>(outz + orow * p.ldo + ch * 8) = sr;
     }
     } else {
+    static_assert(!D2S, "depth-to-space rows: asm read forms only");
     if (has1) asm volatile("s_waitcnt lgkmcnt(0)" ::: "memory");
 #pragma unroll
     for (int j = 0; j < NF; ++j) {
@@ -707,7 +726,7 @@
         return f + 1 == MF || ends;
     }
 };
-template <int F, int MF, int NF, bool GN, int RD, typename RowFn, typename FlushFn>
+template <int F, int MF, int NF, bool GN, int RD, bool D2S, typename RowFn, typename FlushFn>
 __device__ __forceinline__ void e4_retire(const GP& p, f32x4 (&acc)[MF][NF], long long nw0, int lane, unsigned char* stage, E4Res cur, E4Res n1, E4Res n2,
                                           E4Tile<NF> t, GnAcc<GN ? NF : 1>& gn, RowFn rowfn, FlushFn flushfn) {
     if constexpr (F < MF) {
@@ -735,16 +754,16 @@
             f32x4 accf[NF];
 #pragma unroll
             for (int j = 0; j < NF; ++j) accf[j] = acc[F][j];
-            e4_fragment<NF, GN, RD>(p, accf, m0f, nw0, lane, stage, cur, t, gn);
+            e4_fragment<NF, GN, RD, D2S>(p, accf, m0f, nw0, lane, stage, cur, t, gn);
         }
         if constexpr (GN) {
             unsigned slot = 0, sid = 0;
             if (flushfn(F, m0f, slot, sid)) gn_flush<NF>(p, gn, (long long)sid, nw0, lane, stage, slot);
         }
-        e4_retire<F + 1, MF, NF, GN, RD>(p, acc, nw0, lane, stage, n1, n2, n3, t, gn, rowfn, flushfn);
-    }
-}
-template <int MF, int NF, bool GN, int RD = E4_ASM_READS, typename RowFn, typename FlushFn>
+        e4_retire<F + 1, MF, NF, GN, RD, D2S>(p, acc, nw0, lane, stage, n1, n2, n3, t, gn, rowfn, flushfn);
+    }
+}
+template <int MF, int NF, bool GN, int RD = E4_ASM_READS, bool D2S = false, typename RowFn, typename FlushFn>
 __device__ __forceinline__ void e4_retire_tile(const GP& p, f32x4 (&acc)[MF][NF], long long nw0, int lane, unsigned char* stage, RowFn rowfn, FlushFn flushfn) {
     E4Res r0, r1, r2;
     r0.a0 = r0.a1 = r0.a2 = u32x4{0u, 0u, 0u, 0u};
@@ -756,7 +775,7 @@
     asm volatile("" : "+v"(r0.a0), "+v"(r0.a1), "+v"(r0.a2), "+v"(r1.a0), "+v"(r1.a1), "+v"(r1.a2), "+v"(r2.a0), "+v"(r2.a1), "+v"(r2.a2));
     GnAcc<GN ? NF : 1> gn;
     if constexpr (GN) gn_zero(gn);
-    e4_retire<0, MF, NF, GN, RD>(p, acc, nw0, lane, stage, r0, r1, r2, t, gn, rowfn, flushfn);
+    e4_retire<0, MF, NF, GN, RD, D2S>(p, acc, nw0, lane, stage, r0, r1, r2, t, gn, rowfn, flushfn);
 }
 
 struct SkItem {
diff --git a/v3d_amd/engine/packing.py b/v3d_amd/engine/packing.py
--- a/v3d_amd/engine/packing.py
+++ b/v3d_amd/engine/packing.py
@@ -41,6 +41,38 @@
     if Ip != I:
         w = torch.cat([w, w.new_zeros(O, Ip - I, 3, 3)], dim=1)
     return _bf(w.permute(2, 3, 0, 1).reshape(9, O, Ip)), (None if conv.bias is None else _f(conv.bias))
+
+
+def fold_up2_weights(w: torch.Tensor) -> torch.Tensor:
+    O, I = w.shape[0], w.shape[1]
+    taps = {(0, 0): (0,), (0, 1): (1, 2), (1, 0): (0, 1), (1, 1): (2,)}
+    out = w.new_zeros(4, 4, O, I)
+    for py in range(2):
+        for px in range(2):
+            for i in range(2):
+                for j in range(2):
+                    for ky in taps[(py, i)]:
+                        for kx in taps[(px, j)]:
+                            out[2 * i + j, 2 * py + px] += w[:, :, ky, kx]
+    return out.reshape(4, 4 * O, I)
+
+
+class Up2Pack(tuple):
+
+    def __new__(cls, conv: nn.Conv2d):
+        self = super().__new__(cls, pack_conv3x3(conv))
+        self._folded = None
+        return self
+
+    def folded(self):
+        if self._folded is None:
+            w9, bias = self
+            if w9.is_cuda and torch.cuda.is_current_stream_capturing():
+                return None
+            w = w9.to(F32).view(3, 3, w9.shape[1], w9.shape[2]).permute(2, 3, 0, 1)
+            b = bias if bias is not None else torch.zeros(w.shape[0], dtype=F32, device=w9.device)
+            self._folded = (fold_up2_weights(w).to(w9.dtype).contiguous(), b.repeat(4).contiguous())
+        return self._folded
 
 
 def pack_conv3x3_im2col(conv: nn.Conv2d, Kpad=96):
@@ -359,7 +391,7 @@
             elif isinstance(m, Downsample):
                 items.append(("down", pack_conv3x3(m.op)))
             elif isinstance(m, Upsample):
-                items.append(("up", pack_conv3x3(m.conv)))
+                items.append(("up", Up2Pack(m.conv)))
             elif isinstance(m, nn.Conv2d):
                 items.append(("conv_in", pack_conv3x3(m)))
             else:
@@ -447,7 +479,7 @@
     for lvl in dec.up:
         d = {"blocks": [pack_vae_resblock(b) for b in lvl.block], "upsample": None}
         if hasattr(lvl, "upsample"):
-            d["upsample"] = pack_conv3x3(lvl.upsample.conv)
+            d["upsample"] = Up2Pack(lvl.upsample.conv)
         up.append(d)
     co = dec.conv_out
     tw = co.time_mix_conv.weight.detach()
diff --git a/v3d_amd/engine/unet.py b/v3d_amd/engine/unet.py
--- a/v3d_amd/engine/unet.py
+++ b/v3d_amd/engine/unet.py
@@ -222,7 +222,7 @@
                 h = ops.conv3x3(h, p[0], p[1], g.n, g.H, g.W, stride=2)
                 g = Geo(n=g.n, B=g.B, T=g.T, H=(g.H + 1) // 2, W=(g.W + 1) // 2)
             elif kind == "up":
-                h = ops.conv3x3(h, p[0], p[1], g.n, g.H, g.W, up=2)
+                h = ops.upsample_conv3x3(h, p, g.n, g.H, g.W, in_sampler_loop=True)
                 g = Geo(n=g.n, B=g.B, T=g.T, H=g.H * 2, W=g.W * 2)
             else:
                 raise ValueError(kind)
diff --git a/v3d_amd/engine/vae.py b/v3d_amd/engine/vae.py
--- a/v3d_amd/engine/vae.py
+++ b/v3d_amd/engine/vae.py
@@ -55,7 +55,7 @@
             h = vae_resblock(env, g, p, h)
         us = pk.up[lvl]["upsample"]
         if us is not None:
-            h = ops.conv3x3(h, us[0], us[1], g.n, g.H, g.W, up=2)
+            h = ops.upsample_conv3x3(h, us, g.n, g.H, g.W)
             g = Geo(n=g.n, B=g.B, T=g.T, H=g.H * 2, W=g.W * 2)
     ga, be, eps = pk.norm_out
     h = ops.groupnorm(h, None, ga, be, g.n, g.S, eps=eps, silu=True)
diff --git a/v3d_amd/hip.py b/v3d_amd/hip.py
--- a/v3d_amd/hip.py
+++ b/v3d_amd/hip.py
@@ -11,9 +11,11 @@
 _HERE = os.path.dirname(os.path.abspath(__file__))
 LIB_PATH = os.environ.get("V3D_HIP_LIB") or os.path.join(_HERE, "lib", "libv3d_hip.so")
 
-ABI_VERSION = 9
+ABI_VERSION = 10
 
 c_i64, c_i32, c_f32, c_f64, c_vp = C.c_int64, C.c_int32, C.c_float, C.c_double, C.c_void_p
+
+GEMM_CONV3X3_UP2FOLD = 3
 
 
 class _GemmArgs(C.Structure):
@@ -58,6 +60,7 @@
                                 c_vp, c_i64, c_i64, c_i32, c_i32, c_vp]),
     "v3d_ln_proj": (c_i32, [c_vp, c_i64, c_f32, c_vp, c_vp, c_vp, c_i64, c_vp, c_i64, c_i32, c_i32, c_i32, c_i64, c_vp]),
     "v3d_gemm_gn_in_supported": (c_i32, [C.POINTER(_GemmArgs)]),
+    "v3d_gemm_up2_fold_supported": (c_i32, [C.POINTER(_GemmArgs)]),
     "v3d_groupnorm_stats": (c_i32, [c_vp, c_i64, c_vp, c_i64, c_vp, c_i64, c_i64, c_i64, c_i32, c_i64, c_vp]),
     "v3d_groupnorm_stats_table": (c_i32, [c_vp, c_i64, c_vp, c_i64, c_vp, c_i64, c_vp, c_i64, c_i64, c_i32, c_i64, c_vp, c_vp, C.c_double, C.c_float, c_vp, c_vp]),
     "v3d_groupnorm_finalize": (c_i32, [c_vp, c_i64, c_vp, c_i64, c_i32, c_vp, c_vp, c_i64, c_f64, c_f32, c_vp, c_vp]),
@@ -211,7 +214,7 @@
     def _gemm_in_row_chunks(self, g: GemmCall) -> bool:
         import dataclasses
         import math
-        if g.batch != 1 or g.mode == 2 or g.A.dim() != 2:
+        if g.batch != 1 or g.mode == 2 or g.A.dim() != 2 or g.up_fold:
             return False
         lda = g.A.stride(0)
         rows_in = g.A.shape[0]
@@ -277,6 +280,10 @@
         a.add_rpg, a.add_ld, a.coef_rpg = g.add_rpg, g.add_ld, g.coef_rpg
         a.c_acc, a.c_res1, a.c_res2 = g.c_acc, g.c_res1, g.c_res2
         a.mode, a.geglu, a.out_fp32 = g.mode, int(g.geglu), int(out_fp32)
+        if g.up_fold:
+            if g.mode != 1:
+                raise RuntimeError("gemm: up_fold is a form of the CONV3X3 mode")
+            a.mode = GEMM_CONV3X3_UP2FOLD
         a.Hin, a.Win, a.Hout, a.Wout, a.stride, a.up = g.Hin, g.Win, g.Hout, g.Wout, g.stride, g.up
         a.T, a.tmin, a.tmax, a.S = g.T, g.tmin, g.tmax, g.S
         a.batch = g.batch
@@ -313,6 +320,20 @@
         a = self._gemm_args(g)
         return bool(self.lib.v3d_gemm_gn_in_supported(C.byref(a)))
 
+    UP2_FOLD = True
+
+    def gemm_up2_fold_supported(self, g: GemmCall) -> bool:
+        if not g.up_fold or g.A.dim() != 2 or g.A.shape[0] * g.A.stride(0) * 2 > self._MAX_OPERAND_BYTES:
+            return False
+        a = self._gemm_args(g)
+        return bool(self.lib.v3d_gemm_up2_fold_supported(C.byref(a)))
+
+    def gemm_same_tiles(self, a: GemmCall, b: GemmCall) -> bool:
+        if b.A.shape[0] * b.A.stride(0) * 2 > self._MAX_OPERAND_BYTES:
+            return False
+        pa, pb = self.gemm_plan(a), self.gemm_plan(b)
+        return pa["family"] == 3 and pb["family"] == 3 and (pa["bm"], pa["bn"]) == (pb["bm"], pb["bn"])
+
     def groupnorm_stats(self, x1, x2, stats, n_img, S, groups, imgs_per_stat):
         bf = torch.bfloat16
         self._req_c(x1, bf, "gn.x1")
diff --git a/v3d_amd/ops.py b/v3d_amd/ops.py
--- a/v3d_amd/ops.py
+++ b/v3d_amd/ops.py
@@ -54,6 +54,7 @@
     gn_in_rps: int = 0
     gn_in_silu: bool = True
     A2: Optional[torch.Tensor] = None
+    up_fold: bool = False
 
 
 class OpsBase:
@@ -128,6 +129,31 @@
         self.gemm(GemmCall(A=x, W=w, out=out, M=M, N=N, K=K, bias=bias, mode=GEMM_CONV3X3, Hin=Hin, Win=Win,
                            Hout=Hout, Wout=Wout, stride=stride, up=up, pad_mode=pad_mode, **epi))
         return out
+
+    UP2_FOLD = False
+
+    def gemm_up2_fold_supported(self, g: "GemmCall") -> bool:
+        return False
+
+    def upsample_conv3x3(self, x, p, n_img, Hin, Win, *, in_sampler_loop=False):
+        knob = os.environ.get("V3D_UP2_FOLD", "1")
+        if self.UP2_FOLD and knob not in ("", "0") and (knob == "2" or not in_sampler_loop) and hasattr(p, "folded"):
+            folded = p.folded()
+            if folded is not None:
+                wf, bf = folded
+                M, K, Cout = n_img * Hin * Win, x.shape[-1], wf.shape[-2] // 4
+                out = self.empty((4 * M, Cout), self.act_dtype, x.device)
+                call = GemmCall(A=x, W=wf, out=out, M=M, N=4 * Cout, K=K, bias=bf, mode=GEMM_CONV3X3, Hin=Hin, Win=Win, Hout=Hin, Wout=Win, up_fold=True)
+                nine = GemmCall(A=x, W=p[0], out=out, M=4 * M, N=Cout, K=K, bias=p[1], mode=GEMM_CONV3X3, Hin=Hin, Win=Win, Hout=2 * Hin, Wout=2 * Win, up=2)
+                if self.gemm_up2_fold_supported(call) and (knob == "2" or self.gemm_same_tiles(call, nine)):
+                    self.gemm(call)
+                else:
+                    self.gemm(nine)
+                return out
+        return self.conv3x3(x, p[0], p[1], n_img, Hin, Win, up=2)
+
+    def gemm_same_tiles(self, a: "GemmCall", b: "GemmCall") -> bool:
+        return False
 
     def convt3(self, x, w, bias, T, S, *, tmin=0, tmax=None, a_row0=0, M=None, out=None, out_dtype=None, halo_rows=0, **epi):
         K = x.shape[-1]
```

Result: no change. 12.93 frames/s, median of 6 (+0.3%).
